# mims-harvard/G-Meta

Hardware: AMD Instinct MI355X
Metric: meta-tasks/sec (inner-loop fwd+bwd) at task_num=32 (higher is better)
Workload: dtype f32

## Files before the change

g-meta_amd/_lib.py:

```python
import ctypes as C
import os

HERE = os.path.dirname(os.path.abspath(__file__))
LIB_PATH = os.environ.get('GMETA_HIP_LIB') or os.path.join(HERE, 'libgmeta_hip.so')

GM_MAX_GCN = 4
(F_SUB_OFF, F_SET_SUB_OFF, F_PARENT, F_GRAPH, F_INDPTR, F_INDICES, F_INDPTR_T, F_INDICES_T, F_CENTRE, F_NORM,
 F_FEAT_ROW, F_NORM_SRC, F_NORM_CENTRE, F_EDGE_W, F_EDGE_W_T, F_HOP, F_NORM_E1, F_EDGE_CENTRE_T, F_OBS_CENTRE, F_OBS_E1) = range(20)
LINK_SYMMETRIC = 2
LINK_MASK_TARGET = 4
NEG_MODES = {'uniform': 0, 'two_hop': 1}
PAIR_MASK_TARGET = 1
PROP_SELF_LOOPS = 1
PROP_OPS = {'hadamard': 0, 'abs_diff': 1}
DIST_UNREACHED = 255


class Seed(C.Structure):
    _fields_ = [('graph', C.c_int32), ('i', C.c_int32), ('j', C.c_int32)]


class Model(C.Structure):
    _fields_ = [('n_gcn', C.c_int32), ('dims', C.c_int32 * (GM_MAX_GCN + 1)), ('n_out', C.c_int32), ('link_pred', C.c_int32)]

# ... 13 lines not shown
    'gm_batch_weighted': (i32, [vp]),
    'gm_store_destroy': (None, [vp]),
    'gm_store_negative_pairs': (i32, [vp, i32, i64, u64, i32, vp, i64, vp, vp, vp]),
    'gm_store_has_edges': (i32, [vp, i32, vp, i64, vp, vp]),
    'gm_store_pair_scores': (i32, [vp, i32, vp, i64, i32, vp, vp]),
    'gm_store_pair_walks': (i32, [vp, i32, vp, i64, i32, vp, vp]),
    'gm_store_rooted_pagerank': (i32, [vp, i32, vp, i64, C.c_float, i32, vp, vp]),
    'gm_store_pair_pagerank': (i32, [vp, i32, vp, i64, i32, C.c_float, i32, vp, vp]),
    'gm_store_pagerank_candidates': (i32, [vp, i32, vp, i64, i32, C.c_float, i32, vp, vp, vp, vp]),
    'gm_store_node_distances': (i32, [vp, i32, vp, i64, i32, vp, vp]),
    'gm_store_pair_distance': (i32, [vp, i32, vp, i64, i32, i32, vp, vp]),
    'gm_store_pair_distance_profile': (i32, [vp, i32, vp, i64, i32, i32, vp, vp]),
    'gm_store_sketch_build': (i32, [vp, i32, i32, i32, i32, u64, vp, vp]),
    'gm_sketch_dims': (i32, [vp, vp, vp, vp, vp, vp]),
    'gm_sketch_registers': (i32, [vp, i32, vp, i64, vp, vp, vp]),
    'gm_sketch_pair_counts': (i32, [vp, vp, i64, vp, vp, vp]),
    'gm_sketch_destroy': (None, [vp]),
    'gm_store_propagate_build': (i32, [vp, i32, i32, i32, vp, vp]),
    'gm_prop_dims': (i32, [vp, vp, vp, vp, vp, vp]),
    'gm_prop_rows': (i32, [vp, i32, vp, i64, vp, vp]),
    'gm_prop_pair_features': (i32, [vp, vp, i64, i32, vp, vp]),
    'gm_prop_destroy': (None, [vp]),
    'gm_store_neighbour_degrees': (i32, [vp, i32, vp, vp]),
    'gm_store_pair_candidates': (i32, [vp, i32, vp, i64, i32, i32, vp, vp, vp, vp]),
    'gm_extract': (C.c_int, [vp, vp, i32, vp, i32, i32, i32, u64, i32, vp, vp]),
    'gm_extract_pair': (C.c_int, [vp, vp, i32, vp, i32, vp, i32, vp, i32, i32, i32, u64, i32, vp, vp, vp]),
    'gm_batch_from_nodes': (C.c_int, [vp, vp, i32, vp, i32, vp, vp, i32, vp, vp]),
    'gm_set_hop_labels': (None, [i32]),
    'gm_get_hop_labels': (i32, []),
    'gm_batch_hop_labels': (i32, [vp]),
    'gm_batch_mask_target': (i32, [vp]),
    'gm_batch_concat': (C.c_int, [vp, i32, vp, vp]),
    'gm_batch_destroy': (None, [vp]),
    'gm_batch_prepare_cone': (C.c_int, [vp, i32, vp]),
    'gm_batch_prepare_cone_pair': (C.c_int, [vp, vp, i32, vp]),
    'gm_batch_cone_dims': (C.c_int, [vp, i32, vp, vp, vp]),
    'gm_batch_cone_read': (C.c_int, [vp, i32, i32, i32, vp, i64]),
    'gm_batch_dims': (C.c_int, [vp, vp, vp, vp, vp, vp]),
    'gm_batch_read': (C.c_int, [vp, i32, vp, i64]),
    'gm_batch_device_ptr': (C.c_int, [vp, i32, vp]),
    'gm_batch_source_rows': (C.c_int, [vp, vp]),
    'gm_batch_e1_source_rows': (C.c_int, [vp, vp]),
    'gm_gather_features': (C.c_int, [vp, vp, vp]),
    'gm_aggregate': (C.c_int, [vp, i32, i32, vp, i32, vp, vp, vp, vp]),
    'gm_aggregate_bytes': (i64, [vp, i32]),
    'gm_model_param_count': (i64, [vp]),
    'gm_gcn_ws_bytes': (i64, [vp, vp]),
    'gm_gcn_forward': (C.c_int, [vp, vp, vp, i64, vp, vp, vp, vp, i64, vp]),
    'gm_gcn_backward': (C.c_int, [vp, vp, vp, i64, vp, vp, vp, vp, i64, vp, i64, vp]),
    'gm_dense_update': (C.c_int, [vp, vp, i32, vp, i64, i32, vp, i32, vp]),
    'gm_dense_gemm': (C.c_int, [vp, vp, i64, i32, vp, i64, i32, i32, vp, i64, vp, vp, vp, i64, i32, vp, vp, vp, vp, vp, i32, vp, vp]),
    'gm_dense_fused_gemm': (C.c_int, [vp, i32, vp, i64, i32, vp, i64, vp, i64, vp, i64, i32, vp, i64, vp, vp, vp, i64, i32, vp, vp, vp, i32, vp, vp]),
    'gm_dense_wgrad_fused': (C.c_int, [vp, i32, vp, i64, i32, vp, i64, vp, i64, i32, vp, vp, vp, i64, vp, i64, i32, vp]),
    'gm_dense_aggregate': (C.c_int, [vp, i32, i32, vp, i64, i32, i32, vp, vp, i32, vp, i64, i32, vp, vp, vp, i32, vp, i64, i32, i32, i32, i32, i32, vp, vp, vp]),
    'gm_dense_agg_info': (C.c_int, [vp, i32, vp]),
    'gm_dense_fuse_counts': (C.c_int, [vp, vp]),
    'gm_dense_agg_table': (C.c_int, [vp, i32, i32, vp, i64, vp]),
    'gm_dense_dz_centre': (C.c_int, [vp, vp, i32, vp, i64, i32, vp, vp]),
    'gm_dense_wgrad_centre': (C.c_int, [vp, vp, i32, vp, i32, vp, i64, vp, i64, vp]),
    'gm_dense_agg_centre_t': (C.c_int, [vp, vp, i32, vp, vp, i32, vp]),
    'gm_dense_wgrad_e1': (C.c_int, [vp, vp, i32, vp, i32, vp, i64, vp, i64, vp]),
    'gm_dense_wgrad': (C.c_int, [vp, vp, i64, i32, vp, i64, i32, vp, vp, i64, vp, i64, vp, i64, i32, vp, vp, i64, C.c_float, vp, vp, vp, vp]),
    'gm_proto_loss_spt': (C.c_int, [vp, vp, i32, vp, i32, vp, vp, vp, vp, vp]),
    'gm_proto_loss_qry': (C.c_int, [vp, vp, i32, vp, vp, i32, vp, vp, vp, vp, vp]),
    'gm_dense_head_loss': (C.c_int, [vp, vp, i32, i32, i32, i32, vp, i64, i64, i64, vp, vp, i32, i32, vp, i32, vp, vp, vp, vp, vp, vp, vp, vp, i32, vp, i64, vp, vp,
                                     vp, vp, i64, C.c_float, vp, i32, vp, vp]),
    'gm_set_ragged_classes': (None, [i32]),
    'gm_get_ragged_classes': (i32, []),
    'gm_set_readout': (None, [i32]),
    'gm_get_readout': (i32, []),
    'gm_meta_ws_bytes': (i64, [vp, vp, vp, vp]),
    'gm_meta_out_floats': (i64, [vp, vp, vp]),
    'gm_meta_step': (C.c_int, [vp, vp, vp, vp, vp, vp, vp, vp, i64, vp, i64, vp]),
    'gm_adapt_ws_bytes': (i64, [vp, vp, vp]),
    'gm_meta_adapt': (C.c_int, [vp, vp, vp, vp, vp, vp, i64, vp, i32, vp, i64, vp]),
    'gm_predict_ws_bytes': (i64, [vp, vp, vp]),
    'gm_proto_predict': (C.c_int, [vp, vp, vp, vp, i64, vp, vp, i32, vp, vp, vp, vp, i64, vp]),
    'gm_meta_finish': (C.c_int, [vp, i64, i32, vp, vp, vp]),
    'gm_meta_finish_adam': (C.c_int, [vp, i64, i32, vp, vp, vp, vp, vp, i32, C.c_float, C.c_float, C.c_float, C.c_float, vp, vp, vp]),
    'gm_set_gemm_mode': (None, [i32]),
    'gm_get_gemm_mode': (i32, []),
    'gm_get_split_pieces': (i32, []),
    'gm_set_split_pieces': (None, [i32]),
    'gm_set_tuning': (C.c_int, [C.c_char_p, i32]),
    'gm_get_tuning': (i32, [C.c_char_p]),
    'gm_tuning_epoch': (i32, []),
    'gm_set_fuse_agg': (None, [i32]),
    'gm_get_fuse_agg': (i32, []),
    'gm_profile_enable': (None, [i32]),
    'gm_profile_aggregate': (C.c_int, [vp, vp, vp]),
    'gm_profile_read': (C.c_int, [i32, vp, vp, vp]),
    'gm_profile_read_launches': (C.c_int, [i32, vp, vp, i32]),
}
PROBE_PROTOTYPES = {
    'gm_debug_stamp': (C.c_int, [vp, vp]),
    'gm_stream_debug': (C.c_int, [i32, vp, i32]),
    'gm_head_loss_debug': (C.c_int, [i32, vp]),
}

_lib = None


def lib():
    global _lib
    if _lib is None:
        if not os.path.exists(LIB_PATH):
            raise RuntimeError('gmeta_amd: %s is missing -- run `python -c "import __graft_entry__ as g; g.build()"` '
                               '(hipcc --offload-arch=gfx950).  There is no CPU fallback.' % LIB_PATH)
        l = C.CDLL(LIB_PATH)
        for name, (res, args) in PROTOTYPES.items():
            fn = getattr(l, name)
            fn.restype, fn.argtypes = res, args
        for name, (res, args) in PROBE_PROTOTYPES.items():
            if hasattr(l, name):
                fn = getattr(l, name)
# ... 90 lines not shown
```

g-meta_amd/csrc/agg.hip:

```cpp
#include <algorithm>
#include <stdlib.h>
#include <mutex>
#include "gm_internal.h"
#include "agg_hub.h"

#define AGG_BLOCK 256

struct AggK {
    const int32_t* indptr; const int32_t* indices; const float* x; const int32_t* x_row; int64_t ldx;
    const float* s_in; const float* s_out; const float* mask_h; const float* bias; int64_t bias_stride;
    const int32_t* set_row_off; int n_sets; int relu; float* out; int64_t rows; int width; int nblocks;
    const uint8_t* mask_b; uint8_t* relu_bits;
    const int32_t* heavy; int n_heavy, heavy_deg;
    const int32_t* sched; int sched_len;
    int nt;
    int win;
    const int32_t* hub; float* hub_scratch; int hub_part, hub_ld;
    const float* e_w; const int32_t* x_idx;
    int skip_lo, skip_hi;
    const int32_t* rowlist; int64_t n_list;
    int keep_signed;
};
__host__ __device__ __forceinline__ int agg_xcd_first(const int nb, const int x) {
    const int q = nb / GM_NXCD, r = nb % GM_NXCD;
// ... 230 lines not shown
        if (dg >= 1) agg_edge(a, p0, u0, w0);
        if (dg >= 2) agg_edge(a, p0 + 1, u1, w1);
    }
    const int nwin = (int)min((int64_t)a.win, nrows_w - R0);
    const float* xl = a.x + l * 4;
    const unsigned long long live = __ballot(mine && dg >= 0);
    for (int t0 = 0; t0 < nwin; t0 += G * UNR) {
        if (!((live >> t0) & ((1ull << (G * UNR)) - 1))) continue;
        float4 acc[UNR][NCH];
        int rdg[UNR], rp0[UNR], rrow[UNR]; float rso[UNR];
#pragma unroll
        for (int k = 0; k < UNR; ++k) {
            const int rr = t0 + k * G + g;
            const int src = rr < GM_WAVE ? rr : 0;
            rdg[k] = rr < nwin ? __shfl(dg, src, 64) : -1;
            rrow[k] = __shfl(myrow32, src, 64);
            if (a.n_heavy && rdg[k] > a.heavy_deg) rdg[k] = -1;
            rp0[k] = __shfl(p0, src, 64); rso[k] = __shfl(so, src, 64);
            const int a0 = __shfl(u0, src, 64), a1 = __shfl(u1, src, 64);
            const float f0 = __shfl(w0, src, 64), f1 = __shfl(w1, src, 64);
#pragma unroll
            for (int c = 0; c < NCH; ++c) acc[k][c] = make_float4(0.f, 0.f, 0.f, 0.f);
            if (rdg[k] >= 1) {
#pragma unroll
                for (int c = 0; c < NCH; ++c) vfma(acc[k][c], *reinterpret_cast<const float4*>(xl + (int64_t)a0 * a.ldx + c * LPR * 4), f0);
            }
            if (rdg[k] >= 2) {
#pragma unroll
                for (int c = 0; c < NCH; ++c) vfma(acc[k][c], *reinterpret_cast<const float4*>(xl + (int64_t)a1 * a.ldx + c * LPR * 4), f1);
            }
        }
#pragma unroll
        for (int k = 0; k < UNR; ++k) {
            if (rdg[k] < 0) continue;
            const int rr_ = t0 + k * G + g;
            const int64_t row = a.rowlist ? (int64_t)rrow[k] : R0 + rr_;
            const int eend = rp0[k] + rdg[k];
            for (int eb = rp0[k] + 2; eb < eend; eb += LPR) agg_gather_batch<LPR, NCH, LPR, 4>(a, xl, eb, eend, l, g * LPR, acc[k]);
            agg_store_row<LPR, NCH>(a, row, rso[k], l, acc[k], a.nt);
        }
    }
}

int gm_agg_window(int64_t rows, int64_t edges) {
    const bool dense = edges > 8 * rows;
    const int min_waves = dense ? 16384 : 32768;
    const int min_win = dense ? 4 : 2;
    int win = 64;
    while (win > min_win && rows / win < min_waves) win >>= 1;
    return win;
}

int gm_agg_schedule_flat(gm_batch* b, int64_t rows, int win, const int32_t* pos, int n_heavy, const std::vector<int32_t>& tab, int32_t** d_sched, int32_t* len_out,
                         hipStream_t s, gm_stager* sg) {
    const bool split = !tab.empty();
    const int RPB = win * (AGG_BLOCK / GM_WAVE);
    const int nwb = std::max(1, (int)((rows + RPB - 1) / RPB));
    auto x_start = [&](int x) { return agg_xcd_first(nwb, x); };
    auto n_entries = [&](int k) { return split ? tab[k + 1] - tab[k] : 1; };
    int extra[GM_NXCD] = {}; int first[GM_NXCD + 1];
    {
        int hk = 0;
        for (int x = 0; x < GM_NXCD; ++x) {
            const int end = x_start(x + 1);
            first[x] = hk;
            while (hk < n_heavy && pos[hk] / RPB < end) {
                GM_REQUIRE(hk == 0 || pos[hk] >= pos[hk - 1], GM_EINVAL, "aggregate schedule: hub-row list is not ascending");
                extra[x] += n_entries(hk); ++hk;
            }
        }
        first[GM_NXCD] = hk;
        GM_REQUIRE(hk == n_heavy, GM_EINVAL, "aggregate schedule: hub-row list is not ascending / out of range");
    }
    size_t len = 0;
    for (int x = 0; x < GM_NXCD; ++x) len = std::max(len, (size_t)(x_start(x + 1) - x_start(x) + extra[x]));
    std::vector<int32_t> flat(GM_NXCD * len);
    for (int x = 0; x < GM_NXCD; ++x) {
        int32_t* o = flat.data() + x * len; int32_t* const o_end = o + len;
        int wb = x_start(x); const int end = x_start(x + 1);
        for (int hk = first[x]; hk < first[x + 1]; ++hk) {
            const int hb = pos[hk] / RPB;
            while (wb <= hb) *o++ = wb++;
            if (split) for (int g = tab[hk]; g < tab[hk + 1]; ++g) *o++ = -g - 2;
            else *o++ = -hk - 2;
        }
        while (wb < end) *o++ = wb++;
        while (o < o_end) *o++ = -1;
    }
    GM_TRY(gm_balloc(b, d_sched, flat.size(), s));
    GM_TRY(sg->upload(*d_sched, flat));
    *len_out = (int32_t)len;
    return GM_OK;
}

int gm_agg_schedule(gm_batch* b, int64_t rows, int win, const int32_t* heavy_host, const int32_t* heavy_deg_host, int n_heavy, gm_agg_sched* out, hipStream_t s, gm_stager* sg) {
    *out = gm_agg_sched{};
    if (n_heavy <= 0 || rows <= 0) return GM_OK;
    int hub_part = 0;
    std::vector<int32_t> tab;
    if (heavy_deg_host) {
        int maxdeg = 0;
        for (int k = 0; k < n_heavy; ++k) maxdeg = std::max(maxdeg, heavy_deg_host[k]);
        hub_part = std::max(128, ((maxdeg + 31) / 32 + 15) / 16 * 16);
        tab.assign(n_heavy + 1, 0);
        for (int k = 0; k < n_heavy; ++k) tab[k + 1] = tab[k] + std::max(1, (heavy_deg_host[k] + hub_part / 2) / hub_part);
        const int parts = tab[n_heavy];
        if (parts == n_heavy) { hub_part = 0; tab.clear(); }
        else {
            tab.resize(n_heavy + 1 + parts + n_heavy, 0);
            for (int k = 0; k < n_heavy; ++k) for (int g = tab[k]; g < tab[k + 1]; ++g) tab[n_heavy + 1 + g] = k;
        }
    }
    GM_TRY(gm_agg_schedule_flat(b, rows, win, heavy_host, n_heavy, tab, &out->d_sched, &out->len, s, sg));
    if (hub_part) {
        GM_TRY(gm_balloc(b, &out->d_hub, tab.size(), s));
        GM_TRY(sg->upload(out->d_hub, tab));
        GM_TRY(gm_balloc(b, &out->d_hub_scratch, (size_t)tab[n_heavy] * GM_AGG_HUB_LD, s));
        out->hub_part = hub_part; out->hub_words = (int32_t)tab.size(); out->parts = tab[n_heavy];
    }
    out->tab = tab;
    return GM_OK;
}

template <int LPR, int NCH>
static void launch_win(const AggK& a0, hipStream_t s, int* launched) {
    AggK a = a0;
    a.win = (a.sched || a.rowlist) ? a0.win : gm_agg_window(a.rows, 0);
    const int RPB = a.win * (AGG_BLOCK / GM_WAVE);
    a.nblocks = (int)(((a.rowlist ? a.n_list : a.rows) + RPB - 1) / RPB);
    int grid = a.nblocks;
    if (a.sched) grid = GM_NXCD * a.sched_len;
    else if (a.n_heavy > 0) hipLaunchKernelGGL((k_agg_heavy<LPR, NCH>), dim3(a.n_heavy), dim3(AGG_HEAVY_BLOCK), 0, s, a);
    hipLaunchKernelGGL((k_agg_win<LPR, NCH>), dim3(grid), dim3(AGG_BLOCK), 0, s, a);
    if (launched) *launched = GM_AGG_ID_WIN(LPR, NCH) + (a.sched ? GM_AGG_ID_WIN_SCHED + (a.hub ? GM_AGG_ID_WIN_SPLIT : 0) : a.n_heavy > 0 ? GM_AGG_ID_WIN_HEAVY : 0) +
                                (a.rowlist ? GM_AGG_ID_WIN_LIST : 0);
}

// ... 109 lines not shown
```

g-meta_amd/csrc/common.hip:

```cpp
#include <stdarg.h>
#include <stdlib.h>
#include <atomic>
#include <chrono>
#include <map>
#include <mutex>
#include <set>
#include <utility>
#include "gm_internal.h"

static thread_local char g_err[512] = "";

void gm_set_error(const char* fmt, ...) {
    va_list ap;
    va_start(ap, fmt);
    vsnprintf(g_err, sizeof(g_err), fmt, ap);
    va_end(ap);
}

extern "C" const char* gm_last_error(void) { return g_err; }
extern "C" int gm_version(void) { return 100; }

static void pool_keep_memory() {
    static thread_local int done_for = -1;
    int dev = 0;
// ... 251 lines not shown
extern "C" int gm_profile_read(int32_t category, double* total_ms, int64_t* launches, int64_t* work) {
    GM_REQUIRE(category >= 0 && category < GM_PROF_CATS, GM_EINVAL, "profile_read: unknown category %d", category);
    ProfCat& c = g_prof[category];
    double tot = 0;
    for (size_t k = 0; k + 1 < c.used + 1 && k < c.used; k += 2) {
        GM_HIP(hipEventSynchronize(c.ev[k + 1]));
        float ms = 0;
        GM_HIP(hipEventElapsedTime(&ms, c.ev[k], c.ev[k + 1]));
        tot += ms;
    }
    if (total_ms) *total_ms = tot;
    if (launches) *launches = c.launches;
    if (work) *work = c.work;
    return GM_OK;
}
extern "C" int gm_profile_read_launches(int32_t category, double* ms, int64_t* work, int32_t cap) {
    GM_REQUIRE(category >= 0 && category < GM_PROF_CATS && ms && work && cap >= 0, GM_EINVAL, "profile_read_launches: bad arguments");
    ProfCat& c = g_prof[category];
    int n = 0;
    for (size_t k = 0; k + 1 < c.used + 1 && k < c.used && n < cap; k += 2, ++n) {
        GM_HIP(hipEventSynchronize(c.ev[k + 1]));
        float t = 0;
        GM_HIP(hipEventElapsedTime(&t, c.ev[k], c.ev[k + 1]));
        ms[n] = t; work[n] = k / 2 < c.works.size() ? c.works[k / 2] : 0;
    }
    return n;
}
extern "C" int gm_profile_aggregate(double* total_ms, int64_t* launches, int64_t* algorithmic_bytes) {
    return gm_profile_read(GM_PROF_AGG, total_ms, launches, algorithmic_bytes);
}

#ifdef GM_PROBES
__global__ void k_debug_stamp(unsigned long long* out) { *out = wall_clock64(); }
extern "C" int gm_debug_stamp(void* out, void* stream) {
    GM_REQUIRE(out, GM_EINVAL, "debug_stamp: NULL argument");
    hipLaunchKernelGGL(k_debug_stamp, dim3(1), dim3(1), 0, (hipStream_t)stream, (unsigned long long*)out);
    GM_HIP(hipGetLastError());
    return GM_OK;
}
#endif

static gm_knobs g_knobs;
static std::once_flag g_knobs_once;
const gm_knobs& gm_knob() {
    gm_knobs& k = g_knobs;
    std::call_once(g_knobs_once, [] {
        gm_knobs& k = g_knobs;
        auto env = [](const char* name, int dflt) { const char* e = getenv(name); return e ? atoi(e) : dflt; };
        k.timing = env("GM_TIMING", 0);
        const char* gm = getenv("GM_GEMM_MODE");
        k.gemm_mode = (gm && (!strcmp(gm, "split") || !strcmp(gm, "1"))) ? 1 : (gm && (!strcmp(gm, "f32") || !strcmp(gm, "0"))) ? 0 : -1;
        k.gemm_split_min_tiles = env("GM_GEMM_SPLIT_MIN_TILES", -1);
        k.centre_store = env("GM_CENTRE_STORE", 2);
        k.dead_rows = env("GM_DEAD_ROWS", 3);
        k.fuse_agg = env("GM_FUSE_AGG", 1);
        k.fuse_diff = env("GM_FUSE_DIFF", 2);
        k.extract_pref16 = env("GM_EXTRACT_PREF16", 1);
        k.head_stage = env("GM_HEAD_STAGE", 1);
        k.head_threads = env("GM_HEAD_THREADS", 0);
        k.query_streams = env("GM_QUERY_STREAMS", 0);
        k.agg_mid_list = env("GM_AGG_MID_LIST", 1);
        k.agg_mid_win = env("GM_AGG_MID_WIN", 0);
        k.split_pieces = env("GM_SPLIT_PIECES", 3);
        k.split16_min_rows = env("GM_SPLIT16_MIN_ROWS", 65536);
        k.wgrad_split_min_chunks = env("GM_WGRAD_SPLIT_MIN_CHUNKS", -1);
        k.agg_stream = env("GM_AGG_STREAM", 1);
        k.agg_stream_min_rows = env("GM_AGG_STREAM_MIN_ROWS", 100000);
        k.neg_round = env("GM_NEG_ROUND", 0);
        k.pair_lanes = env("GM_PAIR_LANES", 0);
        k.cand_round = env("GM_CAND_ROUND", 0);
        k.cand_bitmap = env("GM_CAND_BITMAP", 0);
        k.walk_chunk = env("GM_WALK_CHUNK", 0);
        k.walk_lanes = env("GM_WALK_LANES", 0);
        k.ppr_chunk = env("GM_PPR_CHUNK", 0);
        k.ppr_cols = env("GM_PPR_COLS", 0);
        k.dist_chunk = env("GM_DIST_CHUNK", 0);
        k.dist_cols = env("GM_DIST_COLS", 0);
        k.dist_plane_kib = env("GM_DIST_PLANE_KIB", 0);
        k.sketch_chunk = env("GM_SKETCH_CHUNK", 0);
        k.sketch_mib = env("GM_SKETCH_MIB", 0);
        k.prop_chunk = env("GM_PROP_CHUNK", 0);
        k.prop_mib = env("GM_PROP_MIB", 0);
    });
    return k;
}

static std::atomic<int> g_tuning_epoch{0};
extern "C" int32_t gm_tuning_epoch(void) { return g_tuning_epoch.load(std::memory_order_relaxed); }
static int gm_knobs::* gm_find_knob(const char* name) {
    (void)gm_knob();
    static const struct { const char* name; int gm_knobs::*field; } tab[] = {
        {"GM_GEMM_SPLIT_MIN_TILES", &gm_knobs::gemm_split_min_tiles}, {"GM_CENTRE_STORE", &gm_knobs::centre_store}, {"GM_DEAD_ROWS", &gm_knobs::dead_rows},
        {"GM_HEAD_STAGE", &gm_knobs::head_stage}, {"GM_HEAD_THREADS", &gm_knobs::head_threads}, {"GM_QUERY_STREAMS", &gm_knobs::query_streams}, {"GM_AGG_MID_LIST", &gm_knobs::agg_mid_list}, {"GM_AGG_MID_WIN", &gm_knobs::agg_mid_win}, {"GM_AGG_STREAM", &gm_knobs::agg_stream}, {"GM_AGG_STREAM_MIN_ROWS", &gm_knobs::agg_stream_min_rows},
        {"GM_SPLIT16_MIN_ROWS", &gm_knobs::split16_min_rows}, {"GM_WGRAD_SPLIT_MIN_CHUNKS", &gm_knobs::wgrad_split_min_chunks}, {"GM_TIMING", &gm_knobs::timing},
        {"GM_FUSE_DIFF", &gm_knobs::fuse_diff}, {"GM_EXTRACT_PREF16", &gm_knobs::extract_pref16},
        {"neg_round", &gm_knobs::neg_round}, {"GM_NEG_ROUND", &gm_knobs::neg_round},
        {"pair_lanes", &gm_knobs::pair_lanes}, {"GM_PAIR_LANES", &gm_knobs::pair_lanes},
        {"cand_round", &gm_knobs::cand_round}, {"GM_CAND_ROUND", &gm_knobs::cand_round},
        {"cand_bitmap", &gm_knobs::cand_bitmap}, {"GM_CAND_BITMAP", &gm_knobs::cand_bitmap},
        {"walk_chunk", &gm_knobs::walk_chunk}, {"GM_WALK_CHUNK", &gm_knobs::walk_chunk},
        {"walk_lanes", &gm_knobs::walk_lanes}, {"GM_WALK_LANES", &gm_knobs::walk_lanes},
        {"ppr_chunk", &gm_knobs::ppr_chunk}, {"GM_PPR_CHUNK", &gm_knobs::ppr_chunk},
        {"ppr_cols", &gm_knobs::ppr_cols}, {"GM_PPR_COLS", &gm_knobs::ppr_cols},
        {"dist_chunk", &gm_knobs::dist_chunk}, {"GM_DIST_CHUNK", &gm_knobs::dist_chunk},
        {"dist_cols", &gm_knobs::dist_cols}, {"GM_DIST_COLS", &gm_knobs::dist_cols},
        {"dist_plane_kib", &gm_knobs::dist_plane_kib}, {"GM_DIST_PLANE_KIB", &gm_knobs::dist_plane_kib},
        {"sketch_chunk", &gm_knobs::sketch_chunk}, {"GM_SKETCH_CHUNK", &gm_knobs::sketch_chunk},
        {"sketch_mib", &gm_knobs::sketch_mib}, {"GM_SKETCH_MIB", &gm_knobs::sketch_mib},
        {"prop_chunk", &gm_knobs::prop_chunk}, {"GM_PROP_CHUNK", &gm_knobs::prop_chunk},
        {"prop_mib", &gm_knobs::prop_mib}, {"GM_PROP_MIB", &gm_knobs::prop_mib},
    };
    for (const auto& e : tab)
        if (!strcmp(name, e.name)) return e.field;
    return nullptr;
}
extern "C" int gm_set_tuning(const char* name, int32_t value) {
    GM_REQUIRE(name, GM_EINVAL, "set_tuning: NULL name");
    int gm_knobs::* f = gm_find_knob(name);
    GM_REQUIRE(f, GM_EINVAL, "set_tuning: unknown or start-up-only knob %s", name);
    g_knobs.*f = value; g_tuning_epoch.fetch_add(1, std::memory_order_relaxed);
    return GM_OK;
}
extern "C" int32_t gm_get_tuning(const char* name) {
    int gm_knobs::* f = name ? gm_find_knob(name) : nullptr;
    return f ? g_knobs.*f : 0;
}

int gm_heavy_deg() { return 64; }
int gm_heavy_deg_for(int64_t rows, int64_t edges) {
    return edges <= 8 * rows ? 32 : 64;
}

static std::mutex g_dev_mu;

int gm_num_cus() {
    static std::map<int, int> cus;
    int dev = 0;
    if (hipGetDevice(&dev) != hipSuccess) { (void)hipGetLastError(); return 256; }
    std::lock_guard<std::mutex> lk(g_dev_mu);
    auto it = cus.find(dev);
    if (it != cus.end()) return it->second;
    int n = 0;
    if (hipDeviceGetAttribute(&n, hipDeviceAttributeMultiprocessorCount, dev) != hipSuccess || n <= 0) { (void)hipGetLastError(); n = 256; }
    cus[dev] = n;
    return n;
}
// ... 12 lines not shown
```

g-meta_amd/csrc/dense_exports.hip:

```cpp
#include <algorithm>
#include "gm_internal.h"

static int set_row_amax(const gm_batch* b, const float* x, int64_t ldx, int cols, unsigned* slots, hipStream_t st) {
    int rc = GM_OK;
    for (int t0 = 0; rc == GM_OK && t0 < b->sets; t0 += 8) {
        const int segs = std::min(8, b->sets - t0);
        int64_t xo[8], xn[8];
        for (int i = 0; i < segs; ++i) {
            const int64_t r0 = b->h_set_row_off[t0 + i], nr = b->h_set_row_off[t0 + i + 1] - r0;
            xo[i] = r0 * ldx; xn[i] = nr > 0 ? (nr - 1) * ldx + cols : 0;
        }
        rc = gm_amax_segs(x, xo, xn, segs, slots + (int64_t)t0 * GM_BOUND_PAD, GM_BOUND_PAD, st);
    }
    return rc;
}

extern "C" int gm_dense_update(const gm_batch_t* b, const float* x, int32_t K, const float* W, int64_t w_stride, int32_t N, float* out, int32_t mode,
                               void* stream) {
    GM_REQUIRE(b && x && W && out && K >= 1 && N >= 1, GM_EINVAL, "dense_update: bad arguments");
    hipStream_t st = (hipStream_t)stream;
    gm_gemm_args g{};
    g.A = x; g.lda = K; g.B = W; g.b_stride = w_stride; g.C = out; g.ldc = N; g.K = K; g.N = N;
    g.tiles = b->d_tiles; g.n_tiles = b->n_tiles; g.rows = b->rows;
    uint16_t* planes = nullptr; unsigned* slots = nullptr;
// ... 13 lines not shown
            g.np = 2; g.a_bound = gm_no_bound(); g.a_bound.amax = slots; g.b_bound = wb;
        }
        if (rc == GM_OK) rc = gm_split_weights(W, w_stride, 0, K, N, 0, sets, planes, st, mode == 2 ? 2 : 3, wb);
        if (rc != GM_OK) { gm_dev_free(planes, st); if (slots) gm_dev_free(slots, st); return rc; }
        g.Bsplit = planes; g.bsplit_stride = w_stride ? (int64_t)3 * K * N : 0;
    }
    const int rc = gm_launch_gemm_nn(g, st);
    if (planes) gm_dev_free(planes, st);
    if (slots) gm_dev_free(slots, st);
    gm_batch_mark_use(b, st);
    return rc;
}

extern "C" int gm_dense_gemm(const gm_batch_t* b, const float* x, int64_t ldx, int32_t K, const float* W, int64_t w_stride, int32_t trans_w, int32_t N,
                             float* out, int64_t ldc, const float* s, const float* s_keep, const float* bias, int64_t bias_stride, int32_t relu,
                             uint8_t* relu_bits, const float* mask_h, const uint8_t* mask_b, float* zero_out, uint32_t* amax_out, int32_t mode,
                             int32_t* launched, void* stream) {
    GM_REQUIRE(b && x && W && out && K >= 1 && N >= 1 && ldx >= K && ldc >= N && mode >= -1 && mode <= 2 && !(mask_h && mask_b), GM_EINVAL,
               "dense_gemm: bad arguments");
    GM_REQUIRE(!amax_out || mode == 2, GM_EINVAL, "dense_gemm: amax_out is an output of the two-piece kernels (mode 2)");
    hipStream_t st = (hipStream_t)stream;
    const int sets = b->sets;
    gm_gemm_args g{};
    g.A = x; g.lda = ldx; g.B = W; g.b_stride = w_stride; g.transB = trans_w ? 1 : 0; g.C = out; g.ldc = ldc; g.K = K; g.N = N;
    g.row_scale = s; g.row_scale_keep = s_keep; g.n_keep = b->rows; g.bias = bias; g.bias_stride = bias_stride; g.relu = relu ? 1 : 0;
    g.relu_bits = relu_bits; g.mask_h = mask_h; g.mask_b = mask_b; g.zero_out = zero_out;
    g.tiles = b->d_tiles; g.n_tiles = b->n_tiles; g.rows = b->rows; g.launched = launched;
    uint16_t* planes = nullptr; unsigned* slots = nullptr;
    int rc = GM_OK;
    if (mode == 1 || mode == 2 || (mode < 0 && gm_gemm_split_ok(b->n_tiles, K, N))) {
        GM_REQUIRE(!mask_h && !mask_b, GM_EINVAL, "dense_gemm: the split kernels take no relu' mask");
        GM_REQUIRE((N == 256 || N == 128) && K % 16 == 0 && K >= 32, GM_EINVAL, "dense_gemm: the split kernels need N = 128 or 256 and K a multiple of 16 (>= 32)");
        const int wsets = w_stride ? sets : 1;
        rc = gm_alloc(&planes, (size_t)wsets * 3 * K * N, st);
        gm_bound wb = gm_no_bound();
        if (rc == GM_OK && mode == 2) {
            rc = gm_alloc(&slots, (size_t)(sets + wsets) * GM_BOUND_PAD, st);
            if (rc == GM_OK && hipMemsetAsync(slots, 0, sizeof(unsigned) * (sets + wsets) * GM_BOUND_PAD, st) != hipSuccess) { gm_set_error("dense_gemm: memset failed"); rc = GM_EHIP; }
            if (rc == GM_OK) rc = set_row_amax(b, x, ldx, K, slots, st);
            if (rc == GM_OK) rc = gm_amax(W, w_stride, 0, (int64_t)K * N, wsets, slots + (int64_t)sets * GM_BOUND_PAD, GM_BOUND_PAD, st);
            wb.amax = slots + (int64_t)sets * GM_BOUND_PAD; wb.stride = w_stride ? GM_BOUND_PAD : 0;
            g.np = 2; g.a_bound = gm_no_bound(); g.a_bound.amax = slots; g.a_bound.stride = GM_BOUND_PAD; g.b_bound = wb; g.amax_out = amax_out;
        }
        if (rc == GM_OK) rc = gm_split_weights(W, w_stride, 0, K, N, trans_w ? 1 : 0, wsets, planes, st, mode == 2 ? 2 : 3, wb);
        g.Bsplit = planes; g.bsplit_stride = w_stride ? (int64_t)3 * K * N : 0;
    }
    if (rc == GM_OK) rc = gm_launch_gemm_nn(g, st);
    if (planes) gm_dev_free(planes, st);
    if (slots) gm_dev_free(slots, st);
    gm_batch_mark_use(b, st);
    return rc;
}

extern "C" int gm_dense_fused_gemm(const gm_batch_t* b, int32_t table, const float* x, int64_t ldx, int32_t K, const float* zside, int64_t ldz,
                                   const float* zfull, int64_t ldzf, const float* W, int64_t w_stride, int32_t N, float* out, int64_t ldc, const float* s,
                                   const float* s_keep, const float* bias, int64_t bias_stride, int32_t relu, uint8_t* relu_bits, float* zero_out,
                                   uint32_t* amax_out, int32_t mode, int32_t* launched, void* stream) {
    GM_REQUIRE(b && W && out && zside && K >= 1 && N >= 1 && ldz >= K && ldc >= N && (mode == 1 || mode == 2) && (table == 0 || table == 1), GM_EINVAL,
               "dense_fused_gemm: bad arguments");
    GM_REQUIRE(b->d_fuse2 && b->d_fuse2_feat, GM_EINVAL, "dense_fused_gemm: the batch carries no source tables");
    GM_REQUIRE(table == 1 || (x && ldx >= K), GM_EINVAL, "dense_fused_gemm: table 0 needs x and ldx >= K");
    GM_REQUIRE(table == 0 || (b->feat && (K == b->feat_dim || K == b->feat_ld)), GM_EINVAL, "dense_fused_gemm: table 1 needs K == feat_dim (%d)", b->feat_dim);
    GM_REQUIRE(!amax_out || mode == 2, GM_EINVAL, "dense_fused_gemm: amax_out is an output of the two-piece kernels (mode 2)");
    GM_REQUIRE(mode != 2 || (zfull && ldzf >= K), GM_EINVAL, "dense_fused_gemm: mode 2 takes its A bounds over a fully aggregated Z (zfull)");
    GM_REQUIRE((N == 256 || N == 128) && K % 16 == 0 && K >= 32, GM_EINVAL, "dense_fused_gemm: the split kernels need N = 128 or 256 and K a multiple of 16 (>= 32)");
    hipStream_t st = (hipStream_t)stream;
    const int sets = b->sets, wsets = w_stride ? sets : 1;
    gm_gemm_args g{};
    g.B = W; g.b_stride = w_stride; g.C = out; g.ldc = ldc; g.K = K; g.N = N;
    g.row_scale = s; g.row_scale_keep = s_keep; g.n_keep = b->rows; g.bias = bias; g.bias_stride = bias_stride; g.relu = relu ? 1 : 0;
    g.relu_bits = relu_bits; g.zero_out = zero_out;
    g.tiles = b->d_tiles; g.n_tiles = b->n_tiles; g.rows = b->rows; g.launched = launched;
    g.zside = zside; g.ldz = ldz;
    if (table == 1) { g.A = b->feat; g.lda = b->feat_ld; g.fuse2 = b->d_fuse2_feat; }
    else { g.A = x; g.lda = ldx; g.fuse2 = b->d_fuse2; }
    uint16_t* planes = nullptr; unsigned* slots = nullptr;
    int rc = gm_alloc(&planes, (size_t)wsets * 3 * K * N, st);
    gm_bound wb = gm_no_bound();
    if (rc == GM_OK && mode == 2) {
        rc = gm_alloc(&slots, (size_t)(sets + wsets) * GM_BOUND_PAD, st);
        if (rc == GM_OK && hipMemsetAsync(slots, 0, sizeof(unsigned) * (sets + wsets) * GM_BOUND_PAD, st) != hipSuccess) { gm_set_error("dense_fused_gemm: memset failed"); rc = GM_EHIP; }
        if (rc == GM_OK) rc = set_row_amax(b, zfull, ldzf, K, slots, st);
        if (rc == GM_OK) rc = gm_amax(W, w_stride, 0, (int64_t)K * N, wsets, slots + (int64_t)sets * GM_BOUND_PAD, GM_BOUND_PAD, st);
        wb.amax = slots + (int64_t)sets * GM_BOUND_PAD; wb.stride = w_stride ? GM_BOUND_PAD : 0;
        g.np = 2; g.a_bound = gm_no_bound(); g.a_bound.amax = slots; g.a_bound.stride = GM_BOUND_PAD; g.b_bound = wb; g.amax_out = amax_out;
    }
    if (rc == GM_OK) rc = gm_split_weights(W, w_stride, 0, K, N, 0, wsets, planes, st, mode == 2 ? 2 : 3, wb);
    g.Bsplit = planes; g.bsplit_stride = w_stride ? (int64_t)3 * K * N : 0;
    if (rc == GM_OK) rc = gm_launch_gemm_nn(g, st);
    if (planes) gm_dev_free(planes, st);
    if (slots) gm_dev_free(slots, st);
    gm_batch_mark_use(b, st);
    return rc;
}

extern "C" int gm_dense_dz_centre(const gm_batch_t* b, const float* dQ, int32_t K, const float* W, int64_t w_stride, int32_t N, float* T, void* stream) {
    GM_REQUIRE(b && dQ && W && T && b->d_dq_tab, GM_EINVAL, "dense_dz_centre: bad arguments");
    GM_REQUIRE((N == 256 || N == 128) && K % 16 == 0 && K >= 64, GM_EINVAL, "dense_dz_centre: the fused split kernel needs N = 128 or 256 and K a multiple of 16 (>= 64)");
    hipStream_t st = (hipStream_t)stream;
    const int wsets = w_stride ? b->sets : 1;
    uint16_t* planes = nullptr;
    GM_TRY(gm_alloc(&planes, (size_t)wsets * 3 * K * N, st));
    gm_gemm_args g{};
    g.A = dQ; g.lda = K; g.B = W; g.b_stride = w_stride; g.transB = 1; g.C = T; g.ldc = N; g.K = K; g.N = N;
    g.row_scale = b->d_norm; g.tiles = b->d_tiles; g.n_tiles = b->n_tiles; g.rows = b->rows;
    g.fuse2 = b->d_dq_tab; g.zside = dQ; g.ldz = K;
    int rc = gm_split_weights(W, w_stride, 0, K, N, 1, wsets, planes, st, 3, gm_no_bound());
    g.Bsplit = planes; g.bsplit_stride = w_stride ? (int64_t)3 * K * N : 0; g.np = 3;
    if (rc == GM_OK) rc = gm_launch_gemm_nn(g, st);
    gm_dev_free(planes, st);
    gm_batch_mark_use(b, st);
    return rc;
}
static int dense_wgrad_keep(const gm_batch_t* b, const float* keep, const float* x, int32_t Kx, const float* dQ, int32_t N, float* dW, int64_t dw_stride, float* db,
                            int64_t db_stride, void* stream) {
    GM_REQUIRE(b && x && dQ && dW && db && keep, GM_EINVAL, "dense_wgrad_centre / _e1: bad arguments");
    const int64_t KN = (int64_t)Kx * N;
    GM_REQUIRE(b->sets == 1 || (dw_stride >= KN && db_stride >= N), GM_EINVAL, "dense_wgrad_centre / _e1: per-set outputs overlap");
    hipStream_t st = (hipStream_t)stream;
    gm_wgrad_args w{};
    w.A = x; w.lda = Kx; w.K = Kx; w.G = dQ; w.ldg = N; w.N = N; w.a_scale = b->d_norm; w.g_keep = keep;
    w.chunks = b->d_chunks; w.n_chunks = b->n_chunks; w.set_chunk_off = b->d_set_chunk_off; w.sets = b->sets; w.rows = b->rows;
    w.dW = dW; w.dw_stride = dw_stride; w.db = db; w.db_stride = db_stride; w.pick = GM_WGRAD_PICK_SPLIT;
    int rc = gm_alloc(&w.partial, (size_t)std::max(1, b->n_chunks) * (size_t)(KN + N), st);
    if (rc == GM_OK) rc = gm_launch_wgrad(w, st);
    if (w.partial) gm_dev_free(w.partial, st);
    gm_batch_mark_use(b, st);
    return rc;
}
extern "C" int gm_dense_wgrad_centre(const gm_batch_t* b, const float* x, int32_t Kx, const float* dQ, int32_t N, float* dW, int64_t dw_stride, float* db,
                                     int64_t db_stride, void* stream) {
    return dense_wgrad_keep(b, b ? b->d_norm_c : nullptr, x, Kx, dQ, N, dW, dw_stride, db, db_stride, stream);
}

extern "C" int gm_dense_agg_centre_t(const gm_batch_t* b, float* T, int32_t width, const uint8_t* mask_b, float* out, int32_t keep, void* stream) {
    GM_REQUIRE(b && T && out && width >= 4 && width % 4 == 0, GM_EINVAL, "dense_agg_centre_t: bad arguments");
    GM_REQUIRE(!keep || (b->d_ect && b->d_norm_e1), GM_EINVAL, "dense_agg_centre_t: the batch carries no centre-edge tables");
    hipStream_t st = (hipStream_t)stream;
    gm_agg_args a{};
    a.indptr = b->d_indptr_t; a.indices = b->d_indices_t;
    a.heavy = b->d_heavy[1]; a.n_heavy = b->n_heavy[1]; a.heavy_deg = b->heavy_deg;
    a.sched = b->d_sched[1]; a.sched_len = b->sched_len[1]; a.sched_win = b->sched_win;
    GM_TRY(gm_agg_hub(a, b, 1, st));
    if (b->weighted) a.e_w = b->d_ew[1];
    a.rows = b->rows; a.x = T; a.ldx = width; a.s_out = b->d_norm; a.mask_b = mask_b; a.out = out; a.width = width;
    if (keep) {
// ... 1 lines not shown
        a.x_idx = b->d_ect; a.s_out = b->d_norm_e1; a.keep_signed = 1;
    }
    const int rc = gm_launch_aggregate(a, st);
    gm_batch_mark_use(b, st);
    return rc;
}
extern "C" int gm_dense_wgrad_e1(const gm_batch_t* b, const float* x, int32_t Kx, const float* dQ, int32_t N, float* dW, int64_t dw_stride, float* db,
                                 int64_t db_stride, void* stream) {
    return dense_wgrad_keep(b, b ? b->d_norm_e1 : nullptr, x, Kx, dQ, N, dW, dw_stride, db, db_stride, stream);
}

extern "C" int gm_dense_wgrad(const gm_batch_t* b, const float* x, int64_t ldx, int32_t K, const float* g, int64_t ldg, int32_t N, const float* s,
                              const float* gb, int64_t ldgb, float* dW, int64_t dw_stride, float* db, int64_t db_stride, int32_t mode,
                              const float* cur, float* next, int64_t p_stride, float lr, float* wt, uint16_t* pl_fwd, uint16_t* pl_dz, void* stream) {
    GM_REQUIRE(b && x && g && dW && K >= 1 && N >= 1 && ldx >= K && ldg >= N && (!gb || ldgb >= N) && mode >= -1 && mode <= 2, GM_EINVAL,
               "dense_wgrad: bad arguments");
    GM_REQUIRE(K <= 2048 && N <= 2048, GM_ERANGE, "dense_wgrad: K=%d N=%d: at most 2048 columns per operand", K, N);
    const int sets = b->sets;
    const int64_t KN = (int64_t)K * N;
    GM_REQUIRE(sets == 1 || (dw_stride >= KN && (!db || db_stride >= N)), GM_EINVAL, "dense_wgrad: per-set outputs overlap");
    GM_REQUIRE(!next || (cur && db && (sets == 1 || p_stride >= KN + N)), GM_EINVAL, "dense_wgrad: the SGD step needs cur, db and a stride of at least (K+1)*N");
    GM_REQUIRE((!wt && !pl_fwd && !pl_dz) || next, GM_EINVAL, "dense_wgrad: wt and the planes are outputs of the SGD step");
    GM_REQUIRE((!pl_fwd && !pl_dz) || (K % 32 == 0 && N % 32 == 0), GM_EINVAL, "dense_wgrad: weight planes need K and N multiples of 32");
    hipStream_t st = (hipStream_t)stream;
    gm_wgrad_args w{};
    w.A = x; w.lda = ldx; w.K = K; w.G = g; w.ldg = ldg; w.N = N; w.Gb = gb; w.ldgb = ldgb; w.a_scale = s;
    w.chunks = b->d_chunks; w.n_chunks = b->n_chunks; w.set_chunk_off = b->d_set_chunk_off; w.sets = sets; w.rows = b->rows;
    w.dW = dW; w.dw_stride = dw_stride; w.db = db; w.db_stride = db_stride;
    if (next) {
        w.sgd_cur = cur; w.sgd_cur_stride = p_stride; w.sgd_next = next; w.sgd_next_stride = p_stride; w.sgd_lr = lr; w.w_off = 0; w.b_off = KN;
        w.wt_next = wt; w.pl_fwd = pl_fwd; w.pl_dz = pl_dz;
    }
    w.pick = mode == 0 ? GM_WGRAD_PICK_EXACT : mode > 0 ? GM_WGRAD_PICK_SPLIT : 0;
    unsigned* slots = nullptr;
    int rc = gm_alloc(&w.partial, (size_t)std::max(1, b->n_chunks) * (size_t)(KN + N), st);
    if (rc == GM_OK && mode == 2) {
        rc = gm_alloc(&slots, (size_t)(2 * sets + 1) * GM_BOUND_PAD, st);
        if (rc == GM_OK && hipMemsetAsync(slots, 0, sizeof(unsigned) * (2 * sets + 1) * GM_BOUND_PAD, st) != hipSuccess) { gm_set_error("dense_wgrad: memset failed"); rc = GM_EHIP; }
        if (rc == GM_OK) rc = set_row_amax(b, x, ldx, K, slots, st);
        if (rc == GM_OK) rc = set_row_amax(b, g, ldg, N, slots + (int64_t)sets * GM_BOUND_PAD, st);
        if (rc == GM_OK && s) rc = gm_amax(s, 0, 0, b->rows, 1, slots + (int64_t)2 * sets * GM_BOUND_PAD, 0, st);
        w.np = 2;
        w.a_bound = gm_no_bound(); w.a_bound.amax = slots; w.a_bound.stride = GM_BOUND_PAD;
        if (s) w.a_bound.gain = reinterpret_cast<const float*>(slots + (int64_t)2 * sets * GM_BOUND_PAD);
        w.g_bound = gm_no_bound(); w.g_bound.amax = slots + (int64_t)sets * GM_BOUND_PAD; w.g_bound.stride = GM_BOUND_PAD;
    }
    if (rc == GM_OK) rc = gm_launch_wgrad(w, st);
    if (w.partial) gm_dev_free(w.partial, st);
    if (slots) gm_dev_free(slots, st);
    gm_batch_mark_use(b, st);
    return rc;
}

extern "C" int gm_dense_wgrad_fused(const gm_batch_t* b, int32_t table, const float* A, int64_t lda, int32_t K, const float* gx, int64_t ldgx, const float* g,
                                    int64_t ldg, int32_t N, const float* s, const float* g_keep, float* dW, int64_t dw_stride, float* db, int64_t db_stride,
                                    int32_t mode, void* stream) {
    GM_REQUIRE(b && A && g && dW && db && K >= 1 && N >= 1 && lda >= K && ldg >= N && mode >= 0 && mode <= 2 && (table == 0 || table == 1), GM_EINVAL,
               "dense_wgrad_fused: bad arguments");
    GM_REQUIRE(K <= 2048 && N <= 2048, GM_ERANGE, "dense_wgrad_fused: K=%d N=%d: at most 2048 columns per operand", K, N);
    GM_REQUIRE(b->d_fuse2 && b->d_fuse2_feat, GM_EINVAL, "dense_wgrad_fused: the batch carries no source tables");
    GM_REQUIRE(table == 1 || (gx && ldgx >= K), GM_EINVAL, "dense_wgrad_fused: table 0 needs gx and ldgx >= K");
    GM_REQUIRE(table == 0 || (b->feat && (K == b->feat_dim || K == b->feat_ld)), GM_EINVAL, "dense_wgrad_fused: table 1 needs K == feat_dim (%d)", b->feat_dim);
    const int sets = b->sets;
    const int64_t KN = (int64_t)K * N;
    GM_REQUIRE(sets == 1 || (dw_stride >= KN && db_stride >= N), GM_EINVAL, "dense_wgrad_fused: per-set outputs overlap");
    hipStream_t st = (hipStream_t)stream;
    gm_wgrad_args w{};
    w.A = A; w.lda = lda; w.K = K; w.G = g; w.ldg = ldg; w.N = N; w.a_scale = s; w.g_keep = g_keep;
    w.chunks = b->d_chunks; w.n_chunks = b->n_chunks; w.set_chunk_off = b->d_set_chunk_off; w.sets = sets; w.rows = b->rows;
    w.dW = dW; w.dw_stride = dw_stride; w.db = db; w.db_stride = db_stride;
    w.fuse2 = table == 1 ? b->d_fuse2_feat : b->d_fuse2;
    w.gx = table == 1 ? b->feat : gx; w.ldgx = table == 1 ? b->feat_ld : ldgx;
    w.pick = mode == 0 ? GM_WGRAD_PICK_EXACT : GM_WGRAD_PICK_SPLIT;
    unsigned* slots = nullptr;
    int rc = gm_alloc(&w.partial, (size_t)std::max(1, b->n_chunks) * (size_t)(KN + N), st);
    if (rc == GM_OK && mode == 2) {
        rc = gm_alloc(&slots, (size_t)(2 * sets + 1) * GM_BOUND_PAD, st);
        if (rc == GM_OK && hipMemsetAsync(slots, 0, sizeof(unsigned) * (2 * sets + 1) * GM_BOUND_PAD, st) != hipSuccess) { gm_set_error("dense_wgrad_fused: memset failed"); rc = GM_EHIP; }
        w.np = 2;
        w.a_bound = gm_no_bound(); w.a_bound.amax = slots; w.a_bound.stride = GM_BOUND_PAD;
        w.g_bound = gm_no_bound(); w.g_bound.amax = slots + (int64_t)sets * GM_BOUND_PAD; w.g_bound.stride = GM_BOUND_PAD;
    }
    if (rc == GM_OK) rc = gm_launch_wgrad(w, st);
    if (w.partial) gm_dev_free(w.partial, st);
    if (slots) gm_dev_free(slots, st);
    gm_batch_mark_use(b, st);
    return rc;
}

extern "C" int gm_dense_aggregate(const gm_batch_t* b, int32_t transposed, int32_t x_src, const float* x, int64_t ldx, int32_t width, int32_t scale_src,
                                  const float* s_in, const float* s_out, int32_t keep_signed, const float* bias, int64_t bias_stride, int32_t relu,
                                  uint8_t* relu_bits, const float* mask_h, const uint8_t* mask_b, int32_t hubs, const int32_t* rowlist, int64_t n_list,
                                  int32_t list_win, int32_t list_sched, int32_t skip_lo, int32_t skip_hi, int32_t stream_ok, float* out, int32_t* launched,
                                  void* stream) {
    GM_REQUIRE(b && out && width >= 1 && x_src >= 0 && x_src <= 3 && scale_src >= 0 && scale_src <= 2 && hubs >= 0 && hubs <= 2, GM_EINVAL, "dense_aggregate: bad arguments");
    GM_REQUIRE(!(mask_h && mask_b), GM_EINVAL, "dense_aggregate: mask_h together with mask_b");
    GM_REQUIRE(!(rowlist && stream_ok), GM_EINVAL, "dense_aggregate: a row list together with the stream kernel");
    GM_REQUIRE(!stream_ok || hubs == 2, GM_EINVAL, "dense_aggregate: the stream kernel takes the batch's hub tables (hubs == 2)");
    const int o = transposed ? 1 : 0;
    const bool gather = x_src == 1 || x_src == 2;
    GM_REQUIRE(gather || (x && ldx >= width), GM_EINVAL, "dense_aggregate: a caller matrix needs x and ldx >= width");
    GM_REQUIRE(!gather || width == b->feat_dim, GM_EINVAL, "dense_aggregate: a gather needs width == feat_dim (%d)", b->feat_dim);
    GM_REQUIRE(x_src != 2 || (!transposed && b->d_efeat), GM_EINVAL, "dense_aggregate: the per-edge feature rows belong to the by-destination CSR");
    GM_REQUIRE(x_src != 3 || (transposed && b->d_ect), GM_EINVAL, "dense_aggregate: the centre-edge table belongs to the by-source CSR of a batch that carries one");
    GM_REQUIRE((scale_src == 1) == (s_in != nullptr), GM_EINVAL, "dense_aggregate: s_in goes with scale_src == 1 and only with it");
    GM_REQUIRE(scale_src != 2 || b->d_enorm[o], GM_EINVAL, "dense_aggregate: the batch has no per-edge norm table");
    GM_REQUIRE(!bias || !bias_stride || b->d_set_row_off, GM_EINVAL, "dense_aggregate: per-set bias without set row offsets");
    GM_REQUIRE(!keep_signed || s_out, GM_EINVAL, "dense_aggregate: keep_signed needs s_out");
    GM_REQUIRE(!relu_bits || relu, GM_EINVAL, "dense_aggregate: relu_bits are written with relu");
    hipStream_t st = (hipStream_t)stream;
    gm_agg_args a{};
    a.indptr = transposed ? b->d_indptr_t : b->d_indptr;
    a.indices = transposed ? b->d_indices_t : b->d_indices;
    a.rows = b->rows; a.width = width; a.out = out; a.launched = launched;
    if (gather) { a.x = b->feat; a.ldx = b->feat_ld; a.x_row = b->d_feat_row; if (x_src == 2) a.x_idx = b->d_efeat; }
    else { a.x = x; a.ldx = ldx; if (x_src == 3) a.x_idx = b->d_ect; }
    if (b->weighted) {
        GM_REQUIRE(scale_src != 1, GM_EINVAL, "dense_aggregate: on a weighted batch the source scale is none or the batch's own table (the per-source gather has no edge-weight slot)");
        GM_REQUIRE(x_src != 1, GM_EINVAL, "dense_aggregate: on a weighted batch the feature gather goes through the per-edge row table (x_src 2; the per-source gather has no edge-weight slot)");
        if (scale_src == 0) a.e_w = b->d_ew[o];
    }
    if (scale_src == 1) a.s_in = s_in;
    if (scale_src == 2) { a.s_in = b->d_norm; a.e_w = b->d_enorm[o]; }
    a.s_out = s_out; a.keep_signed = keep_signed ? 1 : 0;
    a.bias = bias; a.bias_stride = bias_stride; a.set_row_off = b->d_set_row_off; a.n_sets = b->sets;
    a.relu = relu ? 1 : 0; a.relu_bits = relu_bits; a.mask_h = mask_h; a.mask_b = mask_b;
    if (hubs) { a.heavy = b->d_heavy[o]; a.n_heavy = b->n_heavy[o]; a.heavy_deg = b->heavy_deg; }
    if (hubs == 2) { a.sched = b->d_sched[o]; a.sched_len = b->sched_len[o]; a.sched_win = b->sched_win; GM_TRY(gm_agg_hub(a, b, o, st)); }
    if (skip_lo <= skip_hi) { a.skip_on = 1; a.skip_lo = skip_lo; a.skip_hi = skip_hi; }
    if (rowlist) {
        GM_REQUIRE(n_list >= 1 && n_list <= b->rows && list_win >= 2 && list_win <= 64 && (list_win & (list_win - 1)) == 0, GM_EINVAL,
                   "dense_aggregate: a row list needs 1 .. rows entries and a window of 2, 4, .. 64 rows");
        std::vector<int32_t> h((size_t)n_list);
        GM_HIP(hipMemcpyAsync(h.data(), rowlist, sizeof(int32_t) * (size_t)n_list, hipMemcpyDeviceToHost, st));
        GM_HIP(hipStreamSynchronize(st));
        for (int64_t k = 0; k < n_list; ++k)
            GM_REQUIRE(h[k] >= 0 && h[k] < b->rows && (k == 0 || h[k] > h[k - 1]), GM_EINVAL, "dense_aggregate: the row list is not ascending / out of range at entry %lld", (long long)k);
        a.rowlist = rowlist; a.n_list = n_list; a.list_win = list_win;
        if (list_sched) {
            GM_REQUIRE(hubs == 2 && !transposed && b->d_sched_mid && n_list == b->n_mid && list_win == b->mid_win, GM_EINVAL,
                       "dense_aggregate: the list schedule goes with the batch's own list (%d rows, windows of %d) and its hub tables", b->n_mid, b->mid_win);
            a.sched = b->d_sched_mid; a.sched_len = b->sched_len_mid; a.sched_win = b->mid_win;
        } else { a.sched = nullptr; a.sched_len = 0; }
    } else GM_REQUIRE(!list_sched, GM_EINVAL, "dense_aggregate: a list schedule without a row list");
    if (stream_ok && a.e_w && a.e_w == b->d_enorm[o]) GM_TRY(gm_agg_stream_args(a, b, o, gather, st));
    const int rc = gm_launch_aggregate(a, st);
    gm_batch_mark_use(b, st);
    return rc;
}

extern "C" int gm_dense_agg_info(const gm_batch_t* b, int32_t transposed, int64_t* info) {
    GM_REQUIRE(b && info, GM_EINVAL, "dense_agg_info: bad arguments");
    const int o = transposed ? 1 : 0;
    const int64_t v[16] = {b->heavy_deg, b->n_heavy[o], b->sched_win, b->hub_part[o], b->hub_parts[o], b->d_sched[o] ? 1 : 0, b->d_mid ? b->n_mid : 0, b->mid_win,
                           b->d_sched_mid ? 1 : 0, b->d_sseg[o] ? b->stream_nseg[o] : 0, b->stream_nwg[o], b->stream_hubwg[o], b->weighted ? 1 : 0, b->feat_dim, b->feat_ld, 0};
    std::copy(v, v + 16, info);
    return GM_OK;
}
extern "C" int gm_dense_fuse_counts(const gm_batch_t* b, int64_t* counts) {
    GM_REQUIRE(b && counts, GM_EINVAL, "dense_fuse_counts: bad arguments");
    counts[0] = b->unfused_rows; counts[1] = b->unfused_edges;
    return GM_OK;
}
extern "C" int gm_dense_agg_table(const gm_batch_t* b, int32_t which, int32_t transposed, void* dst, int64_t n, void* stream) {
    GM_REQUIRE(b && dst && n >= 0 && which >= 0 && which <= 9, GM_EINVAL, "dense_agg_table: bad arguments");
    const int o = transposed ? 1 : 0;
    const void* src = which == 0 ? (const void*)b->d_enorm[o] : which == 1 ? (const void*)b->d_efeat : which == 2 ? (const void*)b->d_mid : which == 3 ? (const void*)b->d_heavy[o]
                    : which == 4 ? (const void*)b->d_fuse2 : which == 5 ? (const void*)b->d_fuse2_feat : which == 6 ? (const void*)b->d_dq_tab
                    : which == 7 ? (const void*)b->d_fwd_tab[0] : which == 8 ? (const void*)b->d_fwd_tab[1] : (const void*)b->d_fwd_tab_feat;
    const int64_t have = which <= 1 ? b->edges : which == 2 ? b->n_mid : which == 3 ? b->n_heavy[o] : b->rows;
    GM_REQUIRE(src && n <= have, GM_EINVAL, "dense_agg_table: table %d holds %lld entries", which, (long long)(src ? have : 0));
    if (n) GM_HIP(hipMemcpyAsync(dst, src, (which >= 4 ? 16 : 4) * (size_t)n, hipMemcpyDeviceToDevice, (hipStream_t)stream));
    gm_batch_mark_use(b, (hipStream_t)stream);
    return GM_OK;
}
```

g-meta_amd/csrc/extract.hip:

```cpp
#include <algorithm>
#include <initializer_list>
#include <stdlib.h>
#include <string.h>
#include <memory>
#include <mutex>
#include <type_traits>
#include "gm_internal.h"
#include "gm_devutil.h"

#define EX_BLOCK 512
#define EX_WAVES (EX_BLOCK / GM_WAVE)

__device__ __forceinline__ int lane_id() { return __builtin_amdgcn_mbcnt_hi(~0u, __builtin_amdgcn_mbcnt_lo(~0u, 0u)); }
__device__ __forceinline__ int wave_sum(int v) {
#pragma unroll
    for (int o = 32; o > 0; o >>= 1) v += __shfl_xor(v, o, 64);
    return v;
}
template <bool G> __device__ __forceinline__ bool bit_test(const uint32_t* bm, int v) { return (wld<G>(&bm[v >> 5]) >> (v & 31)) & 1u; }
__device__ __forceinline__ void bit_set(uint32_t* bm, int v) { atomicOr(&bm[v >> 5], 1u << (v & 31)); }
template <bool G, typename PT> __device__ __forceinline__ int pref_ld(const PT* p) {
    if constexpr (sizeof(PT) == 4) return (int)wld<G>(reinterpret_cast<const uint32_t*>(p)); else return (int)*p;
}
template <bool G, typename PT> __device__ __forceinline__ int bit_rank(const uint32_t* bm, const PT* pref, int v) {
// ... 572 lines not shown
    if (b->rows <= 0 || b->unfused_edges <= 0) return b->unfused_src = 0;
    const int64_t words = (b->rows + 31) / 32;
    uint32_t* bits = nullptr; unsigned long long* cnt = nullptr; unsigned long long h = 0;
    if (gm_alloc(&bits, (size_t)words, s) != GM_OK || gm_alloc(&cnt, 1, s) != GM_OK) { gm_dev_free(bits, s); return fallback; }
    bool ok = hipMemsetAsync(bits, 0, 4 * (size_t)words, s) == hipSuccess && hipMemsetAsync(cnt, 0, 8, s) == hipSuccess;
    if (ok) {
        hipLaunchKernelGGL(k_mark_sources, dim3((int)std::min<int64_t>(2048, (b->rows + 255) / 256)), dim3(256), 0, s, b->d_indptr, b->d_indices, (int64_t)b->rows, GM_FUSE_MAXDEG, bits);
        hipLaunchKernelGGL(k_count_bits, dim3((int)std::min<int64_t>(512, (words + 255) / 256)), dim3(256), 0, s, bits, words, cnt);
        ok = hipMemcpyAsync(&h, cnt, 8, hipMemcpyDeviceToHost, s) == hipSuccess && hipStreamSynchronize(s) == hipSuccess;
    }
    if (!ok) (void)hipGetLastError();
    gm_dev_free(bits, s); gm_dev_free(cnt, s);
    return ok ? (b->unfused_src = (int64_t)h) : fallback;
}
#define MID_BLOCK 1024
__device__ __forceinline__ bool mid_row(const int32_t* indptr, int64_t r, int64_t rows, int lo, int hi) {
    if (r >= rows) return false;
    const int d = indptr[r + 1] - indptr[r];
    return d >= lo && d <= hi;
}
__global__ __launch_bounds__(MID_BLOCK) void k_mid_count(const int32_t* indptr, int64_t rows, int lo, int hi, int32_t* bcnt) {
    __shared__ int wsum[MID_BLOCK / 64];
    const int64_t r = (int64_t)blockIdx.x * MID_BLOCK + threadIdx.x;
    const unsigned long long m = __ballot(mid_row(indptr, r, rows, lo, hi));
    if ((threadIdx.x & 63) == 0) wsum[threadIdx.x >> 6] = __popcll(m);
    __syncthreads();
    if (threadIdx.x == 0) { int t = 0; for (int k = 0; k < MID_BLOCK / 64; ++k) t += wsum[k]; bcnt[blockIdx.x] = t; }
}
__global__ __launch_bounds__(1024) void k_mid_scan(int32_t* bcnt, int nb) {
    __shared__ int part[1024];
    const int per = (nb + 1023) / 1024, a = threadIdx.x * per, b = min(nb, a + per);
    int t = 0;
    for (int k = a; k < b; ++k) t += bcnt[k];
    part[threadIdx.x] = t;
    __syncthreads();
    if (threadIdx.x == 0) { int run = 0; for (int k = 0; k < 1024; ++k) { const int v = part[k]; part[k] = run; run += v; } }
    __syncthreads();
    int run = part[threadIdx.x];
    for (int k = a; k < b; ++k) { const int v = bcnt[k]; bcnt[k] = run; run += v; }
}
__global__ __launch_bounds__(MID_BLOCK) void k_mid_scatter(const int32_t* indptr, int64_t rows, int lo, int hi, const int32_t* boff, int32_t* list, int cap) {
    __shared__ int wsum[MID_BLOCK / 64];
    const int64_t r = (int64_t)blockIdx.x * MID_BLOCK + threadIdx.x;
    const bool f = mid_row(indptr, r, rows, lo, hi);
    const unsigned long long m = __ballot(f);
    const int lane = threadIdx.x & 63, wv = threadIdx.x >> 6;
    if (lane == 0) wsum[wv] = __popcll(m);
    __syncthreads();
    int base = boff[blockIdx.x];
    for (int k = 0; k < wv; ++k) base += wsum[k];
    const int at = base + __popcll(m & ((1ull << lane) - 1ull));
    if (f && at < cap) list[at] = (int32_t)r;
}
__global__ void k_centre_rows(const int32_t* sub_off, const int32_t* centre, int nc, int n_c, const int32_t* indptr, const float* norm,
                              int32_t* crow, float* cnorm, int32_t* cdeg, float* norm_c, int32_t* centre_copy, int4* dq_tab) {
    const int k = blockIdx.x * blockDim.x + threadIdx.x;
    if (k >= n_c) return;
    const int row = sub_off[k / nc] + centre[k];
    centre_copy[k] = centre[k];
    crow[k] = row; cnorm[k] = norm[row]; cdeg[k] = indptr[row + 1] - indptr[row];
    if (norm_c) norm_c[row] = __uint_as_float(__float_as_uint(norm[row]) & 0x7fffffffu);
    if (dq_tab) dq_tab[row] = make_int4(row | GM_FUSE_SELF, GM_FUSE_ZERO, __float_as_int(1.f), 0);
}
struct CentreW { const float* ew; float* e_coef; };
template <typename... WArgs>
__global__ void k_centre_edges(const int32_t* crow, const int32_t* eoff, int n_c, const int32_t* indptr, const int32_t* indices,
                               const float* norm, int32_t* e_row, int32_t* e_par, float* e_norm, WArgs... w_args) {
    const int k = blockIdx.x;
    if (k >= n_c) return;
    const int p0 = indptr[crow[k]], n = eoff[k + 1] - eoff[k], o = eoff[k];
    for (int j = threadIdx.x; j < n; j += blockDim.x) {
        const int u = indices[p0 + j]; e_row[o + j] = u; e_par[o + j] = k; e_norm[o + j] = norm[u];
        if constexpr (sizeof...(WArgs) != 0) { const CentreW& cw = (w_args, ...); cw.e_coef[o + j] = cw.ew[p0 + j] * norm[u]; }
    }
}
__global__ void k_e1_tables(const int32_t* indices_t, int64_t edges, const float* norm, const float* norm_c, int64_t rows, int32_t* ect, float* norm_e1, int32_t* n_rows) {
    const int64_t n = edges > rows ? edges : rows;
    if (blockIdx.x == 0 && threadIdx.x == 0) *n_rows = 0;
    for (int64_t k = blockIdx.x * (int64_t)blockDim.x + threadIdx.x; k < n; k += (int64_t)gridDim.x * blockDim.x) {
        if (k < rows) norm_e1[k] = __uint_as_float(__float_as_uint(norm[k]) | 0x80000000u);
        if (k < edges) { const int v = indices_t[k]; ect[k] = (__float_as_uint(norm_c[v]) >> 31) ? (int32_t)(rows + (k & (GM_ZERO_ROWS - 1))) : v; }
    }
}
__global__ void k_e1_rows(const int32_t* e_row, int n_e1, float* norm_e1, int32_t* n_rows) {
    const int k = blockIdx.x * blockDim.x + threadIdx.x;
    if (k >= n_e1) return;
    const unsigned old = atomicAnd(reinterpret_cast<unsigned*>(norm_e1) + e_row[k], 0x7fffffffu);
    if (old >> 31) atomicAdd(n_rows, 1);
}
int64_t gm_batch_e1_rows(const gm_batch* b, hipStream_t s) {
    if (b->n_e1_rows >= 0) return b->n_e1_rows;
    const int64_t fallback = std::min<int64_t>(b->n_e1, b->rows);
    if (!b->d_n_e1_rows) return fallback;
    int32_t h = 0;
    if (hipMemcpyAsync(&h, b->d_n_e1_rows, 4, hipMemcpyDeviceToHost, s) != hipSuccess || hipStreamSynchronize(s) != hipSuccess) { (void)hipGetLastError(); return fallback; }
    return b->n_e1_rows = h;
}
__global__ void k_e1_kept_edges(const int32_t* indptr_t, const float* norm_e1, int64_t rows, unsigned long long* out) {
    unsigned long long c = 0;
    for (int64_t r = blockIdx.x * (int64_t)blockDim.x + threadIdx.x; r < rows; r += (int64_t)gridDim.x * blockDim.x)
        if (!(__float_as_uint(norm_e1[r]) >> 31)) c += (unsigned long long)(indptr_t[r + 1] - indptr_t[r]);
#pragma unroll
    for (int off = 32; off >= 1; off >>= 1) c += __shfl_down(c, off, 64);
    if ((threadIdx.x & 63) == 0 && c) atomicAdd(out, c);
}
int64_t gm_batch_e1_edges(const gm_batch* b, hipStream_t s) {
// ... 307 lines not shown
        } else b->spend[o].pending = true;
    }
    if (b->d_fuse2 && gm_knob().agg_mid_list) {
        const int64_t n_mid = b->unfused_rows - (int64_t)b->n_heavy[0];
        if (n_mid > 0 && n_mid < b->rows && h_cnt[0] <= cap) {
            const int nb = (int)((b->rows + MID_BLOCK - 1) / MID_BLOCK);
            int32_t* d_bcnt = nullptr;
            GM_TRY(gm_alloc(&d_bcnt, (size_t)nb, s));
            GM_TRY(gm_balloc(b, &b->d_mid, (size_t)n_mid, s));
            hipLaunchKernelGGL(k_mid_count, dim3(nb), dim3(MID_BLOCK), 0, s, b->d_indptr, (int64_t)b->rows, GM_FUSE_MAXDEG + 1, b->heavy_deg, d_bcnt);
            hipLaunchKernelGGL(k_mid_scan, dim3(1), dim3(1024), 0, s, d_bcnt, nb);
            hipLaunchKernelGGL(k_mid_scatter, dim3(nb), dim3(MID_BLOCK), 0, s, b->d_indptr, (int64_t)b->rows, GM_FUSE_MAXDEG + 1, b->heavy_deg, d_bcnt, b->d_mid, (int)n_mid);
            GM_HIP(hipGetLastError());
            gm_dev_free(d_bcnt, s);
            b->n_mid = (int32_t)n_mid;
            int win = 64;
            while (win > 2 && n_mid / win < 16384) win >>= 1;
            if (gm_knob().agg_mid_win > 0) win = gm_knob().agg_mid_win;
            b->mid_win = win;
            if (b->n_heavy[0] > 0 && b->d_sched[0]) {
                std::vector<int32_t> pos(heavy0.size());
                for (size_t k = 0; k < heavy0.size(); ++k) pos[k] = (int32_t)std::min<int64_t>(n_mid - 1, (int64_t)heavy0[k] * n_mid / b->rows);
                GM_TRY(gm_agg_schedule_flat(b, n_mid, win, pos.data(), (int)heavy0.size(), tab0, &b->d_sched_mid, &b->sched_len_mid, s, &sg));
            }
        }
    }
    tm.lap("mid-list");
    std::vector<int32_t> eoff(b->n_c + 1, 0);
    for (int k = 0; k < b->n_c; ++k) eoff[k + 1] = eoff[k] + h_cdeg[k];
    b->n_e1 = eoff[b->n_c];
    int32_t* d_eoff = nullptr;
    GM_TRY(gm_alloc(&d_eoff, eoff.size(), s));
    GM_TRY(sg.upload(d_eoff, eoff));
    GM_TRY(gm_balloc(b, &b->d_e1_row, b->n_e1, s)); GM_TRY(gm_balloc(b, &b->d_e1_par, b->n_e1, s)); GM_TRY(gm_balloc(b, &b->d_e1_norm, b->n_e1, s));
    if (b->weighted) GM_TRY(gm_balloc(b, &b->d_e1_coef, b->n_e1, s));
    auto centre_edges = [&](auto kern, auto... w) {
        hipLaunchKernelGGL(kern, dim3(b->n_c), dim3(64), 0, s, b->d_crow, d_eoff, b->n_c, b->d_indptr, b->d_indices, b->d_norm, b->d_e1_row, b->d_e1_par, b->d_e1_norm, w...);
    };
    if (b->weighted) centre_edges(k_centre_edges<CentreW>, CentreW{b->d_ew[0], b->d_e1_coef}); else centre_edges(k_centre_edges<>);
    GM_HIP(hipGetLastError());
    if (b->rows > 0 && b->d_norm_c) {
        GM_TRY(gm_balloc(b, &b->d_ect, (size_t)b->edges, s)); GM_TRY(gm_balloc(b, &b->d_norm_e1, (size_t)b->rows, s)); GM_TRY(gm_balloc(b, &b->d_n_e1_rows, 1, s));
        hipLaunchKernelGGL(k_e1_tables, dim3(grid_for(std::max<int64_t>(b->edges, b->rows), 4096)), dim3(256), 0, s, b->d_indices_t, (int64_t)b->edges, b->d_norm, b->d_norm_c, (int64_t)b->rows, b->d_ect, b->d_norm_e1, b->d_n_e1_rows);
        if (b->n_e1 > 0) hipLaunchKernelGGL(k_e1_rows, dim3((b->n_e1 + 255) / 256), dim3(256), 0, s, b->d_e1_row, b->n_e1, b->d_norm_e1, b->d_n_e1_rows);
        GM_HIP(hipGetLastError());
        if (b->d_fuse2 && b->d_fuse2_feat) {
            int4 *tc = nullptr, *te = nullptr, *tf = nullptr;
            GM_TRY(gm_balloc(b, &tc, (size_t)b->rows, s)); GM_TRY(gm_balloc(b, &te, (size_t)b->rows, s)); GM_TRY(gm_balloc(b, &tf, (size_t)b->rows, s));
            GM_TRY(gm_balloc(b, &b->d_obs[0], (size_t)b->rows, s)); GM_TRY(gm_balloc(b, &b->d_obs[1], (size_t)b->rows, s));
            hipLaunchKernelGGL(k_fwd_tables, dim3(grid_for(b->rows, 4096)), dim3(256), 0, s, (const int4*)b->d_fuse2, (const int4*)b->d_fuse2_feat, b->d_norm_c, b->d_norm_e1, (int64_t)b->rows,
                               tc, te, tf, b->d_obs[0], b->d_obs[1]);
            GM_HIP(hipGetLastError());
            b->d_fwd_tab[0] = tc; b->d_fwd_tab[1] = te; b->d_fwd_tab_feat = tf;
        }
    }
    std::vector<int32_t> ccoff, ecoff, c_set_off(b->sets + 1), e_set_off(b->sets + 1);
    for (int t = 0; t <= b->sets; ++t) { c_set_off[t] = b->h_set_sub_off[t] * nc; e_set_off[t] = eoff[b->h_set_sub_off[t] * nc]; }
    const std::vector<int32_t> ct = set_spans(c_set_off, GM_GEMM_BM), cc = set_spans(c_set_off, gm_wgrad_chunk_rows(c_set_off), &ccoff), ec = set_spans(e_set_off, gm_wgrad_chunk_rows(e_set_off), &ecoff);
    b->n_c_tiles = (int32_t)(ct.size() / 3); b->n_c_chunks = (int32_t)(cc.size() / 3); b->n_e1_chunks = (int32_t)(ec.size() / 3);
    GM_TRY(upload_tables(b, sg, s, {{&b->d_c_tiles, &ct}, {&b->d_c_chunks, &cc}, {&b->d_c_set_chunk_off, &ccoff}, {&b->d_e1_chunks, &ec}, {&b->d_e1_set_chunk_off, &ecoff}}));
    gm_dev_free(d_eoff, s);
    return GM_OK;
}
static int gm_batch_finalize(gm_batch* const* bs, int n, hipStream_t s, gm_stager& sg, gm_phase_timer* tm = nullptr) {
    FinalizeCtx fc[2];
    for (int p = 0; p < n; ++p) GM_TRY(finalize_launch(bs[p], s, sg, fc[p]));
    GM_HIP(hipStreamSynchronize(s));
    if (tm) tm->lap("finalize-wait");
    for (int p = 0; p < n; ++p) GM_TRY(finalize_finish(bs[p], s, sg, fc[p]));
    return GM_OK;
}

static int batch_alloc(gm_batch* b, hipStream_t s) {
    GM_TRY(gm_balloc(b, &b->d_sub_off, b->subs + 1, s)); GM_TRY(gm_balloc(b, &b->d_set_sub_off, b->sets + 1, s));
    GM_TRY(gm_balloc(b, &b->d_set_row_off, b->sets + 1, s)); GM_TRY(gm_balloc(b, &b->d_graph, b->subs, s));
    GM_TRY(gm_balloc(b, &b->d_parent, b->rows, s)); GM_TRY(gm_balloc(b, &b->d_feat_row, b->rows, s));
    GM_TRY(gm_balloc(b, &b->d_indptr, b->rows + 1, s)); GM_TRY(gm_balloc(b, &b->d_indices, b->edges, s));
    GM_TRY(gm_balloc(b, &b->d_indptr_t, b->rows + 1, s)); GM_TRY(gm_balloc(b, &b->d_indices_t, b->edges, s));
    GM_TRY(gm_balloc(b, &b->d_centre, (size_t)b->subs * b->centres, s)); GM_TRY(gm_balloc(b, &b->d_norm, b->rows, s));
    if (b->weighted) { GM_TRY(gm_balloc(b, &b->d_ew[0], b->edges, s)); GM_TRY(gm_balloc(b, &b->d_ew[1], b->edges, s)); }
    return GM_OK;
}

static int upload_small(gm_batch* b, gm_stager& sg) {
    GM_TRY(sg.upload(b->d_sub_off, b->h_sub_off)); GM_TRY(sg.upload(b->d_set_sub_off, b->h_set_sub_off));
    GM_TRY(sg.upload(b->d_set_row_off, b->h_set_row_off)); GM_TRY(sg.upload(b->d_graph, b->h_graph));
    return GM_OK;
}
struct BatchDrop { void operator()(gm_batch* b) const { gm_batch_destroy(b); } };
typedef std::unique_ptr<gm_batch, BatchDrop> BatchPtr;

struct ExPart { const int32_t* set_offsets; int32_t n_sets; int32_t n_seeds; };
struct ExPlan { bool gpath, p16, needx, sym; int Wmax; size_t Wp; int64_t cap; size_t lds_a, lds_b; };
static ExPlan ex_plan(const gm_store* store, int64_t cap, bool given, int link, int h) {
    ExPlan pl;
    pl.cap = cap; pl.sym = link == GM_LINK_SYMMETRIC;
    pl.Wmax = (int)((store->max_nodes + 31) >> 5);
    const size_t W = (size_t)pl.Wmax;
    pl.gpath = sizeof(uint32_t) * (2 * W + EX_BLOCK + 256 + 16) > 160 * 1024;
    pl.p16 = !pl.gpath && cap < 65536 && gm_knob().extract_pref16;
    pl.needx = !given && link != 1 && h >= 3;
    pl.Wp = pl.p16 ? (W + 1) / 2 : W;
    pl.lds_a = sizeof(uint32_t) * ((pl.gpath ? 0 : W + ((pl.p16 && !pl.needx) ? pl.Wp : W)) + EX_BLOCK + 256 + 16);
    pl.lds_b = sizeof(uint32_t) * ((pl.gpath ? 0 : W + pl.Wp) + EX_BLOCK + 16);
    return pl;
}
// ... 296 lines not shown
```

g-meta_amd/csrc/gemm.hip:

```cpp
#include <algorithm>
#include <stdlib.h>
#include "gm_internal.h"
#include <atomic>
#include <mutex>
#include "gemm_split.h"

typedef float f32x16 __attribute__((ext_vector_type(16)));

#define BK 16
#ifndef GM_GEMM_MODE_DEFAULT
#define GM_GEMM_MODE_DEFAULT 1
#endif
#define AS_LD 20

struct GemmK {
    const float* A; int64_t lda; const float* B; int64_t b_stride; int transB; float* C; int64_t ldc; int K, N;
    const float* row_scale; const float* bias; int64_t bias_stride; const float* mask_h; int relu;
    const uint8_t* mask_b; uint8_t* relu_bits;
    const int32_t* tiles; int n_tiles; int n_col_tiles; int a_vec, b_vec, c_vec; int nt_store;
    float* zero_out;
};

struct GemmTile { int set, row0, nrows, n0; };
__device__ __forceinline__ GemmTile gemm_tile(const GemmK& g, int BN) {
// ... 367 lines not shown
    return GM_OK;
}
int gm_split_np() {
    const int o = g_split_pieces.load(std::memory_order_relaxed);
    return o > 0 ? o : (gm_knob().split_pieces == 2 ? 2 : 3);
}

template <typename KArgs>
static int launch_kernel(void (*kernel)(KArgs), dim3 grid, dim3 block, size_t lds, hipStream_t s, const KArgs& k, int* launched = nullptr, int id = 0,
                         bool full_lds = false) {
    if (launched) *launched = id;
    if (full_lds) GM_TRY(gm_func_full_lds((const void*)kernel));
    hipLaunchKernelGGL(kernel, grid, block, lds, s, k);
    return GM_OK;
}
template <bool GATHER, int NP>
static int launch_gemm_split(const gm_gemm_args& a, const SplitGemmK& k, int grid, bool half_tiles, hipStream_t s) {
    const dim3 blk(1024);
    if (a.N == 128) return launch_kernel(k_gemm_split_p<GATHER, 1, 2, NP>, dim3(grid), blk, 0, s, k, a.launched, GM_GEMM_ID_SPLIT(GATHER, 1, 2, NP));
    if constexpr (!GATHER)
        if (half_tiles) return launch_kernel(k_gemm_split_p<false, 1, 4, NP>, dim3(2 * a.n_tiles), blk, 0, s, k, a.launched, GM_GEMM_ID_SPLIT(false, 1, 4, NP));
    return launch_kernel(k_gemm_split_p<GATHER, 2, 4, NP>, dim3(grid), blk, 0, s, k, a.launched, GM_GEMM_ID_SPLIT(GATHER, 2, 4, NP));
}
template <int WC>
static int launch_gemm_exact(const gm_gemm_args& a, const GemmK& g, bool vec, hipStream_t s) {
    const dim3 grid(g.n_tiles * g.n_col_tiles), blk(128 * WC);
    const int id = GM_GEMM_ID_NN(WC, vec, a.transB ? 1 : 0);
    if (vec && a.transB) return launch_kernel(k_gemm_nn<WC, true, true>, grid, blk, 0, s, g, a.launched, id);
    if (vec) return launch_kernel(k_gemm_nn<WC, true, false>, grid, blk, 0, s, g, a.launched, id);
    if (a.transB) return launch_kernel(k_gemm_nn<WC, false, true>, grid, blk, 0, s, g, a.launched, id);
    return launch_kernel(k_gemm_nn<WC, false, false>, grid, blk, 0, s, g, a.launched, id);
}

static int launch_gemm_nn(const gm_gemm_args& a, hipStream_t s);
int gm_launch_gemm_nn(const gm_gemm_args& a, hipStream_t s) {
    if (a.n_tiles <= 0) return GM_OK;
    const int cat = a.Bsplit ? (a.np == 2 ? GM_PROF_GEMM_SPLIT16 : GM_PROF_GEMM_SPLIT) : GM_PROF_GEMM;
    gm_prof_begin(cat, s, 2 * a.rows * a.K * a.N);
    if (a.Bsplit) gm_prof_note(GM_PROF_GEMM_SPLIT_BYTES, 4 * a.rows * (int64_t)a.K + 4 * (a.row_scale_keep ? a.n_keep : a.rows) * (int64_t)a.N);
    gm_prof_note(GM_PROF_GEMM_BYTES, 4 * a.rows * (int64_t)a.K + 4 * ((a.Bsplit && a.row_scale_keep) ? a.n_keep : a.rows) * (int64_t)a.N);
    const int rc = launch_gemm_nn(a, s);
    gm_prof_end(cat, s);
    return rc;
}
static int launch_gemm_nn(const gm_gemm_args& a, hipStream_t s) {
    if (a.Bsplit) {
        const bool ok = split_dims_ok(a.K, a.N) && !a.mask_h && !a.mask_b && (a.lda % 4 == 0) && (((uintptr_t)a.A & 15) == 0) &&
                        (a.ldc % 4 == 0) && (((uintptr_t)a.C & 15) == 0) && (!a.bias || a.bias_stride % 4 == 0);
        GM_REQUIRE(ok, GM_EINVAL, "gemm: launch not eligible for the split-bf16 kernel (N=%d K=%d)", a.N, a.K);
        GM_REQUIRE(!a.zero_out || a.ldc == a.N, GM_EINVAL, "gemm: the split kernels zero-fill a [rows, N] buffer only (ldc=%lld N=%d)", (long long)a.ldc, a.N);
        SplitGemmK k{};
        k.A = a.A; k.lda = a.lda; k.Bt = a.Bsplit; k.bt_stride = a.bsplit_stride; k.C = a.C; k.ldc = a.ldc; k.K = a.K; k.N = a.N;
        k.row_scale = a.row_scale_keep ? a.row_scale_keep : a.row_scale; k.keep_signed = a.row_scale_keep ? 1 : 0; k.bias = a.bias; k.bias_stride = a.bias_stride; k.relu = a.relu; k.relu_bits = a.relu_bits;
        k.tiles = a.tiles; k.n_tiles = a.n_tiles; k.n_col_tiles = 1; k.nt_store = 1; k.zero_out = a.zero_out;
        const bool f16 = a.np == 2;
        GM_REQUIRE(!f16 || (a.a_bound.amax && a.b_bound.amax), GM_EINVAL, "gemm: the two-piece split kernel needs bounds for both operands");
        k.a_bound = f16 ? a.a_bound : gm_no_bound(); k.b_bound = f16 ? a.b_bound : gm_no_bound(); k.amax_out = a.amax_out;
        const int cus = gm_num_cus();
        const int grid_cap = a.n_tiles > 2 * cus && a.n_tiles <= 6 * cus && cus >= 128 ? cus - 2 * GM_NXCD : cus;
        if (a.fuse2) {
            GM_REQUIRE(a.K / 16 >= PF_DA && a.zside && (a.ldz % 4 == 0) && (((uintptr_t)a.zside & 15) == 0), GM_EINVAL, "gemm: fused aggregate needs K >= %d and an aligned side buffer", 16 * PF_DA);
            GM_REQUIRE(a.K <= 4096, GM_EINVAL, "gemm: fused aggregate supports K <= 4096");
            k.f2 = reinterpret_cast<const int4*>(a.fuse2); k.zside = a.zside; k.ldz = a.ldz; k.zrow = gm_zero_row(s);
            GM_REQUIRE(k.zrow, GM_EHIP, "gemm: zero row allocation failed");
            const int mult_f = a.n_tiles >= 16 * grid_cap ? 2 : 3;
            const int grid = std::min(a.n_tiles, mult_f * grid_cap);
            GM_TRY(f16 ? (launch_gemm_split<true, 2>(a, k, grid, false, s)) : (launch_gemm_split<true, 3>(a, k, grid, false, s)));
        } else {
            const int grid = std::min(a.n_tiles, grid_cap);
            const bool half_tiles = 2 * a.n_tiles <= grid_cap;
            GM_TRY(f16 ? (launch_gemm_split<false, 2>(a, k, grid, half_tiles, s)) : (launch_gemm_split<false, 3>(a, k, grid, half_tiles, s)));
        }
        GM_HIP(hipGetLastError());
        return GM_OK;
    }
    GemmK g{a.A, a.lda, a.B, a.b_stride, a.transB, a.C, a.ldc, a.K, a.N, a.row_scale, a.bias, a.bias_stride, a.mask_h, a.relu,
            a.mask_b, a.relu_bits, a.tiles, a.n_tiles, 0, 0, 0, 0, 0, nullptr};
    g.a_vec = (a.K % 4 == 0) && (a.lda % 4 == 0) && (((uintptr_t)a.A & 15) == 0);
    g.b_vec = (((uintptr_t)a.B & 15) == 0) && (a.b_stride % 4 == 0) && ((a.transB ? a.K : a.N) % 4 == 0);
    g.c_vec = (a.N % 4 == 0) && (a.ldc % 4 == 0) && (((uintptr_t)a.C & 15) == 0) && (!a.mask_h || (((uintptr_t)a.mask_h & 15) == 0));
    const bool vec = g.a_vec && g.b_vec && a.K >= 4 && a.N >= 4;
    GM_REQUIRE(!(a.mask_b || a.relu_bits) || g.c_vec, GM_EINVAL, "gemm: packed relu masks need 16-byte aligned C with N %% 4 == 0");
    int bn = a.N > 128 ? 256 : a.N > 64 ? 128 : 64;
    while (bn > 64 && (int64_t)a.n_tiles * ((a.N + bn - 1) / bn) < 512) bn >>= 1;
    if (bn == 256 && a.n_tiles < 1536) bn = 128;
    g.n_col_tiles = (a.N + bn - 1) / bn;
    const bool bias_al = !a.bias || ((((uintptr_t)a.bias & 15) == 0) && (a.bias_stride % 4 == 0));
    g.nt_store = 1;
    const bool dma = vec && !a.transB && !a.mask_b && g.c_vec && bias_al && a.K % BK == 0 && a.K >= 2 * BK && a.N % bn == 0;
    if (a.zero_out) {
        if (dma && a.N == a.ldc) g.zero_out = a.zero_out;
        else GM_HIP(hipMemsetAsync(a.zero_out, 0, sizeof(float) * (size_t)a.rows * a.ldc, s));
    }
    if (dma) {
        const dim3 grid(g.n_tiles * g.n_col_tiles);
        if (bn == 256) GM_TRY(launch_kernel(k_gemm_glds<2, 4, 2>, grid, dim3(512), 0, s, g, a.launched, GM_GEMM_ID_GLDS4));
        else if (bn == 128) GM_TRY(launch_kernel(k_gemm_glds<2, 2, 2>, grid, dim3(256), 0, s, g, a.launched, GM_GEMM_ID_GLDS2));
        else if ((int64_t)g.n_tiles * g.n_col_tiles <= 4 * gm_num_cus()) GM_TRY(launch_kernel(k_gemm_glds<4, 2, 1>, grid, dim3(512), 0, s, g, a.launched, GM_GEMM_ID_GLDS_SMALL));
        else GM_TRY(launch_kernel(k_gemm_glds<2, 1, 2>, grid, dim3(128), 0, s, g, a.launched, GM_GEMM_ID_GLDS1));
    } else if (bn == 256) GM_TRY(launch_gemm_exact<4>(a, g, vec, s));
    else if (bn == 128) GM_TRY(launch_gemm_exact<2>(a, g, vec, s));
    else GM_TRY(launch_gemm_exact<1>(a, g, vec, s));
    GM_HIP(hipGetLastError());
    return GM_OK;
}

// ... 583 lines not shown
    if (tid < 32 * np && u.pl_fwd) {
        const int p = tid >> 5, c = tid & 31;
        uint16_t v[8];
#pragma unroll
        for (int q = 0; q < 8; ++q) v[q] = pl[p][q][c];
        uint4 w4 = make_uint4(v[0] | ((uint32_t)v[1] << 16), v[2] | ((uint32_t)v[3] << 16), v[4] | ((uint32_t)v[5] << 16), v[6] | ((uint32_t)v[7] << 16));
        *reinterpret_cast<uint4*>(u.pl_fwd + (int64_t)set * 3 * KN + (int64_t)p * KN + ((int64_t)kb * N + nb * 32 + c) * 8) = w4;
    } else if (tid >= 128 && tid < 128 + 32 * np && u.pl_dz) {
        const int t = tid - 128, p = t >> 5, r = t & 31, kk = r >> 2, no = r & 3;
        uint16_t v[8];
#pragma unroll
        for (int q = 0; q < 8; ++q) v[q] = pl[p][kk][no * 8 + q];
        uint4 w4 = make_uint4(v[0] | ((uint32_t)v[1] << 16), v[2] | ((uint32_t)v[3] << 16), v[4] | ((uint32_t)v[5] << 16), v[6] | ((uint32_t)v[7] << 16));
        *reinterpret_cast<uint4*>(u.pl_dz + (int64_t)set * 3 * KN + (int64_t)p * KN + (((int64_t)(nb * 4 + no)) * K + kb * 8 + kk) * 8) = w4;
    }
}

struct RedK {
    const float* partial; const int32_t* set_chunk_off; int K, N; float* dW; int64_t dw_stride; float* db; int64_t db_stride; WgradSgd u;
    int use_pl, gx;
};
__device__ __forceinline__ void wgrad_reduce_one(const RedK& r, const int bx) {
    if (bx >= r.gx) return;
    if (r.use_pl) wgrad_reduce_pl_body(r.partial, r.set_chunk_off, r.K, r.N, r.dW, r.dw_stride, r.db, r.db_stride, r.u, bx);
    else wgrad_reduce_body(r.partial, r.set_chunk_off, r.K, r.N, r.dW, r.dw_stride, r.db, r.db_stride, r.u, bx, r.gx);
}
__global__ __launch_bounds__(256) void k_wgrad_reduce(RedK r) { wgrad_reduce_one(r, blockIdx.x); }
struct RedN { RedK r[GM_MAX_GCN]; };
__global__ __launch_bounds__(256) void k_wgrad_reduce_n(RedN a) { wgrad_reduce_one(a.r[blockIdx.z], blockIdx.x); }

static int launch_wgrad(const gm_wgrad_args& a, hipStream_t s);
static bool wgrad_fast_ok(const gm_wgrad_args& a) {
    return (a.K % 32 == 0) && (a.N % 32 == 0) && !a.a_row && !a.Gb && (a.lda % 4 == 0) && (a.ldg % 4 == 0) &&
           (((uintptr_t)a.A & 15) == 0) && (((uintptr_t)a.G & 15) == 0);
}
static bool wgrad_split_dims_ok(int K, int N) { return (K == 128 || K == 256) && (N == 128 || N == 256); }
static bool wgrad_split_shape_ok(int n_chunks, int K, int N) {
    return n_chunks > 0 && gm_gemm_mode() == 1 && n_chunks >= (gm_knob().wgrad_split_min_chunks >= 0 ? gm_knob().wgrad_split_min_chunks : gm_num_cus() / 4) &&
           wgrad_split_dims_ok(K, N);
}
static bool wgrad_takes_split(const gm_wgrad_args& a) {
    if (a.pick == GM_WGRAD_PICK_EXACT) return false;
    if (a.pick == GM_WGRAD_PICK_SPLIT) return wgrad_fast_ok(a) && wgrad_split_dims_ok(a.K, a.N);
    return wgrad_fast_ok(a) && wgrad_split_shape_ok(a.n_chunks, a.K, a.N);
}
bool gm_wgrad_gather_ok(int n_chunks, int K, int N) { return wgrad_split_shape_ok(n_chunks, K, N); }
static int wgrad_np(const gm_wgrad_args& a) { return (a.np == 2 && a.a_bound.amax && a.g_bound.amax) ? 2 : 3; }
int gm_launch_wgrad(const gm_wgrad_args& a, hipStream_t s) {
    const bool split = wgrad_takes_split(a);
    GM_REQUIRE(a.pick != GM_WGRAD_PICK_SPLIT || split, GM_EINVAL,
               "wgrad: the split kernel needs K, N in {128, 256}, no Gb / row indirection and 16-byte aligned operands (K=%d N=%d)", a.K, a.N);
    const int cat = split ? (wgrad_np(a) == 2 ? GM_PROF_WGRAD_SPLIT16 : GM_PROF_WGRAD_SPLIT) : GM_PROF_WGRAD;
    gm_prof_begin(cat, s, 2 * a.rows * a.K * a.N);
    gm_prof_note(GM_PROF_WGRAD_BYTES, 4 * a.rows * ((int64_t)a.K + a.N));
    const int rc = launch_wgrad(a, s);
    gm_prof_end(cat, s);
    return rc;
}
static int launch_wgrad(const gm_wgrad_args& a, hipStream_t s) {
    const WgradSgd sgd{a.sgd_cur, a.sgd_cur_stride, a.sgd_next, a.sgd_next_stride, a.sgd_lr, a.w_off, a.b_off, a.sgd_next ? a.wt_next : nullptr,
                       a.sgd_next ? a.pl_fwd : nullptr, a.sgd_next ? a.pl_dz : nullptr, a.pl_np, a.pl_bound};
    GM_REQUIRE(!(a.pl_np == 2 && (a.pl_fwd || a.pl_dz)) || a.pl_bound.amax, GM_EINVAL, "wgrad: two-piece planes need a bound");
    auto reduce = [&](bool want_pl) -> int {
        RedK r{a.partial, a.set_chunk_off, a.K, a.N, a.dW, a.dw_stride, a.db, a.db_stride, sgd, 0, 0};
        r.use_pl = want_pl && (sgd.pl_fwd || sgd.pl_dz) && a.K % 8 == 0 && a.N % 32 == 0;
        r.gx = r.use_pl ? (a.K / 8) * (a.N / 32) + (a.N + 255) / 256 : ((a.K + 1) * a.N + 255) / 256;
        gm_wgrad_hold* h = a.hold;
        if (h && a.hold_this && h->n < GM_MAX_GCN - 1) {
            static_assert(sizeof(RedK) <= sizeof(h->slot[0]), "gm_wgrad_hold slot too small");
            memcpy(h->slot[h->n], &r, sizeof(RedK)); h->sets[h->n] = a.sets; ++h->n;
            return GM_OK;
        }
        if (h && h->n > 0) {
            RedN all{}; int gx = r.gx, n = 0;
            for (; n < h->n; ++n) { memcpy(&all.r[n], h->slot[n], sizeof(RedK)); gx = std::max(gx, all.r[n].gx); GM_REQUIRE(h->sets[n] == a.sets, GM_EINVAL, "wgrad: held reductions of different batches"); }
            all.r[n++] = r; h->n = 0;
            hipLaunchKernelGGL(k_wgrad_reduce_n, dim3(gx, a.sets, n), dim3(256), 0, s, all);
        } else {
            hipLaunchKernelGGL(k_wgrad_reduce, dim3(r.gx, a.sets), dim3(256), 0, s, r);
        }
        GM_HIP(hipGetLastError());
        return GM_OK;
    };
    if (a.n_chunks <= 0) return reduce(false);
    WgradK w{};
    w.A = a.A; w.lda = a.lda; w.K = a.K; w.a_row = a.a_row; w.G = a.G; w.ldg = a.ldg; w.N = a.N; w.Gb = a.Gb; w.ldgb = a.ldgb;
    w.a_scale = a.a_scale; w.chunks = a.chunks; w.n_chunks = a.n_chunks; w.partial = a.partial;
    w.TK = (a.K + 31) / 32; w.TN = (a.N + 31) / 32;
    bool launched = false;
    const bool fast_ok = wgrad_fast_ok(a), split = wgrad_takes_split(a);
    GM_REQUIRE(!a.fuse2 || (split && a.gx && a.np != 2 && a.lda <= (int64_t)(1 << 20) && a.ldgx <= (int64_t)(1 << 20)), GM_EINVAL,
               "wgrad: a table-formed A operand needs the split kernel (K=%d N=%d chunks=%d)", a.K, a.N, a.n_chunks);
    GM_REQUIRE(!a.g_keep || (split && wgrad_np(a) != 2), GM_EINVAL,
               "wgrad: flagged rows of G need the three-piece split kernel (K=%d N=%d chunks=%d)", a.K, a.N, a.n_chunks);
    if (split) {
        const int np = wgrad_np(a);
        const bool dr = a.g_keep != nullptr;
        if (dr) w.a_scale = a.g_keep;
        if (a.fuse2) { w.f2 = (const int4*)a.fuse2; w.gx = a.gx; w.ldgx = a.ldgx; w.zrow = gm_zero_row(s); GM_REQUIRE(w.zrow, GM_ENOMEM, "wgrad: no zero row"); }
        w.a_bound = a.a_bound; w.g_bound = a.g_bound;
        if (a.K == 256 && a.N == 256) GM_TRY((launch_wgrad_split<2, 2>(w, s, np, dr)));
        else if (a.K == 128 && a.N == 256) GM_TRY((launch_wgrad_split<1, 2>(w, s, np, dr)));
        else if (a.K == 256 && a.N == 128) GM_TRY((launch_wgrad_split<2, 1>(w, s, np, dr)));
        else GM_TRY((launch_wgrad_split<1, 1>(w, s, np, dr)));
        launched = true;
    }
    if (fast_ok && !launched) {
// ... 23 lines not shown
```

g-meta_amd/csrc/gemm_split.h:

```cpp
#pragma once
#include <hip/hip_runtime.h>
#include <stdint.h>
#include "gm_bound.h"

typedef __bf16 gm_bf16x8 __attribute__((ext_vector_type(8)));
typedef _Float16 gm_f16x8 __attribute__((ext_vector_type(8)));
typedef float gm_f32x16 __attribute__((ext_vector_type(16)));

#define GS_BM 128
#define GS_BARRIER() do { asm volatile("s_waitcnt lgkmcnt(0)" ::: "memory"); __builtin_amdgcn_s_barrier(); } while (0)

struct GsTile { int set, row0, nrows; };
__device__ __forceinline__ GsTile gs_tile(const int32_t* tiles, int lt) {
    const uint64_t p = (uint64_t)(uintptr_t)(tiles + (int64_t)lt * 3);
    const unsigned lo = __builtin_amdgcn_readfirstlane((unsigned)p), hi = __builtin_amdgcn_readfirstlane((unsigned)(p >> 32));
    const uint64_t sp = ((uint64_t)hi << 32) | lo;
    int a, b, c;
    asm volatile("s_load_dword %0, %3, 0x0\n\ts_load_dword %1, %3, 0x4\n\ts_load_dword %2, %3, 0x8\n\ts_waitcnt lgkmcnt(0)"
                 : "=&s"(a), "=&s"(b), "=&s"(c) : "s"(sp) : "memory");
    return GsTile{a, b, c};
}

__device__ __forceinline__ unsigned gs_sload(const void* q) {
    const uint64_t p = (uint64_t)(uintptr_t)q;
    const unsigned lo = __builtin_amdgcn_readfirstlane((unsigned)p), hi = __builtin_amdgcn_readfirstlane((unsigned)(p >> 32));
    const uint64_t sp = ((uint64_t)hi << 32) | lo;
    unsigned a;
    asm volatile("s_load_dword %0, %1, 0x0\n\ts_waitcnt lgkmcnt(0)" : "=&s"(a) : "s"(sp) : "memory");
    return a;
}

struct SplitGemmK {
    const float* A; int64_t lda;
    const uint16_t* Bt; int64_t bt_stride;
    float* C; int64_t ldc; int K, N;
    const float* row_scale; const float* bias; int64_t bias_stride; const float* mask_h; int relu;
    const uint8_t* mask_b; uint8_t* relu_bits;
    const int32_t* tiles; int n_tiles; int n_col_tiles; int nt_store;
    unsigned long long* dbg;
    int dephase;
    float* zero_out;
    const int4* f2; const float* zside; int64_t ldz; const float* zrow;
    gm_bound a_bound, b_bound; unsigned* amax_out;
    int keep_signed;
};
#define GM_SPLIT_FUSE_SELF 0x40000000
#define GM_SPLIT_FUSE_ZERO 0x20000000

__device__ __forceinline__ void gs_split4(const float4 v, uint2& h, uint2& m, uint2& l) {
    const float x[4] = {v.x, v.y, v.z, v.w};
    uint32_t xh[4], xm[4], xl[4];
#pragma unroll
    for (int i = 0; i < 4; ++i) {
        const uint32_t b = __float_as_uint(x[i]);
        xh[i] = b & 0xffff0000u;
        const float r1 = x[i] - __uint_as_float(xh[i]);
        const uint32_t b1 = __float_as_uint(r1);
        xm[i] = b1 & 0xffff0000u;
        const float r2 = r1 - __uint_as_float(xm[i]);
        xl[i] = __float_as_uint(r2);
    }
    h.x = __builtin_amdgcn_perm(xh[1], xh[0], 0x07060302u); h.y = __builtin_amdgcn_perm(xh[3], xh[2], 0x07060302u);
    m.x = __builtin_amdgcn_perm(xm[1], xm[0], 0x07060302u); m.y = __builtin_amdgcn_perm(xm[3], xm[2], 0x07060302u);
    l.x = __builtin_amdgcn_perm(xl[1], xl[0], 0x07060302u); l.y = __builtin_amdgcn_perm(xl[3], xl[2], 0x07060302u);
}

__device__ __forceinline__ float gs_scale_of(float bound) {
    const unsigned e = (__float_as_uint(bound) >> 23) & 0xffu;
    if (e == 0u || e == 0xffu) return 1.f;
    int se = 15 - ((int)e - 126);
    se = se < -40 ? -40 : (se > 40 ? 40 : se);
    return __uint_as_float((unsigned)(se + 127) << 23);
}
__device__ __forceinline__ float gs_bound_scale(const gm_bound& b, int set) {
    if (!b.amax) return 1.f;
    const float gain = b.gain ? __uint_as_float(gs_sload(b.gain)) : 1.f;
    return gs_scale_of(__uint_as_float(gs_sload(b.amax + (int64_t)set * b.stride)) * gain * b.hgain);
}
__device__ __forceinline__ float gs_bound_scale_v(const gm_bound& b, int set) {
    if (!b.amax) return 1.f;
    const float gain = b.gain ? b.gain[0] : 1.f;
    return gs_scale_of(__uint_as_float(b.amax[(int64_t)set * b.stride]) * gain * b.hgain);
}
__device__ __forceinline__ void gs_note_max(unsigned* slot, unsigned bits) {
    if (bits == 0u) return;
    if (__hip_atomic_load(slot, __ATOMIC_RELAXED, __HIP_MEMORY_SCOPE_AGENT) < bits) atomicMax(slot, bits);
}
__device__ __forceinline__ void gs_split4_f16(const float4 v, const float s, uint2& h, uint2& m) {
    const float x[4] = {v.x * s, v.y * s, v.z * s, v.w * s};
    _Float16 xh[4], xm[4];
#pragma unroll
    for (int i = 0; i < 4; ++i) { xh[i] = (_Float16)x[i]; xm[i] = (_Float16)(x[i] - (float)xh[i]); }
    typedef _Float16 h2 __attribute__((ext_vector_type(2)));
// ... 355 lines not shown
            gm_f32x16 acc[MI][2];
#pragma unroll
            for (int i = 0; i < MI; ++i)
#pragma unroll
                for (int j = 0; j < 2; ++j)
#pragma unroll
                    for (int e = 0; e < 16; ++e) acc[i][j][e] = 0.f;
            for (int c = 0; c < nchunks; ++c, ++gc) {
                const char* S = smem + (gc & 1) * A_ST;
                const char* SB = smem + b_st * B_ST;
                b_st = b_st + 1 == NB ? 0 : b_st + 1;
                if constexpr (NP == 3) {
                    gm_bf16x8 af[MI][3], bf[2][3];
#pragma unroll
                    for (int i = 0; i < MI; ++i)
#pragma unroll
                        for (int p = 0; p < 3; ++p) af[i][p] = *reinterpret_cast<const gm_bf16x8*>(S + a_lane + p * A_PLANE + i * 512);
#pragma unroll
                    for (int j = 0; j < 2; ++j)
#pragma unroll
                        for (int p = 0; p < 3; ++p) bf[j][p] = *reinterpret_cast<const gm_bf16x8*>(SB + b_lane + p * B_PLANE + j * 512);
#define PF_PROD(PA, PB)                                                                                                  \
                    _Pragma("unroll") for (int i = 0; i < MI; ++i) _Pragma("unroll") for (int j = 0; j < 2; ++j)          \
                        acc[i][j] = __builtin_amdgcn_mfma_f32_32x32x16_bf16(af[i][PA], bf[j][PB], acc[i][j], 0, 0, 0);
                    PF_PROD(2, 0) PF_PROD(0, 2) PF_PROD(1, 1) PF_PROD(1, 0) PF_PROD(0, 1) PF_PROD(0, 0)
#undef PF_PROD
                } else {
                    gm_f16x8 af[MI][2], bf[2][2];
#pragma unroll
                    for (int i = 0; i < MI; ++i)
#pragma unroll
                        for (int p = 0; p < 2; ++p) af[i][p] = *reinterpret_cast<const gm_f16x8*>(S + a_lane + p * A_PLANE + i * 512);
#pragma unroll
                    for (int j = 0; j < 2; ++j)
#pragma unroll
                        for (int p = 0; p < 2; ++p) bf[j][p] = *reinterpret_cast<const gm_f16x8*>(SB + b_lane + p * B_PLANE + j * 512);
#define PF_PROD(PA, PB)                                                                                                  \
                    _Pragma("unroll") for (int i = 0; i < MI; ++i) _Pragma("unroll") for (int j = 0; j < 2; ++j)          \
                        acc[i][j] = __builtin_amdgcn_mfma_f32_32x32x16_f16(af[i][PA], bf[j][PB], acc[i][j], 0, 0, 0);
                    PF_PROD(1, 0) PF_PROD(0, 1) PF_PROD(0, 0)
#undef PF_PROD
                }
                GS_BARRIER();
            }
            const GsTile tl = tile_of(b + ti * G);
            const int row0 = tl.row0, nrows = tl.nrows;
            const float* sc_t = scales + (ti & 1) * GS_BM;
            const int t4 = li & 3, q4 = li >> 2;
            const bool odd1 = (li & 1) != 0, odd2 = (li & 2) != 0;
            float4 b4[2];
#pragma unroll
            for (int j = 0; j < 2; ++j) b4[j] = *reinterpret_cast<const float4*>(biasl + (ti & 1) * BN + wc * 64 + j * 32 + q4 * 4);
            if constexpr (NP == 2) { if (g.amax_out && tl.set != vmax_set) { if (vmax_set >= 0) vmax_flush(); vmax_set = tl.set; } }
            const bool keep_only = g.keep_signed && !g.relu_bits && !g.zero_out;
            if (keep_only && __ballot(!(__float_as_uint(sc_t[wr * 32 * MI + (lane & (32 * MI - 1))]) >> 31)) == 0ull) continue;
#pragma unroll
            for (int i = 0; i < MI; ++i) {
#pragma unroll
                for (int gq = 0; gq < 4; ++gq) {
                    const int rl = wr * 32 * MI + i * 32 + gq * 8 + kh * 4 + t4;
                    const float sc_raw = sc_t[rl];
                    const bool keep = !g.keep_signed || !(__float_as_uint(sc_raw) >> 31);
                    if (keep_only && __ballot(keep) == 0ull) continue;
                    const float sc = fabsf(sc_raw);
                    const int64_t row = row0 + rl;
#pragma unroll
                    for (int j = 0; j < 2; ++j) {
                        float a0 = acc[i][j][gq * 4 + 0], a1 = acc[i][j][gq * 4 + 1], a2 = acc[i][j][gq * 4 + 2], a3 = acc[i][j][gq * 4 + 3];
                        gs_quad_transpose(a0, a1, a2, a3, odd1, odd2);
                        float4 v;
                        v.x = a0 * sc + b4[j].x; v.y = a1 * sc + b4[j].y; v.z = a2 * sc + b4[j].z; v.w = a3 * sc + b4[j].w;
                        if (g.relu) { v.x = v.x < 0.f ? 0.f : v.x; v.y = v.y < 0.f ? 0.f : v.y; v.z = v.z < 0.f ? 0.f : v.z; v.w = v.w < 0.f ? 0.f : v.w; }
                        if (rl >= nrows || (keep_only && !keep)) continue;
                        const int col = wc * 64 + j * 32 + q4 * 4;
                        if constexpr (NP == 2) { if (g.amax_out) vmax = fmaxf(fmaxf(vmax, fmaxf(fabsf(v.x), fabsf(v.y))), fmaxf(fabsf(v.z), fabsf(v.w))); }
                        if (g.relu_bits) g.relu_bits[(row * g.ldc + col) >> 2] = (uint8_t)((v.x > 0.f) | ((v.y > 0.f) << 1) | ((v.z > 0.f) << 2) | ((v.w > 0.f) << 3));
                        if (!keep) {
                        } else if (g.nt_store) {
                            typedef float f4v __attribute__((ext_vector_type(4)));
                            f4v vv = {v.x, v.y, v.z, v.w};
                            __builtin_nontemporal_store(vv, reinterpret_cast<f4v*>(g.C + row * g.ldc + col));
                        } else {
                            *reinterpret_cast<float4*>(g.C + row * g.ldc + col) = v;
                        }
                        if (g.zero_out) {
                            typedef float f4z __attribute__((ext_vector_type(4)));
                            f4z z;
                            asm volatile("v_mov_b32 %0, 0\n\tv_mov_b32 %1, 0\n\tv_mov_b32 %2, 0\n\tv_mov_b32 %3, 0" : "=v"(z.x), "=v"(z.y), "=v"(z.z), "=v"(z.w));
                            *reinterpret_cast<f4z*>(g.zero_out + row * g.ldc + col) = z;
                        }
                    }
                }
            }
        }
        if constexpr (NP == 2) { if (g.amax_out && vmax_set >= 0) vmax_flush_last(); }
    }
}
```

g-meta_amd/csrc/gm_internal.h:

```cpp
#pragma once
#include <hip/hip_runtime.h>
#include "gm_bound.h"
#include <stdint.h>
#include <stdio.h>
#include <mutex>
#include <stdlib.h>
#include <string.h>
#include <vector>
#include <algorithm>
#include "../../include/gmeta_hip.h"

#define GM_WAVE 64
#define GM_NXCD 8

void gm_set_error(const char* fmt, ...);

#define GM_HIP(call)                                                                              \
    do {                                                                                          \
        hipError_t e__ = (call);                                                                  \
        if (e__ != hipSuccess) {                                                                  \
            gm_set_error("%s failed: %s (%s:%d)", #call, hipGetErrorString(e__), __FILE__, __LINE__); \
            return GM_EHIP;                                                                       \
        }                                                                                         \
    } while (0)
// ... 81 lines not shown
    int32_t* d_indices_t = nullptr;
    int32_t* d_centre = nullptr;
    std::vector<int32_t> h_centre;
    float* d_norm = nullptr;
    bool weighted = false;
    bool mask_target = false;
    float* d_ew[2] = {nullptr, nullptr};
    int32_t* d_sub_set = nullptr;
    int32_t* d_tiles = nullptr;
    int32_t n_tiles = 0;
    int32_t* d_chunks = nullptr;
    int32_t n_chunks = 0;
    int32_t* d_set_chunk_off = nullptr;
    int32_t* d_heavy[2] = {nullptr, nullptr};
    int32_t n_heavy[2] = {0, 0};
    int32_t heavy_deg = 64;
    int32_t* d_sched[2] = {nullptr, nullptr};
    int32_t sched_len[2] = {0, 0};
    int32_t sched_win = 0;
    int32_t* d_hub[2] = {nullptr, nullptr}; float* d_hub_scratch[2] = {nullptr, nullptr}; int32_t hub_part[2] = {0, 0};
    int32_t hub_words[2] = {0, 0}, hub_parts[2] = {0, 0};
    mutable int32_t* d_hub2[2] = {nullptr, nullptr}; mutable float* d_hub_scratch2[2] = {nullptr, nullptr};
    mutable hipStream_t hub_stream[4] = {nullptr, nullptr, nullptr, nullptr}; mutable bool hub_used[4] = {false, false, false, false}; mutable hipEvent_t hub_ev[4] = {nullptr, nullptr, nullptr, nullptr};
    float* d_enorm[2] = {nullptr, nullptr}; int32_t* d_efeat = nullptr;
    float* d_gain = nullptr;
    void* d_fuse2 = nullptr; void* d_fuse2_feat = nullptr;
    int64_t unfused_rows = 0, unfused_edges = 0;
    int32_t* d_mid = nullptr; int32_t n_mid = 0, mid_win = 0;
    int32_t* d_sptr[2] = {nullptr, nullptr}; int32_t* d_su[2] = {nullptr, nullptr}; int32_t* d_su_feat = nullptr; float* d_sw[2] = {nullptr, nullptr};
    int32_t* d_scum[2] = {nullptr, nullptr}; int2* d_sseg[2] = {nullptr, nullptr}; int32_t* d_sxord[2] = {nullptr, nullptr};
    int32_t stream_nseg[2] = {0, 0}, stream_nwg[2] = {0, 0}, stream_hubwg[2] = {0, 0}, stream_nparts[2] = {0, 0}, stream_enorm[2] = {0, 0};
    struct stream_pending { bool pending = false; bool has_tab = false; int n_parts = 0; std::vector<int32_t> hubs, deg, tab; };
    mutable stream_pending spend[2];
    int32_t* d_sched_mid = nullptr; int32_t sched_len_mid = 0;
    mutable int64_t unfused_src = -1;
    int32_t n_c = 0;
    int32_t* d_crow = nullptr;
    float* d_cnorm = nullptr;
    float* d_norm_c = nullptr;
    float* d_norm_src = nullptr;
    int64_t n_src = 0;
    void* d_dq_tab = nullptr;
    int32_t n_e1 = 0;
    int32_t* d_e1_row = nullptr;
    int32_t* d_e1_par = nullptr;
    int32_t* d_ect = nullptr;
    float* d_norm_e1 = nullptr;
    int32_t* d_n_e1_rows = nullptr;
    mutable int64_t n_e1_rows = -1;
    mutable int64_t n_e1_edges = -1;
    void* d_fwd_tab[2] = {nullptr, nullptr};
    void* d_fwd_tab_feat = nullptr;
    float* d_obs[2] = {nullptr, nullptr};
    mutable int64_t fwd_cnt[2][3] = {{-1, -1, -1}, {-1, -1, -1}};
    float* d_e1_norm = nullptr;
    float* d_e1_coef = nullptr;
    int32_t* d_c_tiles = nullptr; int32_t n_c_tiles = 0;
    int32_t* d_c_chunks = nullptr; int32_t* d_c_set_chunk_off = nullptr; int32_t n_c_chunks = 0;
    int32_t* d_e1_chunks = nullptr; int32_t* d_e1_set_chunk_off = nullptr; int32_t n_e1_chunks = 0;
    mutable int32_t* d_ro_chunks = nullptr; mutable int32_t* d_ro_multi = nullptr; mutable int32_t n_ro_chunks = 0, n_ro_multi = 0;
    mutable hipStream_t ro_stream = nullptr; mutable hipEvent_t ro_ev = nullptr;
    mutable gm_cone* cone[GM_MAX_GCN + 1] = {};
    hipStream_t stream = nullptr;
    struct slab { char* base; size_t cap, used; };
    std::vector<slab> slabs;
    std::mutex slab_mu;
    mutable hipEvent_t used_ev = nullptr;
};
int gm_batch_gains(const gm_batch* b, hipStream_t s);
int gm_balloc_bytes(gm_batch* b, void** p, size_t bytes, hipStream_t s);
template <class T> static inline int gm_balloc(gm_batch* b, T** p, size_t n, hipStream_t s) { return gm_balloc_bytes(b, (void**)p, (n ? n : 1) * sizeof(T), s); }
void gm_batch_mark_use(const gm_batch* b, hipStream_t st);
int gm_batch_wait_build(const gm_batch* b, hipStream_t s);
static inline int gm_hop_feat_dim(const gm_store* st, int centres, int D) { return st->feat_dim + centres * (D + 2); }

struct gm_knobs {
    int timing;
    int extract_pref16;
    int gemm_mode;
    int gemm_split_min_tiles;
    int centre_store;
    int dead_rows;
    int fuse_agg, head_stage;
    int fuse_diff;
    int agg_mid_win;
    int agg_mid_list;
    int query_streams;
    int head_threads;
    int split16_min_rows;
    int split_pieces;
    int wgrad_split_min_chunks;
    int agg_stream;
    int agg_stream_min_rows;
    int neg_round;
    int pair_lanes;
    int cand_round;
    int walk_chunk;
    int walk_lanes;
    int ppr_chunk;
    int ppr_cols;
    int dist_chunk;
    int dist_cols;
    int dist_plane_kib;
    int cand_bitmap;
    int sketch_chunk;
    int sketch_mib;
    int prop_chunk;
    int prop_mib;
};
const gm_knobs& gm_knob();

int gm_nbr_index(const gm_store* s);
void gm_nbr_release(const gm_store* s);
int gm_pair_lanes(const gm_store* s, int32_t g, const char* what, int* lpp);
int gm_pair_scores_launch(const gm_store* s, int32_t g, int lpp, const int32_t* d_pairs, int64_t n, int mask, float* d_out, hipStream_t st);

#define GM_CAND_THREADS 256
#define GM_CAND_WAVES (GM_CAND_THREADS / GM_WAVE)
#define GM_CAND_MAX_K 1024

__device__ __forceinline__ unsigned long long gm_cand_key(uint32_t score_bits, int32_t w) {
    return ((unsigned long long)score_bits << 32) | (unsigned long long)(0xFFFFFFFFu - (uint32_t)w);
}

__device__ __forceinline__ int gm_cand_scan(int v, int* part, int* total) {
    const int lane = (int)threadIdx.x & (GM_WAVE - 1), wave = (int)threadIdx.x / GM_WAVE;
    int inc = v;
#pragma unroll
    for (int o = 1; o < GM_WAVE; o <<= 1) { const int t = __shfl_up(inc, o, GM_WAVE); if (lane >= o) inc += t; }
    __syncthreads();
    if (lane == GM_WAVE - 1) part[wave] = inc;
    __syncthreads();
    int base = 0, tot = 0;
#pragma unroll
    for (int w = 0; w < GM_CAND_WAVES; ++w) { const int p = part[w]; tot += p; if (w < wave) base += p; }
    *total = tot;
    return base + inc;
}
// ... 138 lines not shown
    const uint8_t* mask_b;
    uint8_t* relu_bits;
    const float* bias;
    int64_t bias_stride;
    const int32_t* set_row_off;
    int n_sets;
    int relu;
    float* out;
    int64_t rows;
    int width;
    const int32_t* heavy;
    int n_heavy;
    int heavy_deg;
    const int32_t* sched;
    int sched_len, sched_win;
    const int32_t* hub; float* hub_scratch; int hub_part;
    const int32_t* rowlist; int64_t n_list; int list_win;
    const gm_batch* stream; int stream_o; int stream_feat; int64_t stream_xrows;
    int* launched;
};
#define GM_AGG_ID_LPR(LPR) ((LPR) == 64 ? 6 : (LPR) == 32 ? 5 : (LPR) == 16 ? 4 : (LPR) == 8 ? 3 : (LPR) == 4 ? 2 : 1)
#define GM_AGG_ID_ONE(VEC, LPR) (100 + ((VEC) == 4 ? 10 : 0) + GM_AGG_ID_LPR(LPR))
#define GM_AGG_ID_WIN(LPR, NCH) (200 + 16 * ((NCH) == 2 ? 3 : GM_AGG_ID_LPR(LPR) - 4))
#define GM_AGG_ID_WIN_SCHED 1
#define GM_AGG_ID_WIN_SPLIT 2
#define GM_AGG_ID_WIN_HEAVY 4
#define GM_AGG_ID_WIN_LIST 8
#define GM_AGG_ID_STREAM(LPR, SPLIT) (300 + 2 * (GM_AGG_ID_LPR(LPR) - 4) + ((SPLIT) ? 1 : 0))
int gm_agg_stream_args(gm_agg_args& a, const gm_batch* b, int o, bool gather, hipStream_t s);
bool gm_stream_ok(const gm_agg_args& g);
bool gm_stream_batch_ok(const gm_batch* b, int o);
int gm_launch_stream(const gm_agg_args& g, int nt, hipStream_t s);
int gm_stream_tables(gm_batch* b, int o, const int32_t* hubs_host, const int32_t* deg_host, int n_hubs, int n_parts, const std::vector<int32_t>* part_tab, hipStream_t s,
                     gm_stager* sg);
#define GM_FUSE_SELF 0x40000000
#define GM_FUSE_ZERO 0x20000000
const float* gm_zero_row(hipStream_t s);
#ifndef GM_ZERO_ROWS
#define GM_ZERO_ROWS 1
#endif
#define GM_FUSE_MAXDEG 2
#define GM_AGG_HUB_LD 512
struct gm_agg_sched { int32_t* d_sched = nullptr; int32_t len = 0; int32_t* d_hub = nullptr; float* d_hub_scratch = nullptr; int32_t hub_part = 0; int32_t hub_words = 0, parts = 0;
                      std::vector<int32_t> tab; };
int gm_batch_hub_order(const gm_batch* b, int o, hipStream_t s, int set = 0);
int gm_batch_hub_alt(const gm_batch* b, hipStream_t s);
template <class A> inline int gm_agg_hub(A& a, const gm_batch* b, int o, hipStream_t s, int set = 0) {
    const bool alt = set == 1 && b->d_hub2[o];
    a.hub = alt ? b->d_hub2[o] : b->d_hub[o]; a.hub_scratch = alt ? b->d_hub_scratch2[o] : b->d_hub_scratch[o]; a.hub_part = b->hub_part[o];
    return a.hub ? gm_batch_hub_order(b, o, s, alt ? 1 : 0) : GM_OK;
}
int gm_agg_window(int64_t rows, int64_t edges);
struct gm_stager;
int gm_agg_schedule_flat(gm_batch* b, int64_t rows, int win, const int32_t* pos, int n_heavy, const std::vector<int32_t>& tab, int32_t** d_sched, int32_t* len, hipStream_t s, gm_stager* sg);
int gm_agg_schedule(gm_batch* b, int64_t rows, int win, const int32_t* heavy_host, const int32_t* heavy_deg_host, int n_heavy, gm_agg_sched* out, hipStream_t s, gm_stager* sg);
int gm_heavy_deg();
int gm_heavy_deg_for(int64_t rows, int64_t edges);
int gm_launch_aggregate(const gm_agg_args& a, hipStream_t s);

struct gm_gemm_args {
    const float* A; int64_t lda;
    const float* B; int64_t b_stride;
    int transB;
    float* C; int64_t ldc;
    int K, N;
    const float* row_scale;
    const float* row_scale_keep;
    int64_t n_keep;
    const float* bias; int64_t bias_stride;
    int relu;
    const float* mask_h;
    const uint8_t* mask_b;
    uint8_t* relu_bits;
    const uint16_t* Bsplit; int64_t bsplit_stride;
    const void* fuse2; const float* zside; int64_t ldz;
    int np; gm_bound a_bound, b_bound; unsigned* amax_out;
    float* zero_out;
    const int32_t* tiles;
    int n_tiles;
    int64_t rows;
    int* launched;
};
#define GM_GEMM_ID_GLDS4 1
#define GM_GEMM_ID_GLDS2 2
#define GM_GEMM_ID_GLDS1 3
#define GM_GEMM_ID_GLDS_SMALL 4
#define GM_GEMM_ID_NN(WC, VEC, TB) (10 + 4 * ((WC) == 4 ? 2 : (WC) == 2 ? 1 : 0) + 2 * (VEC) + (TB))
#define GM_GEMM_ID_SPLIT(GATHER, MI, WC, NP) (30 + 10 * (GATHER) + ((MI) == 2 ? 0 : (WC) == 4 ? 2 : 4) + ((NP) == 2))
#define GM_GEMM_BM 128
int gm_launch_gemm_nn(const gm_gemm_args& a, hipStream_t s);
int gm_gemm_mode();
bool gm_gemm_split_ok(int n_tiles, int K, int N);
int gm_split_weights(const float* params, int64_t pstride, int64_t w_off, int K, int N, int trans, int sets, uint16_t* out, hipStream_t s, int np = 3,
                     gm_bound bound = gm_no_bound());
int gm_amax(const float* x, int64_t stride, int64_t off, int64_t n, int sets, unsigned* out, int64_t out_stride, hipStream_t s);
int gm_amax_segs(const float* x, const int64_t* off, const int64_t* n, int segs, unsigned* out, int64_t out_stride, hipStream_t s);
int gm_split_np();

struct gm_wgrad_hold { int n = 0; int sets[GM_MAX_GCN] = {}; alignas(16) unsigned char slot[GM_MAX_GCN][256] = {}; };
struct gm_wgrad_args {
    const float* A; int64_t lda; int K;
    const int32_t* a_row;
    const float* G; int64_t ldg; int N;
    const float* Gb; int64_t ldgb;
    const float* a_scale;
    const int32_t* chunks;
    int n_chunks;
    const int32_t* set_chunk_off;
    int sets;
    float* partial;
    float* dW; int64_t dw_stride;
    float* db; int64_t db_stride;
    const float* sgd_cur; int64_t sgd_cur_stride; float* sgd_next; int64_t sgd_next_stride; float sgd_lr;
    int64_t w_off, b_off;
    int np; gm_bound a_bound, g_bound; int pl_np; gm_bound pl_bound;
    uint16_t* pl_fwd; uint16_t* pl_dz;
    float* wt_next;
    int64_t rows;
    const void* fuse2; const float* gx; int64_t ldgx;
    const float* g_keep;
    gm_wgrad_hold* hold; int hold_this;
    int pick;
};
#define GM_WGRAD_PICK_EXACT 1
#define GM_WGRAD_PICK_SPLIT 2
#define GM_WGRAD_ROWS 1024
int gm_launch_wgrad(const gm_wgrad_args& a, hipStream_t s);
bool gm_wgrad_gather_ok(int n_chunks, int K, int N);

int gm_num_cus();
int gm_func_full_lds(const void* fn);
#define GM_WGRAD_EXTRA_ROUND_PCT 25
static inline int gm_wgrad_chunk_rows(const std::vector<int32_t>& set_off, int n_cu = gm_num_cus()) {
    const int sets = (int)set_off.size() - 1;
    int64_t total = 0; int mx = 1;
    for (int t = 0; t < sets; ++t) { const int n = set_off[t + 1] - set_off[t]; total += n; mx = n > mx ? n : mx; }
    if (total <= 0) return 128;
    auto chunks_at = [&](int cr) { int64_t c = 0; for (int t = 0; t < sets; ++t) c += (set_off[t + 1] - set_off[t] + cr - 1) / cr; return c; };
    int best = 128; double best_eff = -1.0;
    for (int rounds : {1, 2, 3, 4, 6, 8}) {
        const int64_t cap = (int64_t)n_cu * rounds;
        int lo = 1, hi = (mx + 31) / 32;
        if (chunks_at(32 * hi) > cap) continue;
        while (lo < hi) { const int mid = (lo + hi) / 2; if (chunks_at(32 * mid) <= cap) hi = mid; else lo = mid + 1; }
        const int cr = std::max(128, 32 * lo);
        const int64_t c = chunks_at(cr);
        const double eff = (double)total / ((double)((c + n_cu - 1) / n_cu) * n_cu * cr);
        if (eff > best_eff + 0.01 * GM_WGRAD_EXTRA_ROUND_PCT) { best_eff = eff; best = cr; }
    }
    return best;
}

#define GM_PROF_AGG 0
#define GM_PROF_GEMM 1
#define GM_PROF_WGRAD 2
#define GM_PROF_AGG_STRICT 3
#define GM_PROF_GEMM_SPLIT 4
#define GM_PROF_WGRAD_SPLIT 5
#define GM_PROF_GEMM_SPLIT16 6
#define GM_PROF_WGRAD_SPLIT16 7
#define GM_PROF_STEP_CATS 8
#define GM_PROF_EX_NODES 8
#define GM_PROF_EX_FILL 9
#define GM_PROF_EX_FINAL 10
#define GM_PROF_GEMM_SPLIT_BYTES 11
#define GM_PROF_AGG_BOUND 12
#define GM_PROF_GEMM_BYTES 13
#define GM_PROF_WGRAD_BYTES 14
#define GM_PROF_HEAD 15
#define GM_PROF_READOUT 16
#define GM_PROF_READOUT_BWD 17
#define GM_PROF_CATS 18
// ... 13 lines not shown
```

g-meta_amd/csrc/model.hip:

```cpp
#include <algorithm>
#include <atomic>
#include <map>
#include <stdlib.h>
#include "gm_internal.h"


__device__ __forceinline__ float wave_sumf(float v) {
#pragma unroll
    for (int o = 32; o > 0; o >>= 1) v += __shfl_xor(v, o, 64);
    return v;
}

struct HeadK {
    const float* H; int64_t ldh; int Hd;
    const int32_t* sub_off; const int32_t* centre; int nc; const int32_t* sub_set; const int32_t* set_sub_off;
    const float* params; int64_t pstride; int64_t wl_off, bl_off; int hc, C; int subs;
    int compact;
    unsigned* dq_amax;
    int subs_per_set;
};

__device__ __forceinline__ int64_t centre_row(const HeadK& k, int s, int which) {
    return k.compact ? (int64_t)s * k.nc + which : (int64_t)k.sub_off[s] + k.centre[s * k.nc + which];
}
// ... 522 lines not shown
        if (id < P) { const int64_t src = id < cut ? id : id + shift; if (gq) for (int t = 0; t < T; ++t) s += gq[t * stride + src] + gp[t * stride + src]; }
        else if (id < P + K1) { for (int t = 0; t < T; ++t) s += lq[t * K1 + (id - P)]; if (vw && id == P + K1 - 1) s = __uint_as_float(0x7fc00000u); }
        else if (id < P + 2 * K1) { for (int t = 0; t < T; ++t) s += aq[t * K1 + (id - P - K1)]; }
        else if (id == P + 2 * K1) s = (float)T;
        else s = aq[id - P - 2 * K1 - 1];
        out[id] = s;
    }
}

struct Carver {
    char* base; int64_t used = 0, cap;
    Carver(void* p, int64_t c) : base((char*)p), cap(c) {}
    template <class T> T* take(int64_t n) {
        const int64_t bytes = ((n > 0 ? n : 1) * (int64_t)sizeof(T) + 255) / 256 * 256;
        T* r = base ? (T*)(base + used) : nullptr;
        used += bytes;
        return r;
    }
    bool ok() const { return !base || used <= cap; }
};

#define GM_W_HEADROOM 1024.f
struct PlaneDir {
    const float* fw0 = nullptr; int64_t TP = 0; int K = 0;
    uint16_t* base = nullptr; int64_t per_k = 0;
    int64_t off[GM_MAX_GCN][2] = {};
    bool valid[64][GM_MAX_GCN][2] = {};
    int index_of(const float* params) const {
        if (!base || !fw0 || params < fw0) return 0;
        const int64_t d = params - fw0;
        if (d % TP) return 0;
        const int64_t k = d / TP + 1;
        return (k >= 1 && k <= K && k < 64) ? (int)k : 0;
    }
    uint16_t* slot(int k, int l, int o) const { return (k && off[l][o] >= 0) ? base + (int64_t)(k - 1) * per_k + off[l][o] : nullptr; }
    uint16_t* lookup(const float* params, int l, int o) const { const int k = index_of(params); return (k && off[l][o] >= 0 && valid[k][l][o]) ? slot(k, l, o) : nullptr; }
    unsigned* wam = nullptr; const float* theta = nullptr;
    unsigned* viol = nullptr;
    bool w_bound(const float* params, int l, gm_bound& bd) const {
        bd = gm_no_bound();
        if (!wam || !(index_of(params) || params == theta)) return false;
        bd.amax = wam + (int64_t)l * GM_BOUND_PAD; bd.stride = 0; bd.gain = nullptr; bd.hgain = GM_W_HEADROOM; bd.viol = viol;
        return true;
    }
};

struct GcnCtx {
    const gm_batch* b; gm_layout L;
    PlaneDir* pd;
    bool is_support = false;
    enum DqFill { DQ_MEMSET, DQ_ZEROED, DQ_CENTRE } dq = DQ_MEMSET;
    bool t_zero = false;
    bool zfused[GM_MAX_GCN] = {};
    float* Z[GM_MAX_GCN]; float* H[GM_MAX_GCN]; float* X0; float* bufA; float* bufB; float* partial;
    float* partial_l[GM_MAX_GCN];
    gm_wgrad_hold hold;
    uint16_t* Wsplit;
    float* WTl[GM_MAX_GCN];
    const float* wt_of[GM_MAX_GCN]; int64_t wt_stride[GM_MAX_GCN];
    uint8_t* M[GM_MAX_GCN];
    float* cG2; float* cT2; float* cG1; float* partial_c;
    float* Pool; float* Gpool; float* ro_part;
    const float* x0_user; const int32_t* centre; int z1_valid;
    int zw[GM_MAX_GCN];
    const gm_cone* cone;
    SgdK sgd;
    int hub_set = 0;
    int np = 3; unsigned* am = nullptr; int am_passes = 0, am_pass = -1;
    const unsigned* feat_bound = nullptr;
    bool hv[GM_MAX_GCN] = {}, tv[GM_MAX_GCN] = {}; bool dqv = false;
    unsigned* am_slot(int i) const { return am + ((int64_t)am_pass * (2 * L.n_gcn + 1) + i) * b->sets * GM_BOUND_PAD; }
    unsigned* amH(int l) const { return am_slot(l); }
    unsigned* amT(int l) const { return am_slot(L.n_gcn + l); }
    unsigned* amdQ() const { return am_slot(2 * L.n_gcn); }
};
static bool in_bound(const GcnCtx& c, int l, gm_bound& bd) {
    bd = gm_no_bound();
    if (c.np != 2 || c.am_pass < 0 || !c.b->d_gain) return false;
    if (l == 0) {
        if (c.x0_user || !c.feat_bound) return false;
        bd.amax = c.feat_bound; bd.stride = 1;
    } else {
        if (!c.hv[l - 1]) return false;
        bd.amax = c.amH(l - 1); bd.stride = GM_BOUND_PAD;
    }
    bd.gain = c.b->d_gain; bd.hgain = 1.f;
    return true;
}
static bool dq_bound(const GcnCtx& c, int l, gm_bound& bd) {
    bd = gm_no_bound();
    if (c.np != 2 || c.am_pass < 0 || !c.b->d_gain) return false;
    if (l == c.L.n_gcn - 1) { if (!c.dqv) return false; bd.amax = c.amdQ(); bd.gain = nullptr; }
    else { if (!c.tv[l + 1]) return false; bd.amax = c.amT(l + 1); bd.gain = c.b->d_gain + 1; }
    bd.stride = GM_BOUND_PAD; bd.hgain = 1.f;
    return true;
}
static int weight_planes(GcnCtx& c, const float* params, int64_t pstride, int l, int o, int K, int N, bool want16, hipStream_t st, const uint16_t** pl, gm_bound* bb, int* np) {
    const gm_layout& L = c.L;
    uint16_t* have = (c.pd && pstride) ? c.pd->lookup(params, l, o) : nullptr;
    *bb = gm_no_bound();
    if (have && c.np == 2) {
        if (want16 && c.pd->w_bound(params, l, *bb)) { *pl = have; *np = 2; return GM_OK; }
        have = nullptr;
    }
    if (have) { *pl = have; *np = 3; return GM_OK; }
    const bool f16 = want16 && c.pd && c.pd->w_bound(params, l, *bb);
// ... 69 lines not shown
    return cv.used + 256;
}

static int head_subs_per_set(const gm_batch* b) {
    int n = b->sets > 0 ? b->subs / b->sets : 0;
    for (int t = 0; t <= b->sets && n; ++t) if (b->h_set_sub_off[t] != t * n) n = 0;
    return n;
}
static HeadK make_head(const GcnCtx& c, const float* params, int64_t pstride) {
    const gm_layout& L = c.L; const gm_batch* b = c.b;
    HeadK k{};
    k.H = c.H[L.n_gcn - 1]; k.ldh = L.dims[L.n_gcn]; k.Hd = L.dims[L.n_gcn];
    k.sub_off = b->d_sub_off; k.centre = c.centre ? c.centre : b->d_centre; k.nc = b->centres; k.sub_set = b->d_sub_set;
    k.set_sub_off = b->d_set_sub_off; k.params = params; k.pstride = pstride; k.wl_off = L.wl_off; k.bl_off = L.bl_off;
    k.hc = L.hc; k.C = L.n_out; k.subs = b->subs; k.compact = c.cone ? 1 : 0;
    if (mean_readout(c)) { k.H = c.Pool; k.compact = 1; k.nc = 1; }
    k.dq_amax = (c.np == 2 && c.am_pass >= 0) ? c.amdQ() : nullptr;
    k.subs_per_set = head_subs_per_set(b);
    return k;
}
static int launch_head_fwd(const GcnCtx& c, const float* params, int64_t pstride, float* logits, hipStream_t st) {
    hipLaunchKernelGGL(k_head_fwd, dim3((c.b->subs + 3) / 4), dim3(256), 0, st, make_head(c, params, pstride), logits);
    GM_HIP(hipGetLastError());
    return GM_OK;
}
static int launch_head_bwd(GcnCtx& c, const float* params, int64_t pstride, const float* dlogits, float* dparams, int64_t dstride, float* dQ, float* Gc, hipStream_t st) {
    const HeadK k = make_head(c, params, pstride);
    hipLaunchKernelGGL(k_head_bwd, dim3(c.b->sets), dim3(256), 0, st, k, dlogits, dparams, dstride, dQ, Gc);
    GM_HIP(hipGetLastError());
    if (dQ && k.dq_amax) c.dqv = true;
    return GM_OK;
}

static int launch_agg(const gm_agg_args& a, int64_t bytes, int64_t strict_bytes, hipStream_t st) {
    gm_prof_agg_begin(st, bytes); gm_prof_note(GM_PROF_AGG_STRICT, strict_bytes);
    const int rc = gm_launch_aggregate(a, st);
    gm_prof_agg_end(st);
    return rc;
}
static int batch_agg(const GcnCtx& c, int dir, hipStream_t st, gm_agg_args& a) {
    const gm_batch* b = c.b;
    a = gm_agg_args{};
    if (dir == 0) { a.indptr = b->d_indptr; a.indices = b->d_indices; } else { a.indptr = b->d_indptr_t; a.indices = b->d_indices_t; }
    a.heavy = b->d_heavy[dir]; a.n_heavy = b->n_heavy[dir]; a.heavy_deg = b->heavy_deg;
    a.sched = b->d_sched[dir]; a.sched_len = b->sched_len[dir]; a.sched_win = b->sched_win;
    GM_TRY(gm_agg_hub(a, b, dir, st, c.hub_set));
    a.rows = b->rows;
    if (b->weighted) a.e_w = b->d_ew[dir];
    return GM_OK;
}

static bool dz_split_ok(const GcnCtx& c, int l) { return c.Wsplit && gm_gemm_split_ok(c.b->n_tiles, c.L.dims[l + 1], c.L.dims[l]); }
static bool dz_centre_ok(const GcnCtx& c, int l) { return dz_split_ok(c, l) && c.L.dims[l + 1] >= 64 && c.L.dims[l + 1] <= 4096 && c.b->d_dq_tab; }
static float* t_zero_rows(const GcnCtx& c) {
    const gm_layout& L = c.L; const int Lg = L.n_gcn;
    if (c.cone || Lg < 2 || !c.bufB || L.dims[Lg - 1] > L.dims[Lg]) return nullptr;
    for (int l = 0; l < Lg - 1; ++l) if (std::min(L.dims[l], L.dims[l + 1]) > L.dims[Lg - 1]) return nullptr;
    return c.bufB + c.b->rows * (int64_t)L.dims[Lg - 1];
}
static int t_zero_fill(GcnCtx& c, hipStream_t st) {
    float* z = t_zero_rows(c);
    c.t_zero = z && gm_knob().dead_rows >= 2 && gm_knob().centre_store != 0 && dz_centre_ok(c, c.L.n_gcn - 1) && c.b->d_ect && c.b->d_norm_e1;
    if (c.t_zero) GM_HIP(hipMemsetAsync(z, 0, sizeof(float) * GM_ZERO_ROWS * c.L.dims[c.L.n_gcn - 1], st));
    return GM_OK;
}

int gm_gather_rows(const gm_batch* b, const int32_t* feat_row, int64_t n, int F, float* out, hipStream_t st);
static int cone_forward(GcnCtx& c, const float* params, int64_t pstride, float* logits, hipStream_t st, int reuse_z1, int skip_head);
static int cone_backward(GcnCtx& c, const float* params, int64_t pstride, const float* dlogits, float* dparams, int64_t dstride, hipStream_t st, int skip_head);

static std::atomic<int> g_fuse_agg_override{-1};
extern "C" void gm_set_fuse_agg(int32_t on) { g_fuse_agg_override.store(on < 0 ? -1 : (on ? 1 : 0), std::memory_order_relaxed); }
extern "C" int32_t gm_get_fuse_agg(void) { const int o = g_fuse_agg_override.load(std::memory_order_relaxed); return o >= 0 ? o : gm_knob().fuse_agg; }

static int gcn_forward(GcnCtx& c, const float* params, int64_t pstride, float* logits, hipStream_t st, int reuse_z1, int skip_head = 0, int fwd_only = 0) {
    if (c.cone) return cone_forward(c, params, pstride, logits, st, reuse_z1, skip_head);
    const gm_layout& L = c.L; const gm_batch* b = c.b;
    if (!c.x0_user) GM_TRY(gm_check_feat_dim(b, L.dims[0], "forward"));
    GM_REQUIRE((L.link != 0) == (b->centres == 2), GM_EINVAL, "forward: link_pred model needs a 2-centre batch and vice versa");
    const float* xin = c.x0_user;
    c.dq = GcnCtx::DQ_MEMSET;
    const bool mean = mean_readout(c);
    if (mean) GM_TRY(readout_tables(b, st));
    const bool dead_rows = gm_knob().dead_rows && gm_knob().centre_store != 0 && !c.centre;
    if (c.np == 2) {
        ++c.am_pass;
        GM_REQUIRE(c.am_pass < c.am_passes, GM_EINVAL, "forward: more passes than bound slots (%d)", c.am_passes);
        for (int l = 0; l < GM_MAX_GCN; ++l) c.hv[l] = c.tv[l] = false;
        c.dqv = false;
    }
    auto layer_split_ok = [&](int l) {
        return c.Wsplit && gm_gemm_split_ok(b->n_tiles, L.dims[l], L.dims[l + 1]) && ((uintptr_t)(params + L.b_off[l]) & 15) == 0 && pstride % 4 == 0;
    };
    auto layer_fuse = [&](int l) {
        const int fi = L.dims[l], fo = L.dims[l + 1];
        const bool gather = (l == 0 && !c.x0_user);
        const bool keeps_stream = gm_knob().fuse_diff == 2 && c.is_support && gm_knob().agg_stream && gm_stream_batch_ok(b, 0);
        const bool diff_ok = fwd_only == 2 && gm_knob().fuse_diff && !keeps_stream && c.np != 2 && !c.cone && gm_wgrad_gather_ok(b->n_chunks, fi, fo);
        return (fwd_only == 1 || diff_ok) && gm_get_fuse_agg() && layer_split_ok(l) && !(l == 0 && reuse_z1) && fi >= 64 && fi % 4 == 0 && b->d_fuse2 && b->d_enorm[0] &&
               (!gather || (b->feat_ld % 4 == 0 && b->feat_ld >= fi)) &&
               2 * b->unfused_rows <= b->rows;
    };
    const int Lg = L.n_gcn;
    const bool fwd3_last = fwd_only == 1 && gm_knob().dead_rows >= 3 && dead_rows && gm_knob().centre_store >= 1 && !mean && c.np != 2 && b->d_norm_c && b->d_norm_e1 &&
                           b->d_fwd_tab[0] && b->d_obs[0] && L.dims[Lg - 1] <= L.dims[Lg] && layer_fuse(Lg - 1) &&
                           (Lg >= 2 || c.x0_user);
    const bool fwd3_below = fwd3_last && Lg >= 2 && L.dims[Lg - 2] <= L.dims[Lg - 1] && layer_split_ok(Lg - 2) && b->d_fwd_tab[1] && b->d_fwd_tab_feat && b->d_obs[1];
    for (int l = 0; l < L.n_gcn; ++l) {
        const int fi = L.dims[l], fo = L.dims[l + 1];
        const bool gather = (l == 0 && !c.x0_user);
        const int obs = (fwd3_last && l == Lg - 1) ? 0 : (fwd3_below && l == Lg - 2) ? 1 : -1;
        if (fi > fo) {
            const float* A = xin; int64_t lda = fi;
            if (gather) { GM_TRY(gm_gather_rows(b, b->d_feat_row, b->rows, fi, c.X0, st)); A = c.X0; }
            gm_gemm_args g{}; g.A = A; g.lda = lda; g.B = params + L.w_off[l]; g.b_stride = pstride; g.C = c.Z[l]; g.ldc = fo; g.K = fi; g.N = fo;
            g.row_scale = b->d_norm; g.tiles = b->d_tiles; g.n_tiles = b->n_tiles; g.rows = b->rows;
            GM_TRY(gm_launch_gemm_nn(g, st));
            gm_agg_args a; GM_TRY(batch_agg(c, 0, st, a));
            a.x = c.Z[l]; a.ldx = fo; a.s_out = b->d_norm;
            a.bias = params + L.b_off[l]; a.bias_stride = pstride; a.set_row_off = b->d_set_row_off; a.n_sets = b->sets; a.relu = 1;
            a.out = c.H[l]; a.width = fo; a.relu_bits = c.M[l];
            GM_TRY(launch_agg(a, gm_aggregate_bytes(b, fo), gm_aggregate_bytes(b, fo), st));
        } else {
            const bool split_ok = layer_split_ok(l);
            const bool fuse = layer_fuse(l);
            c.zfused[l] = fuse && fwd_only == 2;
            if (!(l == 0 && reuse_z1 && c.z1_valid)) {
                gm_agg_args a; GM_TRY(batch_agg(c, 0, st, a));
                a.s_in = b->d_norm; a.e_w = b->d_enorm[0]; a.out = c.Z[l]; a.width = fi;
                if (gather) { a.x = b->feat; a.x_row = b->d_feat_row; a.x_idx = b->d_efeat; a.ldx = b->feat_ld; }
                else { a.x = xin; a.ldx = fi; }
                if (fuse) {
                    a.skip_on = 1; a.skip_lo = 0; a.skip_hi = GM_FUSE_MAXDEG;
                    if (b->d_mid && c.hub_set == 0 && gm_knob().agg_mid_list && (b->n_heavy[0] == 0 || b->d_sched_mid)) {
                        a.rowlist = b->d_mid; a.n_list = b->n_mid; a.list_win = b->mid_win;
                        if (b->n_heavy[0] > 0) { a.sched = b->d_sched_mid; a.sched_len = b->sched_len_mid; a.sched_win = b->mid_win; }
                        else { a.sched = nullptr; a.sched_len = 0; }
                    }
                    int64_t pb0 = 4 * (b->rows + 1) + 4 * b->unfused_edges + 4 * b->unfused_rows + 4 * b->unfused_rows * (int64_t)fi;
                    int64_t src, src_bound = std::min<int64_t>(b->unfused_edges, b->rows);
                    if (obs >= 0) {
                        a.s_out = b->d_obs[obs]; a.keep_signed = 1;
                        int64_t w[3] = {std::min<int64_t>(b->unfused_rows, obs == 0 ? b->n_c : b->n_e1), b->unfused_edges, 0};
                        w[2] = std::min<int64_t>(w[1], b->rows);
                        if (gm_prof_enabled()) GM_TRY(gm_batch_fwd_counts(b, obs, st, w));
                        pb0 = 4 * (b->rows + 1) + 8 * b->unfused_rows + 4 * w[1] + 4 * w[0] * (int64_t)fi;
                        src = w[2]; src_bound = std::min<int64_t>(w[1], b->rows);
                    } else src = gm_prof_enabled() ? gm_batch_unfused_sources(b, st) : src_bound;
                    const int64_t pb = pb0 + 4 * src * (int64_t)fi;
                    const int64_t pbs = pb0 + 4 * (gather ? std::min<int64_t>(src, b->feat_rows) : src) * (int64_t)fi;
                    gm_prof_note(GM_PROF_AGG_BOUND, pb0 + 4 * src_bound * (int64_t)fi - pb);
                    GM_TRY(launch_agg(a, pb, pbs, st));
                } else {
                    if (a.e_w) GM_TRY(gm_agg_stream_args(a, b, 0, gather, st));
                    int64_t strict = gm_aggregate_bytes(b, fi);
                    if (gather) strict += 4 * b->rows - 4 * b->rows * (int64_t)fi + std::min<int64_t>(4 * b->rows * (int64_t)fi, 4 * b->feat_rows * (int64_t)fi);
                    GM_TRY(launch_agg(a, gm_aggregate_bytes(b, fi), strict, st));
                    if (l == 0) c.z1_valid = 1;
                }
            }
            gm_gemm_args g{}; g.A = c.Z[l]; g.lda = fi; g.B = params + L.w_off[l]; g.b_stride = pstride; g.C = c.H[l]; g.ldc = fo; g.K = fi; g.N = fo;
            g.row_scale = b->d_norm; g.bias = params + L.b_off[l]; g.bias_stride = pstride; g.relu = 1; g.tiles = b->d_tiles; g.n_tiles = b->n_tiles; g.rows = b->rows;
            g.relu_bits = fwd_only == 1 ? nullptr : c.M[l];
            if (l == L.n_gcn - 1 && !mean && !c.centre && b->d_norm_c && (gm_knob().centre_store >= 2 || (gm_knob().centre_store == 1 && fwd_only == 1))) { g.row_scale_keep = b->d_norm_c; g.n_keep = b->n_c; }
            if (dead_rows && split_ok && l < L.n_gcn - 1 && (fwd_only == 1 || (fwd_only == 2 && c.M[l])) && L.dims[l + 1] <= L.dims[l + 2] && b->d_norm_src) {
                g.row_scale_keep = b->d_norm_src; g.n_keep = b->n_src;
            }
            if (obs == 1) { g.row_scale_keep = b->d_norm_e1; g.n_keep = gm_prof_enabled() ? gm_batch_e1_rows(b, st) : std::min<int64_t>(b->n_e1, b->rows); }
            if (split_ok) {
                gm_bound ab = gm_no_bound(), bb;
                const bool want16 = in_bound(c, l, ab);
                const uint16_t* pl = nullptr;
                int np = 3;
                GM_TRY(weight_planes(c, params, pstride, l, 0, fi, fo, want16, st, &pl, &bb, &np));
                g.Bsplit = pl; g.bsplit_stride = pstride ? (int64_t)3 * fi * fo : 0;
                g.np = np; g.a_bound = ab; g.b_bound = bb;
                if (np == 2) { g.amax_out = c.amH(l); c.hv[l] = true; }
            }
            if (fwd_only == 2 && l == L.n_gcn - 1 && fo == L.dims[L.n_gcn] && !mean) {
                const bool dz_ok = l == 0 || dz_centre_ok(c, l);
                if (dead_rows && split_ok && g.np != 2 && c.np != 2 && b->d_norm_c && dz_ok && gm_wgrad_gather_ok(b->n_chunks, fi, fo)) c.dq = GcnCtx::DQ_CENTRE;
                else { g.zero_out = c.bufA; c.dq = GcnCtx::DQ_ZEROED; }
            }
            if (fuse) {
                g.zside = c.Z[l]; g.ldz = fi;
                if (gather) { g.A = b->feat; g.lda = b->feat_ld; g.fuse2 = obs == 1 ? b->d_fwd_tab_feat : b->d_fuse2_feat; }
                else { g.A = xin; g.lda = fi; g.fuse2 = obs >= 0 ? b->d_fwd_tab[obs] : b->d_fuse2; }
            }
            GM_TRY(gm_launch_gemm_nn(g, st));
        }
        xin = c.H[l];
    }
    if (mean) GM_TRY(readout_fwd(c, st));
    return skip_head ? GM_OK : launch_head_fwd(c, params, pstride, logits, st);
}

static int gcn_backward_sparse(GcnCtx& c, const float* params, int64_t pstride, const float* dlogits, float* dparams, int64_t dstride, hipStream_t st, int skip_head);
static bool sparse_bwd_ok(const gm_layout& L);

static int gcn_backward(GcnCtx& c, const float* params, int64_t pstride, const float* dlogits, float* dparams, int64_t dstride, hipStream_t st, int sparse = 0,
                        int skip_head = 0) {
    if (c.cone) return cone_backward(c, params, pstride, dlogits, dparams, dstride, st, skip_head);
    if (sparse && sparse_bwd_ok(c.L)) return gcn_backward_sparse(c, params, pstride, dlogits, dparams, dstride, st, skip_head);
    const gm_layout& L = c.L; const gm_batch* b = c.b;
    const int Lg = L.n_gcn;
    float* dQ = c.bufA; float* T = c.bufB;
    c.hold.n = 0;
    const bool dq_centre = skip_head && c.dq == GcnCtx::DQ_CENTRE;
    const bool t_centre = dq_centre && c.t_zero && gm_knob().dead_rows >= 2;
    const bool dq_e1 = t_centre && Lg == 2 && L.dims[0] <= L.dims[1] && c.np != 2 && gm_wgrad_gather_ok(b->n_chunks, L.dims[0], L.dims[1]);
    if (!skip_head && mean_readout(c)) {
        GM_TRY(launch_head_bwd(c, params, pstride, dlogits, dparams, dstride, nullptr, c.Gpool, st));
        GM_TRY(readout_bwd(c, st));
    } else if (!skip_head) {
        GM_HIP(hipMemsetAsync(dQ, 0, sizeof(float) * b->rows * L.dims[Lg], st));
        GM_TRY(launch_head_bwd(c, params, pstride, dlogits, dparams, dstride, dQ, nullptr, st));
    }
    for (int l = Lg - 1; l >= 0; --l) {
        const int fi = L.dims[l], fo = L.dims[l + 1];
        const float* Xprev = l > 0 ? c.H[l - 1] : (c.x0_user ? c.x0_user : c.X0);
        const float* maskprev = l > 0 ? c.H[l - 1] : nullptr;
        const uint8_t* maskbits = l > 0 ? c.M[l - 1] : nullptr;
        if (maskbits) maskprev = nullptr;
        gm_wgrad_args w{}; w.chunks = b->d_chunks; w.n_chunks = b->n_chunks; w.set_chunk_off = b->d_set_chunk_off; w.sets = b->sets; w.rows = b->rows;
        w.partial = c.partial; w.dW = dparams + L.w_off[l]; w.dw_stride = dstride; w.db = dparams + L.b_off[l]; w.db_stride = dstride;
        w.a_scale = b->d_norm; w.K = fi; w.N = fo;
        wgrad_sgd(w, c, l);
        w.hold = &c.hold; w.hold_this = l > 0 ? 1 : 0;
        if (l > 0) w.partial = c.partial_l[l];
        if (fi > fo) {
            gm_agg_args a; GM_TRY(batch_agg(c, 1, st, a));
            a.x = dQ; a.ldx = fo; a.s_in = b->d_norm; a.e_w = b->d_enorm[1]; a.out = T; a.width = fo;
            GM_TRY(launch_agg(a, gm_aggregate_bytes(b, fo), gm_aggregate_bytes(b, fo), st));
            w.A = Xprev; w.lda = fi; w.G = T; w.ldg = fo; w.Gb = dQ; w.ldgb = fo;
            GM_TRY(gm_launch_wgrad(w, st));
            if (l > 0) {
                gm_gemm_args g{}; g.A = T; g.lda = fo; g.B = params + L.w_off[l]; g.b_stride = pstride; g.transB = 1; g.C = dQ; g.ldc = fi; g.K = fo; g.N = fi;
                g.row_scale = b->d_norm; g.mask_h = maskprev; g.mask_b = maskbits; g.tiles = b->d_tiles; g.n_tiles = b->n_tiles; g.rows = b->rows;
                GM_TRY(gm_launch_gemm_nn(g, st));
            }
        } else {
            w.A = c.Z[l]; w.lda = fi; w.G = dQ; w.ldg = fo;
            if (dq_centre && l == Lg - 1) w.g_keep = b->d_norm_c;
            if (dq_e1 && l == Lg - 2) w.g_keep = b->d_norm_e1;
            if (c.zfused[l]) {
                const bool gather = l == 0 && !c.x0_user;
                w.fuse2 = gather ? b->d_fuse2_feat : b->d_fuse2;
                w.gx = gather ? b->feat : (l > 0 ? c.H[l - 1] : c.x0_user); w.ldgx = gather ? b->feat_ld : fi;
            }
            if (l > 0) {
                gm_gemm_args g{}; g.A = dQ; g.lda = fo; g.C = T; g.ldc = fi; g.K = fo; g.N = fi;
                g.row_scale = b->d_norm; g.tiles = b->d_tiles; g.n_tiles = b->n_tiles; g.rows = b->rows;
                const bool use_split = dz_split_ok(c, l);
                const bool use_wt = !use_split && c.WTl[l] && fi % 64 == 0 && fo % 16 == 0;
                if (use_split) {
                    gm_bound ab = gm_no_bound(), bb;
                    const bool want16 = dq_bound(c, l, ab);
                    const uint16_t* pl = nullptr; int np = 3;
                    GM_TRY(weight_planes(c, params, pstride, l, 1, fo, fi, want16, st, &pl, &bb, &np));
                    g.Bsplit = pl; g.bsplit_stride = pstride ? (int64_t)3 * fi * fo : 0;
                    g.np = np; g.a_bound = ab; g.b_bound = bb;
                    if (np == 2) { g.amax_out = c.amT(l); c.tv[l] = true; }
                    g.B = params + L.w_off[l]; g.b_stride = pstride; g.transB = 1;
                    if (dq_centre && l == Lg - 1 && dz_centre_ok(c, l)) { g.fuse2 = b->d_dq_tab; g.zside = dQ; g.ldz = fo; }
                    if (t_centre && l == Lg - 1) { g.row_scale_keep = b->d_norm_c; g.n_keep = b->n_c; }
                } else if (use_wt) {
                    if (!(c.wt_of[l] == params && c.wt_stride[l] == pstride)) {
                        const int nt = pstride ? b->sets : 1;
                        hipLaunchKernelGGL(k_transpose_w, dim3((fo + 31) / 32, (fi + 31) / 32, nt), dim3(256), 0, st, params, pstride, L.w_off[l], fi, fo, c.WTl[l]);
                        GM_HIP(hipGetLastError());
                        c.wt_of[l] = params; c.wt_stride[l] = pstride;
                    }
                    g.B = c.WTl[l]; g.b_stride = pstride ? (int64_t)fi * fo : 0; g.transB = 0;
                } else { g.B = params + L.w_off[l]; g.b_stride = pstride; g.transB = 1; }
                GM_REQUIRE(!(dq_centre && l == Lg - 1) || g.fuse2, GM_EINVAL, "backward: dQ was left unfilled for a dZ GEMM that cannot read it through the table");
                GM_TRY(gm_launch_gemm_nn(g, st));
                if (use_wt && c.sgd.next) { w.wt_next = c.WTl[l]; }
            }
            int kn = 0;
            if (c.pd && c.sgd.next && (kn = c.pd->index_of(c.sgd.next)) != 0) { w.pl_fwd = c.pd->slot(kn, l, 0); w.pl_dz = c.pd->slot(kn, l, 1); }
            if (c.np == 2) {
                gm_bound ab, gb;
                if (in_bound(c, l, ab) && dq_bound(c, l, gb)) { w.np = 2; w.a_bound = ab; w.g_bound = gb; }
                if (kn) {
                    if (c.pd->w_bound(c.sgd.next, l, w.pl_bound)) w.pl_np = 2; else { w.pl_fwd = nullptr; w.pl_dz = nullptr; }
                }
            }
            GM_TRY(gm_launch_wgrad(w, st));
            if (kn) { c.pd->valid[kn][l][0] = w.pl_fwd != nullptr; c.pd->valid[kn][l][1] = w.pl_dz != nullptr; }
            if (w.wt_next) { c.wt_of[l] = c.sgd.next; c.wt_stride[l] = c.sgd.next_stride; }
            if (l > 0) {
                gm_agg_args a; GM_TRY(batch_agg(c, 1, st, a));
                a.x = T; a.ldx = fi; a.s_out = b->d_norm; a.mask_h = maskprev; a.mask_b = maskbits;
                a.out = dQ; a.width = fi;
                int64_t by = gm_aggregate_bytes(b, fi);
                if (t_centre && l == Lg - 1) {
                    a.x_idx = b->d_ect;
                    int64_t n_out = b->rows, e_out = b->edges;
                    if (dq_e1) {
                        a.s_out = b->d_norm_e1; a.keep_signed = 1;
// ... 1233 lines not shown
```

include/gmeta_hip.h:

```cpp
#ifndef GMETA_HIP_H
#define GMETA_HIP_H
#include <stdint.h>
#ifdef __cplusplus
extern "C" {
#endif

#define GM_OK 0
#define GM_EINVAL (-1)
#define GM_ENOMEM (-2)
#define GM_EHIP (-3)
#define GM_ERANGE (-4)
#define GM_MAX_GCN 4

typedef struct gm_store gm_store_t;
typedef struct gm_batch gm_batch_t;

typedef struct gm_seed { int32_t graph, i, j; } gm_seed_t;

typedef struct gm_model {
    int32_t n_gcn;
    int32_t dims[GM_MAX_GCN + 1];
    int32_t n_out;
    int32_t link_pred;
} gm_model_t;
// ... 94 lines not shown
enum gm_field {
    GM_F_SUB_OFF = 0,
    GM_F_SET_SUB_OFF,
    GM_F_PARENT,
    GM_F_GRAPH,
    GM_F_INDPTR,
    GM_F_INDICES,
    GM_F_INDPTR_T,
    GM_F_INDICES_T,
    GM_F_CENTRE,
    GM_F_NORM,
    GM_F_FEAT_ROW,
    GM_F_NORM_SRC,
    GM_F_NORM_CENTRE,
    GM_F_EDGE_W,
    GM_F_EDGE_W_T = 14,
    GM_F_HOP = 15,
    GM_F_NORM_E1 = 16,
    GM_F_EDGE_CENTRE_T = 17,
    GM_F_OBS_CENTRE = 18,
    GM_F_OBS_E1 = 19
};
int32_t gm_batch_weighted(const gm_batch_t* b);
int gm_batch_read(const gm_batch_t* b, int32_t field, void* host_dst, int64_t bytes);
int gm_batch_device_ptr(const gm_batch_t* b, int32_t field, void** dptr);
int gm_batch_source_rows(const gm_batch_t* b, int64_t* n_rows);
int gm_batch_e1_source_rows(const gm_batch_t* b, int64_t* n_rows);

int gm_gather_features(const gm_batch_t* b, float* x_out, void* stream);

int gm_aggregate(const gm_batch_t* b, int32_t transposed, int32_t gather, const float* x, int32_t width,
                 const float* s_in, const float* s_out, float* out, void* stream);
int64_t gm_aggregate_bytes(const gm_batch_t* b, int32_t width);

int64_t gm_model_param_count(const gm_model_t* m);
int64_t gm_gcn_ws_bytes(const gm_batch_t* b, const gm_model_t* m);
int gm_gcn_forward(const gm_batch_t* b, const gm_model_t* m, const float* params, int64_t param_stride,
                   const float* x0, const int32_t* centre_local, float* logits, void* ws, int64_t ws_bytes,
                   void* stream);
int gm_gcn_backward(const gm_batch_t* b, const gm_model_t* m, const float* params, int64_t param_stride,
                    const float* x0, const int32_t* centre_local, const float* dlogits, float* dparams,
                    int64_t dparam_stride, void* ws, int64_t ws_bytes, void* stream);

int gm_dense_update(const gm_batch_t* b, const float* x, int32_t K, const float* W, int64_t w_stride, int32_t N, float* out, int32_t mode,
                    void* stream);
int gm_dense_gemm(const gm_batch_t* b, const float* x, int64_t ldx, int32_t K, const float* W, int64_t w_stride, int32_t trans_w, int32_t N,
                  float* out, int64_t ldc, const float* s, const float* s_keep, const float* bias, int64_t bias_stride, int32_t relu,
                  uint8_t* relu_bits, const float* mask_h, const uint8_t* mask_b, float* zero_out, uint32_t* amax_out, int32_t mode,
                  int32_t* launched, void* stream);
int gm_dense_fused_gemm(const gm_batch_t* b, int32_t table, const float* x, int64_t ldx, int32_t K, const float* zside, int64_t ldz, const float* zfull,
                        int64_t ldzf, const float* W, int64_t w_stride, int32_t N, float* out, int64_t ldc, const float* s, const float* s_keep,
                        const float* bias, int64_t bias_stride, int32_t relu, uint8_t* relu_bits, float* zero_out, uint32_t* amax_out, int32_t mode,
                        int32_t* launched, void* stream);
int gm_dense_aggregate(const gm_batch_t* b, int32_t transposed, int32_t x_src, const float* x, int64_t ldx, int32_t width, int32_t scale_src,
                       const float* s_in, const float* s_out, int32_t keep_signed, const float* bias, int64_t bias_stride, int32_t relu,
                       uint8_t* relu_bits, const float* mask_h, const uint8_t* mask_b, int32_t hubs, const int32_t* rowlist, int64_t n_list,
                       int32_t list_win, int32_t list_sched, int32_t skip_lo, int32_t skip_hi, int32_t stream_ok, float* out, int32_t* launched,
                       void* stream);
int gm_dense_agg_info(const gm_batch_t* b, int32_t transposed, int64_t* info);
int gm_dense_fuse_counts(const gm_batch_t* b, int64_t* counts);
int gm_dense_agg_table(const gm_batch_t* b, int32_t which, int32_t transposed, void* dst, int64_t n, void* stream);
int gm_dense_dz_centre(const gm_batch_t* b, const float* dQ, int32_t K, const float* W, int64_t w_stride, int32_t N, float* T, void* stream);
int gm_dense_wgrad_centre(const gm_batch_t* b, const float* x, int32_t Kx, const float* dQ, int32_t N, float* dW, int64_t dw_stride, float* db,
                          int64_t db_stride, void* stream);
int gm_dense_agg_centre_t(const gm_batch_t* b, float* T, int32_t width, const uint8_t* mask_b, float* out, int32_t keep, void* stream);
int gm_dense_wgrad_e1(const gm_batch_t* b, const float* x, int32_t Kx, const float* dQ, int32_t N, float* dW, int64_t dw_stride, float* db,
                      int64_t db_stride, void* stream);
int gm_dense_wgrad(const gm_batch_t* b, const float* x, int64_t ldx, int32_t K, const float* g, int64_t ldg, int32_t N, const float* s,
                   const float* gb, int64_t ldgb, float* dW, int64_t dw_stride, float* db, int64_t db_stride, int32_t mode,
                   const float* cur, float* next, int64_t p_stride, float lr, float* wt, uint16_t* pl_fwd, uint16_t* pl_dz, void* stream);
int gm_dense_wgrad_fused(const gm_batch_t* b, int32_t table, const float* A, int64_t lda, int32_t K, const float* gx, int64_t ldgx, const float* g,
                         int64_t ldg, int32_t N, const float* s, const float* g_keep, float* dW, int64_t dw_stride, float* db, int64_t db_stride,
                         int32_t mode, void* stream);

int gm_proto_loss_spt(const gm_batch_t* b, const float* logits, int32_t n_out, const int32_t* y, int32_t n_support,
                      float* loss, float* acc, float* protos, float* dlogits, void* stream);
int gm_proto_loss_qry(const gm_batch_t* b, const float* logits, int32_t n_out, const int32_t* y, const float* protos,
                      int32_t c_task, float* loss, float* acc, float* dlogits, float* dprotos, void* stream);
void gm_set_ragged_classes(int32_t on);
int32_t gm_get_ragged_classes(void);
int gm_dense_head_loss(const gm_batch_t* b, const float* H, int32_t Hd, int32_t nc, int32_t compact, int32_t C, const float* params,
                       int64_t param_stride, int64_t wl_off, int64_t bl_off, const int32_t* centre_local, const int32_t* y, int32_t mode,
                       int32_t n_support, const float* protos, int32_t c_task, const int32_t* spt_labels, const int32_t* spt_counts, float* logits,
                       float* dlogits, float* dprotos, float* protos_out, float* loss, float* acc, int32_t bwd, float* dparams,
                       int64_t dparam_stride, float* dQ, float* Gc, const float* sgd_cur, float* sgd_next, int64_t sgd_stride, float sgd_lr,
                       uint32_t* dq_amax, int32_t path, int32_t* launched, void* stream);

#define GM_READOUT_CENTRE 0
#define GM_READOUT_MEAN 1
void gm_set_readout(int32_t mode);
int32_t gm_get_readout(void);

int64_t gm_meta_ws_bytes(const gm_batch_t* spt, const gm_batch_t* qry, const gm_model_t* m, const gm_hparams_t* hp);
int64_t gm_meta_out_floats(const gm_batch_t* spt, const gm_model_t* m, const gm_hparams_t* hp);
int gm_meta_step(const gm_batch_t* spt, const gm_batch_t* qry, const int32_t* y_spt, const int32_t* y_qry,
                 const gm_model_t* m, const gm_hparams_t* hp, const float* theta, float* out, int64_t out_floats,
                 void* ws, int64_t ws_bytes, void* stream);

int64_t gm_adapt_ws_bytes(const gm_batch_t* spt, const gm_model_t* m, const gm_hparams_t* hp);
int gm_meta_adapt(const gm_batch_t* spt, const int32_t* y_spt, const gm_model_t* m, const gm_hparams_t* hp, const float* theta, float* fw_out,
                  int64_t fw_stride, float* protos_out, int32_t c_task, void* ws, int64_t ws_bytes, void* stream);
int64_t gm_predict_ws_bytes(const gm_batch_t* qry, const gm_model_t* m, const gm_hparams_t* hp);
int gm_proto_predict(const gm_batch_t* qry, const gm_model_t* m, const gm_hparams_t* hp, const float* params, int64_t param_stride,
                     const float* protos, const int32_t* n_classes, int32_t c_task, float* logits_out, float* logp_out, int32_t* pred_out,
                     void* ws, int64_t ws_bytes, void* stream);

int gm_meta_finish(const float* head, int64_t P, int32_t K1, float* grad, float* found_inf, void* stream);
int gm_meta_finish_adam(const float* head, int64_t P, int32_t K1, float* theta, float* exp_avg, float* exp_avg_sq, float* grad, float* steps, int32_t n_steps,
                        float lr, float beta1, float beta2, float eps, float* found_inf, uint32_t* ticket, void* stream);

void gm_set_gemm_mode(int32_t mode);
int32_t gm_get_gemm_mode(void);
void gm_set_split_pieces(int32_t pieces);
int32_t gm_get_split_pieces(void);
int gm_set_tuning(const char* name, int32_t value);
int32_t gm_get_tuning(const char* name);
int32_t gm_tuning_epoch(void);

void gm_set_fuse_agg(int32_t on);
int32_t gm_get_fuse_agg(void);

void gm_profile_enable(int32_t on);
int gm_profile_aggregate(double* total_ms, int64_t* launches, int64_t* algorithmic_bytes);
int gm_profile_read(int32_t category, double* total_ms, int64_t* launches, int64_t* work);
int gm_profile_read_launches(int32_t category, double* ms, int64_t* work, int32_t cap);

// ... 5 lines not shown
```

Before: 1836.

## Restrict forward aggregation to observable rows via compact row lists

```diff
diff --git a/g-meta_amd/_lib.py b/g-meta_amd/_lib.py
--- a/g-meta_amd/_lib.py
+++ b/g-meta_amd/_lib.py
@@ -89,6 +89,7 @@
     'gm_dense_gemm': (C.c_int, [vp, vp, i64, i32, vp, i64, i32, i32, vp, i64, vp, vp, vp, i64, i32, vp, vp, vp, vp, vp, i32, vp, vp]),
     'gm_dense_fused_gemm': (C.c_int, [vp, i32, vp, i64, i32, vp, i64, vp, i64, vp, i64, i32, vp, i64, vp, vp, vp, i64, i32, vp, vp, vp, i32, vp, vp]),
     'gm_dense_wgrad_fused': (C.c_int, [vp, i32, vp, i64, i32, vp, i64, vp, i64, i32, vp, vp, vp, i64, vp, i64, i32, vp]),
+    'gm_dense_wgrad_fused_rows': (C.c_int, [vp, i32, vp, i64, i32, vp, i64, vp, i64, i32, vp, vp, vp, i64, vp, i64, i32, vp]),
     'gm_dense_aggregate': (C.c_int, [vp, i32, i32, vp, i64, i32, i32, vp, vp, i32, vp, i64, i32, vp, vp, vp, i32, vp, i64, i32, i32, i32, i32, i32, vp, vp, vp]),
     'gm_dense_agg_info': (C.c_int, [vp, i32, vp]),
     'gm_dense_fuse_counts': (C.c_int, [vp, vp]),
@@ -98,6 +99,9 @@
     'gm_dense_agg_centre_t': (C.c_int, [vp, vp, i32, vp, vp, i32, vp]),
     'gm_dense_wgrad_e1': (C.c_int, [vp, vp, i32, vp, i32, vp, i64, vp, i64, vp]),
     'gm_dense_wgrad': (C.c_int, [vp, vp, i64, i32, vp, i64, i32, vp, vp, i64, vp, i64, vp, i64, i32, vp, vp, i64, C.c_float, vp, vp, vp, vp]),
+    'gm_dense_fused_gemm_rows': (C.c_int, [vp, i32, i32, vp, i64, i32, vp, i64, vp, i64, i32, vp, i64, vp, vp, vp, i64, i32, vp, vp]),
+    'gm_dense_obs_list': (C.c_int, [vp, i32, vp, vp, i64, vp, i64, vp]),
+    'gm_dense_obs_aggregate': (C.c_int, [vp, i32, i32, vp, i64, i32, vp, vp]),
     'gm_proto_loss_spt': (C.c_int, [vp, vp, i32, vp, i32, vp, vp, vp, vp, vp]),
     'gm_proto_loss_qry': (C.c_int, [vp, vp, i32, vp, vp, i32, vp, vp, vp, vp, vp]),
     'gm_dense_head_loss': (C.c_int, [vp, vp, i32, i32, i32, i32, vp, i64, i64, i64, vp, vp, i32, i32, vp, i32, vp, vp, vp, vp, vp, vp, vp, vp, i32, vp, i64, vp, vp,
diff --git a/g-meta_amd/csrc/agg.hip b/g-meta_amd/csrc/agg.hip
--- a/g-meta_amd/csrc/agg.hip
+++ b/g-meta_amd/csrc/agg.hip
@@ -306,12 +306,13 @@
 }
 
 int gm_agg_schedule_flat(gm_batch* b, int64_t rows, int win, const int32_t* pos, int n_heavy, const std::vector<int32_t>& tab, int32_t** d_sched, int32_t* len_out,
-                         hipStream_t s, gm_stager* sg) {
+                         hipStream_t s, gm_stager* sg, const int32_t* ids) {
     const bool split = !tab.empty();
     const int RPB = win * (AGG_BLOCK / GM_WAVE);
     const int nwb = std::max(1, (int)((rows + RPB - 1) / RPB));
     auto x_start = [&](int x) { return agg_xcd_first(nwb, x); };
-    auto n_entries = [&](int k) { return split ? tab[k + 1] - tab[k] : 1; };
+    auto hub_of = [&](int k) { return ids ? ids[k] : k; };
+    auto n_entries = [&](int k) { return split ? tab[hub_of(k) + 1] - tab[hub_of(k)] : 1; };
     int extra[GM_NXCD] = {}; int first[GM_NXCD + 1];
     {
         int hk = 0;
@@ -335,8 +336,8 @@
         for (int hk = first[x]; hk < first[x + 1]; ++hk) {
             const int hb = pos[hk] / RPB;
             while (wb <= hb) *o++ = wb++;
-            if (split) for (int g = tab[hk]; g < tab[hk + 1]; ++g) *o++ = -g - 2;
-            else *o++ = -hk - 2;
+            if (split) for (int g = tab[hub_of(hk)]; g < tab[hub_of(hk) + 1]; ++g) *o++ = -g - 2;
+            else *o++ = -hub_of(hk) - 2;
         }
         while (wb < end) *o++ = wb++;
         while (o < o_end) *o++ = -1;
diff --git a/g-meta_amd/csrc/common.hip b/g-meta_amd/csrc/common.hip
--- a/g-meta_amd/csrc/common.hip
+++ b/g-meta_amd/csrc/common.hip
@@ -327,7 +327,7 @@
         k.gemm_mode = (gm && (!strcmp(gm, "split") || !strcmp(gm, "1"))) ? 1 : (gm && (!strcmp(gm, "f32") || !strcmp(gm, "0"))) ? 0 : -1;
         k.gemm_split_min_tiles = env("GM_GEMM_SPLIT_MIN_TILES", -1);
         k.centre_store = env("GM_CENTRE_STORE", 2);
-        k.dead_rows = env("GM_DEAD_ROWS", 3);
+        k.dead_rows = env("GM_DEAD_ROWS", 4);
         k.fuse_agg = env("GM_FUSE_AGG", 1);
         k.fuse_diff = env("GM_FUSE_DIFF", 2);
         k.extract_pref16 = env("GM_EXTRACT_PREF16", 1);
@@ -336,6 +336,7 @@
         k.query_streams = env("GM_QUERY_STREAMS", 0);
         k.agg_mid_list = env("GM_AGG_MID_LIST", 1);
         k.agg_mid_win = env("GM_AGG_MID_WIN", 0);
+        k.agg_obs_list = env("GM_AGG_OBS_LIST", 1);
         k.split_pieces = env("GM_SPLIT_PIECES", 3);
         k.split16_min_rows = env("GM_SPLIT16_MIN_ROWS", 65536);
         k.wgrad_split_min_chunks = env("GM_WGRAD_SPLIT_MIN_CHUNKS", -1);
@@ -366,7 +367,7 @@
     (void)gm_knob();
     static const struct { const char* name; int gm_knobs::*field; } tab[] = {
         {"GM_GEMM_SPLIT_MIN_TILES", &gm_knobs::gemm_split_min_tiles}, {"GM_CENTRE_STORE", &gm_knobs::centre_store}, {"GM_DEAD_ROWS", &gm_knobs::dead_rows},
-        {"GM_HEAD_STAGE", &gm_knobs::head_stage}, {"GM_HEAD_THREADS", &gm_knobs::head_threads}, {"GM_QUERY_STREAMS", &gm_knobs::query_streams}, {"GM_AGG_MID_LIST", &gm_knobs::agg_mid_list}, {"GM_AGG_MID_WIN", &gm_knobs::agg_mid_win}, {"GM_AGG_STREAM", &gm_knobs::agg_stream}, {"GM_AGG_STREAM_MIN_ROWS", &gm_knobs::agg_stream_min_rows},
+        {"GM_HEAD_STAGE", &gm_knobs::head_stage}, {"GM_HEAD_THREADS", &gm_knobs::head_threads}, {"GM_QUERY_STREAMS", &gm_knobs::query_streams}, {"GM_AGG_MID_LIST", &gm_knobs::agg_mid_list}, {"GM_AGG_MID_WIN", &gm_knobs::agg_mid_win}, {"GM_AGG_OBS_LIST", &gm_knobs::agg_obs_list}, {"GM_AGG_STREAM", &gm_knobs::agg_stream}, {"GM_AGG_STREAM_MIN_ROWS", &gm_knobs::agg_stream_min_rows},
         {"GM_SPLIT16_MIN_ROWS", &gm_knobs::split16_min_rows}, {"GM_WGRAD_SPLIT_MIN_CHUNKS", &gm_knobs::wgrad_split_min_chunks}, {"GM_TIMING", &gm_knobs::timing},
         {"GM_FUSE_DIFF", &gm_knobs::fuse_diff}, {"GM_EXTRACT_PREF16", &gm_knobs::extract_pref16},
         {"neg_round", &gm_knobs::neg_round}, {"GM_NEG_ROUND", &gm_knobs::neg_round},
diff --git a/g-meta_amd/csrc/dense_exports.hip b/g-meta_amd/csrc/dense_exports.hip
--- a/g-meta_amd/csrc/dense_exports.hip
+++ b/g-meta_amd/csrc/dense_exports.hip
@@ -89,15 +89,17 @@
     return rc;
 }
 
-extern "C" int gm_dense_fused_gemm(const gm_batch_t* b, int32_t table, const float* x, int64_t ldx, int32_t K, const float* zside, int64_t ldz,
-                                   const float* zfull, int64_t ldzf, const float* W, int64_t w_stride, int32_t N, float* out, int64_t ldc, const float* s,
-                                   const float* s_keep, const float* bias, int64_t bias_stride, int32_t relu, uint8_t* relu_bits, float* zero_out,
-                                   uint32_t* amax_out, int32_t mode, int32_t* launched, void* stream) {
-    GM_REQUIRE(b && W && out && zside && K >= 1 && N >= 1 && ldz >= K && ldc >= N && (mode == 1 || mode == 2) && (table == 0 || table == 1), GM_EINVAL,
+static int dense_fused_gemm(const gm_batch_t* b, int32_t table, int32_t bits_kept, const float* x, int64_t ldx, int32_t K, const float* zside, int64_t ldz,
+                            const float* zfull, int64_t ldzf, const float* W, int64_t w_stride, int32_t N, float* out, int64_t ldc, const float* s,
+                            const float* s_keep, const float* bias, int64_t bias_stride, int32_t relu, uint8_t* relu_bits, float* zero_out,
+                            uint32_t* amax_out, int32_t mode, int32_t* launched, void* stream) {
+    GM_REQUIRE(b && W && out && zside && K >= 1 && N >= 1 && ldz >= K && ldc >= N && (mode == 1 || mode == 2) && table >= 0 && table <= 4, GM_EINVAL,
                "dense_fused_gemm: bad arguments");
     GM_REQUIRE(b->d_fuse2 && b->d_fuse2_feat, GM_EINVAL, "dense_fused_gemm: the batch carries no source tables");
-    GM_REQUIRE(table == 1 || (x && ldx >= K), GM_EINVAL, "dense_fused_gemm: table 0 needs x and ldx >= K");
-    GM_REQUIRE(table == 0 || (b->feat && (K == b->feat_dim || K == b->feat_ld)), GM_EINVAL, "dense_fused_gemm: table 1 needs K == feat_dim (%d)", b->feat_dim);
+    GM_REQUIRE(table < 2 || (b->d_fwd_tab[0] && b->d_fwd_tab[1] && b->d_fwd_tab_feat), GM_EINVAL, "dense_fused_gemm: the batch carries no restricted source tables");
+    const bool over_feat = table == 1 || table == 4;
+    GM_REQUIRE(over_feat || (x && ldx >= K), GM_EINVAL, "dense_fused_gemm: a table over batch rows needs x and ldx >= K");
+    GM_REQUIRE(!over_feat || (b->feat && (K == b->feat_dim || K == b->feat_ld)), GM_EINVAL, "dense_fused_gemm: a table over feature rows needs K == feat_dim (%d)", b->feat_dim);
     GM_REQUIRE(!amax_out || mode == 2, GM_EINVAL, "dense_fused_gemm: amax_out is an output of the two-piece kernels (mode 2)");
     GM_REQUIRE(mode != 2 || (zfull && ldzf >= K), GM_EINVAL, "dense_fused_gemm: mode 2 takes its A bounds over a fully aggregated Z (zfull)");
     GM_REQUIRE((N == 256 || N == 128) && K % 16 == 0 && K >= 32, GM_EINVAL, "dense_fused_gemm: the split kernels need N = 128 or 256 and K a multiple of 16 (>= 32)");
@@ -106,11 +108,11 @@
     gm_gemm_args g{};
     g.B = W; g.b_stride = w_stride; g.C = out; g.ldc = ldc; g.K = K; g.N = N;
     g.row_scale = s; g.row_scale_keep = s_keep; g.n_keep = b->rows; g.bias = bias; g.bias_stride = bias_stride; g.relu = relu ? 1 : 0;
-    g.relu_bits = relu_bits; g.zero_out = zero_out;
+    g.relu_bits = relu_bits; g.bits_kept = bits_kept ? 1 : 0; g.zero_out = zero_out;
     g.tiles = b->d_tiles; g.n_tiles = b->n_tiles; g.rows = b->rows; g.launched = launched;
     g.zside = zside; g.ldz = ldz;
-    if (table == 1) { g.A = b->feat; g.lda = b->feat_ld; g.fuse2 = b->d_fuse2_feat; }
-    else { g.A = x; g.lda = ldx; g.fuse2 = b->d_fuse2; }
+    if (over_feat) { g.A = b->feat; g.lda = b->feat_ld; g.fuse2 = table == 1 ? b->d_fuse2_feat : b->d_fwd_tab_feat; }
+    else { g.A = x; g.lda = ldx; g.fuse2 = table == 0 ? b->d_fuse2 : b->d_fwd_tab[table - 2]; }
     uint16_t* planes = nullptr; unsigned* slots = nullptr;
     int rc = gm_alloc(&planes, (size_t)wsets * 3 * K * N, st);
     gm_bound wb = gm_no_bound();
@@ -129,6 +131,21 @@
     if (slots) gm_dev_free(slots, st);
     gm_batch_mark_use(b, st);
     return rc;
+}
+
+extern "C" int gm_dense_fused_gemm(const gm_batch_t* b, int32_t table, const float* x, int64_t ldx, int32_t K, const float* zside, int64_t ldz,
+                                   const float* zfull, int64_t ldzf, const float* W, int64_t w_stride, int32_t N, float* out, int64_t ldc, const float* s,
+                                   const float* s_keep, const float* bias, int64_t bias_stride, int32_t relu, uint8_t* relu_bits, float* zero_out,
+                                   uint32_t* amax_out, int32_t mode, int32_t* launched, void* stream) {
+    GM_REQUIRE(table == 0 || table == 1, GM_EINVAL, "dense_fused_gemm: bad arguments");
+    return dense_fused_gemm(b, table, 0, x, ldx, K, zside, ldz, zfull, ldzf, W, w_stride, N, out, ldc, s, s_keep, bias, bias_stride, relu, relu_bits, zero_out, amax_out, mode,
+                            launched, stream);
+}
+extern "C" int gm_dense_fused_gemm_rows(const gm_batch_t* b, int32_t table, int32_t bits_kept, const float* x, int64_t ldx, int32_t K, const float* zside, int64_t ldz,
+                                        const float* W, int64_t w_stride, int32_t N, float* out, int64_t ldc, const float* s, const float* s_keep, const float* bias,
+                                        int64_t bias_stride, int32_t relu, uint8_t* relu_bits, void* stream) {
+    return dense_fused_gemm(b, table, bits_kept, x, ldx, K, zside, ldz, nullptr, 0, W, w_stride, N, out, ldc, s, s_keep, bias, bias_stride, relu, relu_bits, nullptr, nullptr, 1,
+                            nullptr, stream);
 }
 
 extern "C" int gm_dense_dz_centre(const gm_batch_t* b, const float* dQ, int32_t K, const float* W, int64_t w_stride, int32_t N, float* T, void* stream) {
@@ -236,15 +253,17 @@
     return rc;
 }
 
-extern "C" int gm_dense_wgrad_fused(const gm_batch_t* b, int32_t table, const float* A, int64_t lda, int32_t K, const float* gx, int64_t ldgx, const float* g,
-                                    int64_t ldg, int32_t N, const float* s, const float* g_keep, float* dW, int64_t dw_stride, float* db, int64_t db_stride,
-                                    int32_t mode, void* stream) {
-    GM_REQUIRE(b && A && g && dW && db && K >= 1 && N >= 1 && lda >= K && ldg >= N && mode >= 0 && mode <= 2 && (table == 0 || table == 1), GM_EINVAL,
+static int dense_wgrad_fused(const gm_batch_t* b, int32_t table, const float* A, int64_t lda, int32_t K, const float* gx, int64_t ldgx, const float* g,
+                             int64_t ldg, int32_t N, const float* s, const float* g_keep, float* dW, int64_t dw_stride, float* db, int64_t db_stride,
+                             int32_t mode, void* stream) {
+    GM_REQUIRE(b && A && g && dW && db && K >= 1 && N >= 1 && lda >= K && ldg >= N && mode >= 0 && mode <= 2 && table >= 0 && table <= 4, GM_EINVAL,
                "dense_wgrad_fused: bad arguments");
     GM_REQUIRE(K <= 2048 && N <= 2048, GM_ERANGE, "dense_wgrad_fused: K=%d N=%d: at most 2048 columns per operand", K, N);
     GM_REQUIRE(b->d_fuse2 && b->d_fuse2_feat, GM_EINVAL, "dense_wgrad_fused: the batch carries no source tables");
-    GM_REQUIRE(table == 1 || (gx && ldgx >= K), GM_EINVAL, "dense_wgrad_fused: table 0 needs gx and ldgx >= K");
-    GM_REQUIRE(table == 0 || (b->feat && (K == b->feat_dim || K == b->feat_ld)), GM_EINVAL, "dense_wgrad_fused: table 1 needs K == feat_dim (%d)", b->feat_dim);
+    GM_REQUIRE(table < 2 || (b->d_fwd_tab[0] && b->d_fwd_tab[1] && b->d_fwd_tab_feat), GM_EINVAL, "dense_wgrad_fused: the batch carries no restricted source tables");
+    const bool over_feat = table == 1 || table == 4;
+    GM_REQUIRE(over_feat || (gx && ldgx >= K), GM_EINVAL, "dense_wgrad_fused: a table over batch rows needs gx and ldgx >= K");
+    GM_REQUIRE(!over_feat || (b->feat && (K == b->feat_dim || K == b->feat_ld)), GM_EINVAL, "dense_wgrad_fused: a table over feature rows needs K == feat_dim (%d)", b->feat_dim);
     const int sets = b->sets;
     const int64_t KN = (int64_t)K * N;
     GM_REQUIRE(sets == 1 || (dw_stride >= KN && db_stride >= N), GM_EINVAL, "dense_wgrad_fused: per-set outputs overlap");
@@ -253,8 +272,8 @@
     w.A = A; w.lda = lda; w.K = K; w.G = g; w.ldg = ldg; w.N = N; w.a_scale = s; w.g_keep = g_keep;
     w.chunks = b->d_chunks; w.n_chunks = b->n_chunks; w.set_chunk_off = b->d_set_chunk_off; w.sets = sets; w.rows = b->rows;
     w.dW = dW; w.dw_stride = dw_stride; w.db = db; w.db_stride = db_stride;
-    w.fuse2 = table == 1 ? b->d_fuse2_feat : b->d_fuse2;
-    w.gx = table == 1 ? b->feat : gx; w.ldgx = table == 1 ? b->feat_ld : ldgx;
+    w.fuse2 = table == 0 ? b->d_fuse2 : table == 1 ? b->d_fuse2_feat : table == 4 ? b->d_fwd_tab_feat : b->d_fwd_tab[table - 2];
+    w.gx = over_feat ? b->feat : gx; w.ldgx = over_feat ? b->feat_ld : ldgx;
     w.pick = mode == 0 ? GM_WGRAD_PICK_EXACT : GM_WGRAD_PICK_SPLIT;
     unsigned* slots = nullptr;
     int rc = gm_alloc(&w.partial, (size_t)std::max(1, b->n_chunks) * (size_t)(KN + N), st);
@@ -270,6 +289,18 @@
     if (slots) gm_dev_free(slots, st);
     gm_batch_mark_use(b, st);
     return rc;
+}
+
+extern "C" int gm_dense_wgrad_fused(const gm_batch_t* b, int32_t table, const float* A, int64_t lda, int32_t K, const float* gx, int64_t ldgx, const float* g,
+                                    int64_t ldg, int32_t N, const float* s, const float* g_keep, float* dW, int64_t dw_stride, float* db, int64_t db_stride,
+                                    int32_t mode, void* stream) {
+    GM_REQUIRE(table == 0 || table == 1, GM_EINVAL, "dense_wgrad_fused: bad arguments");
+    return dense_wgrad_fused(b, table, A, lda, K, gx, ldgx, g, ldg, N, s, g_keep, dW, dw_stride, db, db_stride, mode, stream);
+}
+extern "C" int gm_dense_wgrad_fused_rows(const gm_batch_t* b, int32_t table, const float* A, int64_t lda, int32_t K, const float* gx, int64_t ldgx, const float* g,
+                                         int64_t ldg, int32_t N, const float* s, const float* g_keep, float* dW, int64_t dw_stride, float* db, int64_t db_stride,
+                                         int32_t mode, void* stream) {
+    return dense_wgrad_fused(b, table, A, lda, K, gx, ldgx, g, ldg, N, s, g_keep, dW, dw_stride, db, db_stride, mode, stream);
 }
 
 extern "C" int gm_dense_aggregate(const gm_batch_t* b, int32_t transposed, int32_t x_src, const float* x, int64_t ldx, int32_t width, int32_t scale_src,
@@ -333,6 +364,42 @@
     return rc;
 }
 
+extern "C" int gm_dense_obs_list(const gm_batch_t* b, int32_t which, int64_t* info, int32_t* list_dst, int64_t n, int32_t* sched_dst, int64_t n_sched, void* stream) {
+    GM_REQUIRE(b && info && (which == 0 || which == 1) && n >= 0 && n_sched >= 0, GM_EINVAL, "dense_obs_list: bad arguments");
+    GM_REQUIRE(b->obs_ok[which], GM_EINVAL, "dense_obs_list: the batch carries no compact list %d", which);
+    info[0] = b->n_obs[which]; info[1] = b->obs_win[which]; info[2] = b->d_sched_obs[which] ? b->sched_len_obs[which] : 0; info[3] = b->n_obs_hubs[which];
+    GM_REQUIRE(n <= info[0] && n_sched <= GM_NXCD * info[2], GM_EINVAL, "dense_obs_list: list %d holds %lld rows and %lld schedule entries", which, (long long)info[0], (long long)(GM_NXCD * info[2]));
+    if (list_dst && n) GM_HIP(hipMemcpyAsync(list_dst, b->d_obs_list[which], 4 * (size_t)n, hipMemcpyDeviceToDevice, (hipStream_t)stream));
+    if (sched_dst && n_sched) GM_HIP(hipMemcpyAsync(sched_dst, b->d_sched_obs[which], 4 * (size_t)n_sched, hipMemcpyDeviceToDevice, (hipStream_t)stream));
+    gm_batch_mark_use(b, (hipStream_t)stream);
+    return GM_OK;
+}
+extern "C" int gm_dense_obs_aggregate(const gm_batch_t* b, int32_t which, int32_t x_src, const float* x, int64_t ldx, int32_t width, float* out, void* stream) {
+    GM_REQUIRE(b && out && (which == 0 || which == 1) && (x_src == 0 || x_src == 2) && width >= 1, GM_EINVAL, "dense_obs_aggregate: bad arguments");
+    GM_REQUIRE(b->obs_ok[which] && b->d_obs[which] && b->d_enorm[0], GM_EINVAL, "dense_obs_aggregate: the batch carries no compact list %d", which);
+    GM_REQUIRE(x_src == 2 || (x && ldx >= width), GM_EINVAL, "dense_obs_aggregate: a caller matrix needs x and ldx >= width");
+    GM_REQUIRE(x_src == 0 || (b->feat && b->d_efeat && width <= b->feat_ld), GM_EINVAL, "dense_obs_aggregate: the batch has no feature table of that width");
+    if (b->n_obs[which] == 0 && b->n_obs_hubs[which] == 0) return GM_OK;
+    hipStream_t st = (hipStream_t)stream;
+    gm_agg_args a{};
+    a.indptr = b->d_indptr; a.indices = b->d_indices; a.rows = b->rows; a.width = width; a.out = out;
+    if (x_src == 2) { a.x = b->feat; a.x_row = b->d_feat_row; a.x_idx = b->d_efeat; a.ldx = b->feat_ld; } else { a.x = x; a.ldx = ldx; }
+    a.s_in = b->d_norm; a.e_w = b->d_enorm[0];
+    a.s_out = b->d_obs[which]; a.keep_signed = 1;
+    a.skip_on = 1; a.skip_lo = 0; a.skip_hi = GM_FUSE_MAXDEG;
+    a.heavy_deg = b->heavy_deg;
+    a.rowlist = b->d_obs_list[which]; a.n_list = b->n_obs[which]; a.list_win = b->obs_win[which];
+    if (b->n_obs_hubs[which] > 0) {
+        GM_REQUIRE(b->d_sched_obs[which], GM_EINVAL, "dense_obs_aggregate: observable hub rows without a schedule");
+        a.heavy = b->d_heavy[0]; a.n_heavy = b->n_heavy[0];
+        a.sched = b->d_sched_obs[which]; a.sched_len = b->sched_len_obs[which]; a.sched_win = b->obs_win[which];
+        GM_TRY(gm_agg_hub(a, b, 0, st));
+    }
+    const int rc = gm_launch_aggregate(a, st);
+    gm_batch_mark_use(b, st);
+    return rc;
+}
+
 extern "C" int gm_dense_agg_info(const gm_batch_t* b, int32_t transposed, int64_t* info) {
     GM_REQUIRE(b && info, GM_EINVAL, "dense_agg_info: bad arguments");
     const int o = transposed ? 1 : 0;
diff --git a/g-meta_amd/csrc/extract.hip b/g-meta_amd/csrc/extract.hip
--- a/g-meta_amd/csrc/extract.hip
+++ b/g-meta_amd/csrc/extract.hip
@@ -648,6 +648,33 @@
     const int at = base + __popcll(m & ((1ull << lane) - 1ull));
     if (f && at < cap) list[at] = (int32_t)r;
 }
+__global__ __launch_bounds__(MID_BLOCK) void k_obs_count(const int32_t* indptr, int64_t rows, int lo, int hi, const float* obs, int32_t* bcnt, int32_t* total) {
+    __shared__ int wsum[MID_BLOCK / 64];
+    const int64_t r = (int64_t)blockIdx.x * MID_BLOCK + threadIdx.x;
+    const unsigned long long m = __ballot(mid_row(indptr, r, rows, lo, hi) && obs[r] > 0.f);
+    if ((threadIdx.x & 63) == 0) wsum[threadIdx.x >> 6] = __popcll(m);
+    __syncthreads();
+    if (threadIdx.x == 0) { int t = 0; for (int k = 0; k < MID_BLOCK / 64; ++k) t += wsum[k]; bcnt[blockIdx.x] = t; if (t) atomicAdd(total, t); }
+}
+__global__ __launch_bounds__(MID_BLOCK) void k_obs_scatter(const int32_t* indptr, int64_t rows, int lo, int hi, const float* obs, const int32_t* boff, int32_t* list, int cap) {
+    __shared__ int wsum[MID_BLOCK / 64];
+    const int64_t r = (int64_t)blockIdx.x * MID_BLOCK + threadIdx.x;
+    const bool f = mid_row(indptr, r, rows, lo, hi) && obs[r] > 0.f;
+    const unsigned long long m = __ballot(f);
+    const int lane = threadIdx.x & 63, wv = threadIdx.x >> 6;
+    if (lane == 0) wsum[wv] = __popcll(m);
+    __syncthreads();
+    int base = boff[blockIdx.x];
+    for (int k = 0; k < wv; ++k) base += wsum[k];
+    const int at = base + __popcll(m & ((1ull << lane) - 1ull));
+    if (f && at < cap) list[at] = (int32_t)r;
+}
+__global__ void k_obs_hubs(const int32_t* heavy, int n, const float* obs0, const float* obs1, int32_t* flags) {
+    const int j = blockIdx.x * blockDim.x + threadIdx.x;
+    if (j >= n) return;
+    const int32_t r = heavy[j];
+    flags[j] = obs0[r] > 0.f ? 1 : 0; flags[n + j] = obs1[r] > 0.f ? 1 : 0;
+}
 __global__ void k_centre_rows(const int32_t* sub_off, const int32_t* centre, int nc, int n_c, const int32_t* indptr, const float* norm,
                               int32_t* crow, float* cnorm, int32_t* cdeg, float* norm_c, int32_t* centre_copy, int4* dq_tab) {
     const int k = blockIdx.x * blockDim.x + threadIdx.x;
@@ -1061,6 +1088,45 @@
                                tc, te, tf, b->d_obs[0], b->d_obs[1]);
             GM_HIP(hipGetLastError());
             b->d_fwd_tab[0] = tc; b->d_fwd_tab[1] = te; b->d_fwd_tab_feat = tf;
+            const int nh = b->n_heavy[0];
+            if (gm_knob().agg_mid_list && h_cnt[0] <= cap && (nh == 0 || b->d_sched[0])) {
+                const int nb = (int)((b->rows + MID_BLOCK - 1) / MID_BLOCK);
+                const int64_t n_win = std::max<int64_t>(0, b->unfused_rows - (int64_t)nh);
+                const int64_t lcap[2] = {std::min<int64_t>(n_win, b->n_c), std::min<int64_t>(n_win, b->n_e1)};
+                int32_t* d_tmp = nullptr;
+                GM_TRY(gm_alloc(&d_tmp, (size_t)2 * nb + 2 + 2 * (size_t)std::max(1, nh), s));
+                int32_t* d_tot = d_tmp + 2 * nb; int32_t* d_flags = d_tot + 2;
+                GM_HIP(hipMemsetAsync(d_tot, 0, 2 * sizeof(int32_t), s));
+                for (int k = 0; k < 2; ++k) {
+                    GM_TRY(gm_balloc(b, &b->d_obs_list[k], (size_t)lcap[k], s));
+                    hipLaunchKernelGGL(k_obs_count, dim3(nb), dim3(MID_BLOCK), 0, s, b->d_indptr, (int64_t)b->rows, GM_FUSE_MAXDEG + 1, b->heavy_deg, b->d_obs[k], d_tmp + k * nb, d_tot + k);
+                    hipLaunchKernelGGL(k_mid_scan, dim3(1), dim3(1024), 0, s, d_tmp + k * nb, nb);
+                    hipLaunchKernelGGL(k_obs_scatter, dim3(nb), dim3(MID_BLOCK), 0, s, b->d_indptr, (int64_t)b->rows, GM_FUSE_MAXDEG + 1, b->heavy_deg, b->d_obs[k], d_tmp + k * nb,
+                                       b->d_obs_list[k], (int)lcap[k]);
+                }
+                if (nh > 0) hipLaunchKernelGGL(k_obs_hubs, dim3((nh + 255) / 256), dim3(256), 0, s, b->d_heavy[0], nh, b->d_obs[0], b->d_obs[1], d_flags);
+                GM_HIP(hipGetLastError());
+                const int32_t* h_tot = sg.download((const int32_t*)d_tot, (size_t)2 + 2 * (size_t)std::max(1, nh));
+                GM_REQUIRE(h_tot, GM_ENOMEM, "finalize: pinned staging failed");
+                GM_HIP(hipStreamSynchronize(s));
+                gm_dev_free(d_tmp, s);
+                for (int k = 0; k < 2; ++k) {
+                    const int64_t n = h_tot[k];
+                    GM_REQUIRE(n >= 0 && n <= lcap[k], GM_EHIP, "finalize: %lld observable window rows exceed their bound %lld", (long long)n, (long long)lcap[k]);
+                    b->n_obs[k] = (int32_t)n;
+                    int win = 64;
+                    while (win > 2 && n / win < 16384) win >>= 1;
+                    if (gm_knob().agg_mid_win > 0) win = gm_knob().agg_mid_win;
+                    b->obs_win[k] = win;
+                    std::vector<int32_t> ids, pos;
+                    for (int j = 0; j < nh; ++j) if (h_tot[2 + k * nh + j]) {
+                        ids.push_back(j); pos.push_back((int32_t)std::min<int64_t>(std::max<int64_t>(n, 1) - 1, (int64_t)heavy0[j] * n / b->rows));
+                    }
+                    b->n_obs_hubs[k] = (int32_t)ids.size();
+                    if (!ids.empty()) GM_TRY(gm_agg_schedule_flat(b, n, win, pos.data(), (int)ids.size(), tab0, &b->d_sched_obs[k], &b->sched_len_obs[k], s, &sg, ids.data()));
+                    b->obs_ok[k] = true;
+                }
+            }
         }
     }
     std::vector<int32_t> ccoff, ecoff, c_set_off(b->sets + 1), e_set_off(b->sets + 1);
diff --git a/g-meta_amd/csrc/gemm.hip b/g-meta_amd/csrc/gemm.hip
--- a/g-meta_amd/csrc/gemm.hip
+++ b/g-meta_amd/csrc/gemm.hip
@@ -443,6 +443,7 @@
         SplitGemmK k{};
         k.A = a.A; k.lda = a.lda; k.Bt = a.Bsplit; k.bt_stride = a.bsplit_stride; k.C = a.C; k.ldc = a.ldc; k.K = a.K; k.N = a.N;
         k.row_scale = a.row_scale_keep ? a.row_scale_keep : a.row_scale; k.keep_signed = a.row_scale_keep ? 1 : 0; k.bias = a.bias; k.bias_stride = a.bias_stride; k.relu = a.relu; k.relu_bits = a.relu_bits;
+        k.bits_kept = (a.bits_kept && a.row_scale_keep && a.relu_bits) ? 1 : 0;
         k.tiles = a.tiles; k.n_tiles = a.n_tiles; k.n_col_tiles = 1; k.nt_store = 1; k.zero_out = a.zero_out;
         const bool f16 = a.np == 2;
         GM_REQUIRE(!f16 || (a.a_bound.amax && a.b_bound.amax), GM_EINVAL, "gemm: the two-piece split kernel needs bounds for both operands");
@@ -1132,7 +1133,7 @@
                "wgrad: the split kernel needs K, N in {128, 256}, no Gb / row indirection and 16-byte aligned operands (K=%d N=%d)", a.K, a.N);
     const int cat = split ? (wgrad_np(a) == 2 ? GM_PROF_WGRAD_SPLIT16 : GM_PROF_WGRAD_SPLIT) : GM_PROF_WGRAD;
     gm_prof_begin(cat, s, 2 * a.rows * a.K * a.N);
-    gm_prof_note(GM_PROF_WGRAD_BYTES, 4 * a.rows * ((int64_t)a.K + a.N));
+    gm_prof_note(GM_PROF_WGRAD_BYTES, 4 * ((a.fuse2 && a.a_rows > 0) ? a.a_rows : a.rows) * (int64_t)a.K + 4 * a.rows * (int64_t)a.N);
     const int rc = launch_wgrad(a, s);
     gm_prof_end(cat, s);
     return rc;
diff --git a/g-meta_amd/csrc/gemm_split.h b/g-meta_amd/csrc/gemm_split.h
--- a/g-meta_amd/csrc/gemm_split.h
+++ b/g-meta_amd/csrc/gemm_split.h
@@ -38,7 +38,7 @@
     const uint8_t* mask_b; uint8_t* relu_bits;
     const int32_t* tiles; int n_tiles; int n_col_tiles; int nt_store;
     unsigned long long* dbg;
-    int dephase;
+    int bits_kept;
     float* zero_out;
     const int4* f2; const float* zside; int64_t ldz; const float* zrow;
     gm_bound a_bound, b_bound; unsigned* amax_out;
@@ -500,7 +500,7 @@
 #pragma unroll
             for (int j = 0; j < 2; ++j) b4[j] = *reinterpret_cast<const float4*>(biasl + (ti & 1) * BN + wc * 64 + j * 32 + q4 * 4);
             if constexpr (NP == 2) { if (g.amax_out && tl.set != vmax_set) { if (vmax_set >= 0) vmax_flush(); vmax_set = tl.set; } }
-            const bool keep_only = g.keep_signed && !g.relu_bits && !g.zero_out;
+            const bool keep_only = g.keep_signed && (!g.relu_bits || g.bits_kept) && !g.zero_out;
             if (keep_only && __ballot(!(__float_as_uint(sc_t[wr * 32 * MI + (lane & (32 * MI - 1))]) >> 31)) == 0ull) continue;
 #pragma unroll
             for (int i = 0; i < MI; ++i) {
diff --git a/g-meta_amd/csrc/gm_internal.h b/g-meta_amd/csrc/gm_internal.h
--- a/g-meta_amd/csrc/gm_internal.h
+++ b/g-meta_amd/csrc/gm_internal.h
@@ -157,6 +157,8 @@
     void* d_fwd_tab[2] = {nullptr, nullptr};
     void* d_fwd_tab_feat = nullptr;
     float* d_obs[2] = {nullptr, nullptr};
+    int32_t* d_obs_list[2] = {nullptr, nullptr}; int32_t n_obs[2] = {0, 0}, obs_win[2] = {0, 0}, n_obs_hubs[2] = {0, 0}; bool obs_ok[2] = {false, false};
+    int32_t* d_sched_obs[2] = {nullptr, nullptr}; int32_t sched_len_obs[2] = {0, 0};
     mutable int64_t fwd_cnt[2][3] = {{-1, -1, -1}, {-1, -1, -1}};
     float* d_e1_norm = nullptr;
     float* d_e1_coef = nullptr;
@@ -189,6 +191,7 @@
     int fuse_agg, head_stage;
     int fuse_diff;
     int agg_mid_win;
+    int agg_obs_list;
     int agg_mid_list;
     int query_streams;
     int head_threads;
@@ -433,7 +436,7 @@
 }
 int gm_agg_window(int64_t rows, int64_t edges);
 struct gm_stager;
-int gm_agg_schedule_flat(gm_batch* b, int64_t rows, int win, const int32_t* pos, int n_heavy, const std::vector<int32_t>& tab, int32_t** d_sched, int32_t* len, hipStream_t s, gm_stager* sg);
+int gm_agg_schedule_flat(gm_batch* b, int64_t rows, int win, const int32_t* pos, int n_heavy, const std::vector<int32_t>& tab, int32_t** d_sched, int32_t* len, hipStream_t s, gm_stager* sg, const int32_t* ids = nullptr);
 int gm_agg_schedule(gm_batch* b, int64_t rows, int win, const int32_t* heavy_host, const int32_t* heavy_deg_host, int n_heavy, gm_agg_sched* out, hipStream_t s, gm_stager* sg);
 int gm_heavy_deg();
 int gm_heavy_deg_for(int64_t rows, int64_t edges);
@@ -453,6 +456,7 @@
     const float* mask_h;
     const uint8_t* mask_b;
     uint8_t* relu_bits;
+    int bits_kept;
     const uint16_t* Bsplit; int64_t bsplit_stride;
     const void* fuse2; const float* zside; int64_t ldz;
     int np; gm_bound a_bound, b_bound; unsigned* amax_out;
@@ -499,6 +503,7 @@
     float* wt_next;
     int64_t rows;
     const void* fuse2; const float* gx; int64_t ldgx;
+    int64_t a_rows;
     const float* g_keep;
     gm_wgrad_hold* hold; int hold_this;
     int pick;
diff --git a/g-meta_amd/csrc/model.hip b/g-meta_amd/csrc/model.hip
--- a/g-meta_amd/csrc/model.hip
+++ b/g-meta_amd/csrc/model.hip
@@ -598,6 +598,7 @@
     enum DqFill { DQ_MEMSET, DQ_ZEROED, DQ_CENTRE } dq = DQ_MEMSET;
     bool t_zero = false;
     bool zfused[GM_MAX_GCN] = {};
+    int8_t zrows[GM_MAX_GCN] = {};
     float* Z[GM_MAX_GCN]; float* H[GM_MAX_GCN]; float* X0; float* bufA; float* bufB; float* partial;
     float* partial_l[GM_MAX_GCN];
     gm_wgrad_hold hold;
@@ -773,6 +774,10 @@
 
 static bool dz_split_ok(const GcnCtx& c, int l) { return c.Wsplit && gm_gemm_split_ok(c.b->n_tiles, c.L.dims[l + 1], c.L.dims[l]); }
 static bool dz_centre_ok(const GcnCtx& c, int l) { return dz_split_ok(c, l) && c.L.dims[l + 1] >= 64 && c.L.dims[l + 1] <= 4096 && c.b->d_dq_tab; }
+static bool dq_e1_ok(const GcnCtx& c) {
+    const gm_layout& L = c.L;
+    return L.n_gcn == 2 && L.dims[0] <= L.dims[1] && c.np != 2 && gm_wgrad_gather_ok(c.b->n_chunks, L.dims[0], L.dims[1]);
+}
 static float* t_zero_rows(const GcnCtx& c) {
     const gm_layout& L = c.L; const int Lg = L.n_gcn;
     if (c.cone || Lg < 2 || !c.bufB || L.dims[Lg - 1] > L.dims[Lg]) return nullptr;
@@ -795,6 +800,7 @@
 extern "C" int32_t gm_get_fuse_agg(void) { const int o = g_fuse_agg_override.load(std::memory_order_relaxed); return o >= 0 ? o : gm_knob().fuse_agg; }
 
 static int gcn_forward(GcnCtx& c, const float* params, int64_t pstride, float* logits, hipStream_t st, int reuse_z1, int skip_head = 0, int fwd_only = 0) {
+    for (int l = 0; l < GM_MAX_GCN; ++l) c.zrows[l] = 0;
     if (c.cone) return cone_forward(c, params, pstride, logits, st, reuse_z1, skip_head);
     const gm_layout& L = c.L; const gm_batch* b = c.b;
     if (!c.x0_user) GM_TRY(gm_check_feat_dim(b, L.dims[0], "forward"));
@@ -827,10 +833,17 @@
                            b->d_fwd_tab[0] && b->d_obs[0] && L.dims[Lg - 1] <= L.dims[Lg] && layer_fuse(Lg - 1) &&
                            (Lg >= 2 || c.x0_user);
     const bool fwd3_below = fwd3_last && Lg >= 2 && L.dims[Lg - 2] <= L.dims[Lg - 1] && layer_split_ok(Lg - 2) && b->d_fwd_tab[1] && b->d_fwd_tab_feat && b->d_obs[1];
+    const bool dq_centre_fwd = fwd_only == 2 && !mean && L.dims[Lg - 1] <= L.dims[Lg] && dead_rows && layer_split_ok(Lg - 1) && c.np != 2 && b->d_norm_c &&
+                               (Lg == 1 || dz_centre_ok(c, Lg - 1)) && gm_wgrad_gather_ok(b->n_chunks, L.dims[Lg - 1], L.dims[Lg]);
+    const bool diff4_last = dq_centre_fwd && skip_head && gm_knob().dead_rows >= 4 && gm_knob().centre_store >= 2 && Lg >= 2 &&
+                            b->d_norm_e1 && b->d_fwd_tab[0] && b->d_obs[0] && layer_fuse(Lg - 1);
+    const bool diff4_below = diff4_last && c.t_zero && gm_knob().dead_rows >= 2 && dq_e1_ok(c) && c.M[Lg - 2] && layer_fuse(Lg - 2) &&
+                             b->d_fwd_tab[1] && b->d_fwd_tab_feat && b->d_obs[1];
     for (int l = 0; l < L.n_gcn; ++l) {
         const int fi = L.dims[l], fo = L.dims[l + 1];
         const bool gather = (l == 0 && !c.x0_user);
-        const int obs = (fwd3_last && l == Lg - 1) ? 0 : (fwd3_below && l == Lg - 2) ? 1 : -1;
+        const int obs = ((fwd3_last || diff4_last) && l == Lg - 1) ? 0 : ((fwd3_below || diff4_below) && l == Lg - 2) ? 1 : -1;
+        c.zrows[l] = (fwd_only == 2 && obs >= 0) ? (int8_t)(obs + 1) : 0;
         if (fi > fo) {
             const float* A = xin; int64_t lda = fi;
             if (gather) { GM_TRY(gm_gather_rows(b, b->d_feat_row, b->rows, fi, c.X0, st)); A = c.X0; }
@@ -866,6 +879,13 @@
                         w[2] = std::min<int64_t>(w[1], b->rows);
                         if (gm_prof_enabled()) GM_TRY(gm_batch_fwd_counts(b, obs, st, w));
                         pb0 = 4 * (b->rows + 1) + 8 * b->unfused_rows + 4 * w[1] + 4 * w[0] * (int64_t)fi;
+                        if (gm_knob().dead_rows >= 4 && gm_knob().agg_obs_list && a.rowlist && b->obs_ok[obs] && (b->n_obs_hubs[obs] == 0 || b->d_sched_obs[obs]) &&
+                            (b->n_obs[obs] > 0 || b->n_obs_hubs[obs] > 0)) {
+                            a.rowlist = b->d_obs_list[obs]; a.n_list = b->n_obs[obs]; a.list_win = b->obs_win[obs];
+                            if (b->n_obs_hubs[obs] > 0) { a.sched = b->d_sched_obs[obs]; a.sched_len = b->sched_len_obs[obs]; a.sched_win = b->obs_win[obs]; }
+                            else { a.sched = nullptr; a.sched_len = 0; a.heavy = nullptr; a.n_heavy = 0; }
+                            pb0 = 12 * w[0] + 4 * w[1] + 4 * w[0] * (int64_t)fi;
+                        }
                         src = w[2]; src_bound = std::min<int64_t>(w[1], b->rows);
                     } else src = gm_prof_enabled() ? gm_batch_unfused_sources(b, st) : src_bound;
                     const int64_t pb = pb0 + 4 * src * (int64_t)fi;
@@ -888,6 +908,7 @@
                 g.row_scale_keep = b->d_norm_src; g.n_keep = b->n_src;
             }
             if (obs == 1) { g.row_scale_keep = b->d_norm_e1; g.n_keep = gm_prof_enabled() ? gm_batch_e1_rows(b, st) : std::min<int64_t>(b->n_e1, b->rows); }
+            if (obs == 1 && fwd_only == 2) g.bits_kept = 1;
             if (split_ok) {
                 gm_bound ab = gm_no_bound(), bb;
                 const bool want16 = in_bound(c, l, ab);
@@ -899,10 +920,10 @@
                 if (np == 2) { g.amax_out = c.amH(l); c.hv[l] = true; }
             }
             if (fwd_only == 2 && l == L.n_gcn - 1 && fo == L.dims[L.n_gcn] && !mean) {
-                const bool dz_ok = l == 0 || dz_centre_ok(c, l);
-                if (dead_rows && split_ok && g.np != 2 && c.np != 2 && b->d_norm_c && dz_ok && gm_wgrad_gather_ok(b->n_chunks, fi, fo)) c.dq = GcnCtx::DQ_CENTRE;
+                if (dq_centre_fwd && g.np != 2) c.dq = GcnCtx::DQ_CENTRE;
                 else { g.zero_out = c.bufA; c.dq = GcnCtx::DQ_ZEROED; }
             }
+            GM_REQUIRE(!(c.zrows[l] == 1) || c.dq == GcnCtx::DQ_CENTRE, GM_EINVAL, "forward: Z_L was restricted to the centre rows for a backward that reads dQ_L whole");
             if (fuse) {
                 g.zside = c.Z[l]; g.ldz = fi;
                 if (gather) { g.A = b->feat; g.lda = b->feat_ld; g.fuse2 = obs == 1 ? b->d_fwd_tab_feat : b->d_fuse2_feat; }
@@ -921,6 +942,7 @@
 
 static int gcn_backward(GcnCtx& c, const float* params, int64_t pstride, const float* dlogits, float* dparams, int64_t dstride, hipStream_t st, int sparse = 0,
                         int skip_head = 0) {
+    if (c.cone || (sparse && sparse_bwd_ok(c.L))) for (int l = 0; l < GM_MAX_GCN; ++l) GM_REQUIRE(!c.zrows[l], GM_EINVAL, "backward: layer %d ran on restricted rows, which only the dense backward can read", l);
     if (c.cone) return cone_backward(c, params, pstride, dlogits, dparams, dstride, st, skip_head);
     if (sparse && sparse_bwd_ok(c.L)) return gcn_backward_sparse(c, params, pstride, dlogits, dparams, dstride, st, skip_head);
     const gm_layout& L = c.L; const gm_batch* b = c.b;
@@ -929,7 +951,13 @@
     c.hold.n = 0;
     const bool dq_centre = skip_head && c.dq == GcnCtx::DQ_CENTRE;
     const bool t_centre = dq_centre && c.t_zero && gm_knob().dead_rows >= 2;
-    const bool dq_e1 = t_centre && Lg == 2 && L.dims[0] <= L.dims[1] && c.np != 2 && gm_wgrad_gather_ok(b->n_chunks, L.dims[0], L.dims[1]);
+    const bool dq_e1 = t_centre && dq_e1_ok(c);
+    for (int l = 0; l < Lg; ++l) {
+        if (!c.zrows[l]) continue;
+        GM_REQUIRE(c.zfused[l] && L.dims[l] <= L.dims[l + 1], GM_EINVAL, "backward: layer %d ran on restricted rows without the fused loader", l);
+        GM_REQUIRE(!skip_head || (c.zrows[l] == 1 ? (dq_centre && l == Lg - 1) : (dq_e1 && l == Lg - 2)), GM_EINVAL,
+                   "backward: the forward left layer %d's unobservable rows unwritten, and this pass would read them (dQ is not restricted to match)", l);
+    }
     if (!skip_head && mean_readout(c)) {
         GM_TRY(launch_head_bwd(c, params, pstride, dlogits, dparams, dstride, nullptr, c.Gpool, st));
         GM_TRY(readout_bwd(c, st));
@@ -967,6 +995,9 @@
             if (c.zfused[l]) {
                 const bool gather = l == 0 && !c.x0_user;
                 w.fuse2 = gather ? b->d_fuse2_feat : b->d_fuse2;
+                if (c.zrows[l] == 1) { w.fuse2 = b->d_fwd_tab[0]; w.a_rows = b->n_c; }
+                if (c.zrows[l] == 2) { w.fuse2 = gather ? b->d_fwd_tab_feat : b->d_fwd_tab[1]; w.a_rows = gm_prof_enabled() ? gm_batch_e1_rows(b, st) : std::min<int64_t>(b->n_e1, b->rows); }
+                GM_REQUIRE(w.fuse2, GM_EINVAL, "backward: no source table for layer %d", l);
                 w.gx = gather ? b->feat : (l > 0 ? c.H[l - 1] : c.x0_user); w.ldgx = gather ? b->feat_ld : fi;
             }
             if (l > 0) {
diff --git a/include/gmeta_hip.h b/include/gmeta_hip.h
--- a/include/gmeta_hip.h
+++ b/include/gmeta_hip.h
@@ -170,6 +170,11 @@
                         int64_t ldzf, const float* W, int64_t w_stride, int32_t N, float* out, int64_t ldc, const float* s, const float* s_keep,
                         const float* bias, int64_t bias_stride, int32_t relu, uint8_t* relu_bits, float* zero_out, uint32_t* amax_out, int32_t mode,
                         int32_t* launched, void* stream);
+int gm_dense_fused_gemm_rows(const gm_batch_t* b, int32_t table, int32_t bits_kept, const float* x, int64_t ldx, int32_t K, const float* zside, int64_t ldz,
+                             const float* W, int64_t w_stride, int32_t N, float* out, int64_t ldc, const float* s, const float* s_keep, const float* bias,
+                             int64_t bias_stride, int32_t relu, uint8_t* relu_bits, void* stream);
+int gm_dense_obs_list(const gm_batch_t* b, int32_t which, int64_t* info, int32_t* list_dst, int64_t n, int32_t* sched_dst, int64_t n_sched, void* stream);
+int gm_dense_obs_aggregate(const gm_batch_t* b, int32_t which, int32_t x_src, const float* x, int64_t ldx, int32_t width, float* out, void* stream);
 int gm_dense_aggregate(const gm_batch_t* b, int32_t transposed, int32_t x_src, const float* x, int64_t ldx, int32_t width, int32_t scale_src,
                        const float* s_in, const float* s_out, int32_t keep_signed, const float* bias, int64_t bias_stride, int32_t relu,
                        uint8_t* relu_bits, const float* mask_h, const uint8_t* mask_b, int32_t hubs, const int32_t* rowlist, int64_t n_list,
@@ -190,6 +195,9 @@
 int gm_dense_wgrad_fused(const gm_batch_t* b, int32_t table, const float* A, int64_t lda, int32_t K, const float* gx, int64_t ldgx, const float* g,
                          int64_t ldg, int32_t N, const float* s, const float* g_keep, float* dW, int64_t dw_stride, float* db, int64_t db_stride,
                          int32_t mode, void* stream);
+int gm_dense_wgrad_fused_rows(const gm_batch_t* b, int32_t table, const float* A, int64_t lda, int32_t K, const float* gx, int64_t ldgx, const float* g,
+                              int64_t ldg, int32_t N, const float* s, const float* g_keep, float* dW, int64_t dw_stride, float* db, int64_t db_stride,
+                              int32_t mode, void* stream);
 
 int gm_proto_loss_spt(const gm_batch_t* b, const float* logits, int32_t n_out, const int32_t* y, int32_t n_support,
                       float* loss, float* acc, float* protos, float* dlogits, void* stream);
```

Result: no change. 1842, median of 3 (+0.3%).
